# hpgmg/hpgmg

Measured on AMD Instinct MI355X. Metric: DOF/s (fine-grid) for FMG F-cycle, higher is better.
Workload: dtype f64

## Files before the change

### hpgmg_amd/__init__.py

```python
import ctypes
import os

_PKG = os.path.dirname(os.path.abspath(__file__))
REPO_ROOT = os.path.dirname(_PKG)

VECTOR_TEMP, VECTOR_U, VECTOR_F, VECTOR_E, VECTOR_R, VECTOR_DINV = 0, 1, 2, 3, 4, 5
VECTOR_BETA_I, VECTOR_BETA_J, VECTOR_BETA_K, VECTOR_ALPHA, VECTOR_L1INV = 6, 7, 8, 9, 10
BC_PERIODIC, BC_DIRICHLET = 0, 1
STENCIL_SHAPE_BOX, STENCIL_SHAPE_STAR, STENCIL_SHAPE_NO_CORNERS = 0, 1, 2
RESTRICT_CELL, RESTRICT_FACE_I, RESTRICT_FACE_J, RESTRICT_FACE_K = 0, 1, 2, 3
OP_7PT, OP_27PT, OP_FV4, OP_FV2 = 0, 1, 2, 3
SMOOTH_CHEBY, SMOOTH_GSRB, SMOOTH_JACOBI = 0, 1, 2
BOTTOM_BICGSTAB, BOTTOM_CG, BOTTOM_CABICGSTAB, BOTTOM_CACG = 0, 1, 2, 3
(INFO_DIM, INFO_BOX_DIM, INFO_GHOSTS, INFO_JSTRIDE, INFO_KSTRIDE, INFO_VOLUME, INFO_NUM_MY_BOXES,
 INFO_NUM_VECTORS, INFO_BOXES_IN_I, INFO_MY_RANK, INFO_NUM_RANKS, INFO_NUM_MY_BLOCKS, INFO_ACTIVE, INFO_COUNT) = range(14)


class Config(ctypes.Structure):
    _fields_ = [("op", ctypes.c_int), ("smoother", ctypes.c_int), ("helmholtz", ctypes.c_int), ("variable_coeff", ctypes.c_int)]


class UserInfo(ctypes.Structure):
    _fields_ = [("norm_of_residual", ctypes.c_double), ("norm_of_f", ctypes.c_double), ("mean_shift", ctypes.c_double),
                ("vcycles", ctypes.c_int), ("converged", ctypes.c_int)]


DENSE_CELL, DENSE_FACE_I, DENSE_FACE_J, DENSE_FACE_K = 0, 1, 2, 3
DENSE_CHECK_FINITE, DENSE_CHECK_POSITIVE, DENSE_CHECK_NONNEGATIVE = 0, 1, 2
DENSE_NOT_FINITE, DENSE_OUT_OF_RANGE = 1, 2
WHERE_HOST, WHERE_PLUGIN = 0, 1
(USER_OK, USER_BAD_ARGUMENT, USER_CONFLICT, USER_MULTI_RANK, USER_NOT_FINITE, USER_OUT_OF_RANGE,
 USER_NOT_READY, USER_UNSUPPORTED) = 0, -1, -2, -3, -4, -5, -6, -7
USER_FMG, USER_MG, USER_PCG, USER_FPCG = 0, 1, 2, 3
FACE_DIRICHLET, FACE_NEUMANN, FACE_ROBIN = 0, 1, 3


class HipLevel(ctypes.Structure):
    _fields_ = [("box_base", ctypes.c_void_p), ("box_low", ctypes.c_void_p), ("num_boxes", ctypes.c_int),
                ("dim", ctypes.c_int), ("ghosts", ctypes.c_int), ("jStride", ctypes.c_int), ("kStride", ctypes.c_int),
                ("volume", ctypes.c_int), ("dim_i", ctypes.c_int), ("dim_j", ctypes.c_int), ("dim_k", ctypes.c_int),
                ("periodic", ctypes.c_int), ("box_nbr", ctypes.c_void_p), ("flags", ctypes.c_int), ("box_stride", ctypes.c_longlong)]


def _declare_driver_api(lib):
    c_int, c_dbl, vp = ctypes.c_int, ctypes.c_double, ctypes.c_void_p
    P = ctypes.POINTER
    sig = {
        "hpgmg_configure": (c_int, [P(Config)]),
        "hpgmg_get_config": (None, [P(Config)]),
        "hpgmg_vectors_reserved": (c_int, []),
        "hpgmg_backend_name": (ctypes.c_char_p, []),
        "hpgmg_set_verbose": (None, [c_int]),
        "hpgmg_set_box_alignment": (None, [c_int, c_int, c_int, c_int]),
        "hpgmg_choose_boxes_in_i": (c_int, [c_int, c_int, c_int]),
        "hpgmg_solver_create": (vp, [c_int, c_int, c_int, c_int, c_int]),
        "hpgmg_solver_create_explicit": (vp, [c_int, c_int, c_int, c_int, c_int]),
        "hpgmg_solver_destroy": (None, [vp]),
        "hpgmg_solver_num_levels": (c_int, [vp]),
        "hpgmg_solver_level": (vp, [vp, c_int]),
        "hpgmg_solver_restrict_rhs": (None, [vp, c_int]),
        "hpgmg_solver_fmg": (c_dbl, [vp, c_int]),
        "hpgmg_solver_bench": (c_dbl, [vp, c_int, c_int, c_int]),
        "hpgmg_solver_richardson": (None, [vp, P(c_dbl)]),
        "hpgmg_level_info": (None, [vp, P(c_int)]),
        "hpgmg_level_h": (c_dbl, [vp]),
        "hpgmg_level_timers": (None, [vp, P(c_dbl)]),
        "hpgmg_set_timer_mode": (None, [c_int]),
        "hpgmg_get_timer_mode": (c_int, []),
        "hpgmg_level_eigenvalue": (c_dbl, [vp]),
        "hpgmg_level_must_subtract_mean": (c_int, [vp]),
        "hpgmg_level_set_eigenvalue": (None, [vp, c_dbl]),
        "hpgmg_level_box_low": (None, [vp, c_int, P(c_int)]),
        "hpgmg_level_list_counts": (c_int, [vp, c_int, c_int, P(c_int)]),
        "hpgmg_level_read_vector": (None, [vp, c_int, c_int, vp]),
        "hpgmg_level_write_vector": (None, [vp, c_int, c_int, vp]),
        "hpgmg_level_create": (vp, [c_int, c_int, c_int, c_int, c_int, c_int, c_int, c_dbl]),
        "hpgmg_level_destroy": (None, [vp]),
        "hpgmg_mg_create": (vp, [vp, c_dbl, c_dbl, c_int]),
        "hpgmg_mg_destroy": (None, [vp]),
        "hpgmg_mg_level": (vp, [vp, c_int]),
        "hpgmg_mg_num_levels": (c_int, [vp]),
        "hpgmg_set_transport": (None, [vp]),
        "hpgmg_set_bottom_solver": (None, [c_int]), "hpgmg_get_bottom_solver": (c_int, []),
        "hpgmg_set_ucycles": (None, [c_int]),
        "hpgmg_set_fmg_vcycles": (None, [c_int]),
        "MGSolve": (None, [vp, c_int, c_int, c_int, c_dbl, c_dbl, c_dbl]),
        "FMGSolve": (None, [vp, c_int, c_int, c_int, c_dbl, c_dbl, c_dbl]),
        "MGPCG": (None, [vp, c_int, c_int, c_int, c_dbl, c_dbl, c_dbl]),
        "hpgmg_solver_mg": (vp, [vp]),
        "stencil_get_radius": (c_int, []), "stencil_get_shape": (c_int, []),
        "apply_op": (None, [vp, c_int, c_int, c_dbl, c_dbl]),
        "residual": (None, [vp, c_int, c_int, c_int, c_dbl, c_dbl]),
        "smooth": (None, [vp, c_int, c_int, c_dbl, c_dbl]),
        "rebuild_operator": (None, [vp, vp, c_dbl, c_dbl]),
        "restriction": (None, [vp, c_int, vp, c_int, c_int]),
        "interpolation_vcycle": (None, [vp, c_int, c_dbl, vp, c_int]),
        "interpolation_fcycle": (None, [vp, c_int, c_dbl, vp, c_int]),
        "exchange_boundary": (None, [vp, c_int, c_int]),
        "apply_BCs": (None, [vp, c_int, c_int]),
        "apply_BCs_p1": (None, [vp, c_int, c_int]),
        "dot": (c_dbl, [vp, c_int, c_int]), "norm": (c_dbl, [vp, c_int]), "mean": (c_dbl, [vp, c_int]),
        "matmul": (None, [vp, P(c_dbl), P(c_int), P(c_int), c_int, c_int, c_int]),
        "error": (c_dbl, [vp, c_int, c_int]),
        "add_vectors": (None, [vp, c_int, c_dbl, c_int, c_dbl, c_int]),
        "scale_vector": (None, [vp, c_int, c_dbl, c_int]),
        "zero_vector": (None, [vp, c_int]),
        "shift_vector": (None, [vp, c_int, c_int, c_dbl]),
        "mul_vectors": (None, [vp, c_int, c_dbl, c_int, c_int]),
        "invert_vector": (None, [vp, c_int, c_dbl, c_int]),
        "init_vector": (None, [vp, c_int, c_dbl]),
        "color_vector": (None, [vp, c_int, c_int, c_int, c_int, c_int]),
        "random_vector": (None, [vp, c_int]),
        "initialize_problem": (None, [vp, c_dbl, c_dbl, c_dbl]),
        "IterativeSolver": (None, [vp, c_int, c_int, c_dbl, c_dbl, c_dbl]),
        "hpgmg_dense_pack": (c_int, [vp, c_int, vp, c_int, c_int, c_int]),
        "hpgmg_dense_unpack": (c_int, [vp, c_int, vp, c_int]),
        "hpgmg_user_create": (c_int, [c_int, c_int, c_int, c_int, c_int, c_dbl, c_dbl, c_dbl, P(vp)]),
        "hpgmg_user_destroy": (None, [vp]),
        "hpgmg_user_set_verbose": (None, [vp, c_int]),
        "hpgmg_user_solver_of": (vp, [vp]),
        "hpgmg_user_set_coefficients": (c_int, [vp, vp, vp, vp, vp, c_int]),
        "hpgmg_user_set_rhs": (c_int, [vp, vp, c_int, P(c_dbl)]),
        "hpgmg_user_solve": (c_int, [vp, c_int, c_dbl, vp, c_int, P(UserInfo)]),
        "hpgmg_user_set_max_iterations": (c_int, [vp, c_int]),
        "hpgmg_user_get_solution": (c_int, [vp, vp, c_int]),
        "hpgmg_user_apply": (c_int, [vp, vp, vp, c_int]),
        "hpgmg_user_set_rhs_dirichlet": (c_int, [vp, vp, vp, c_int, P(c_dbl)]),
        "hpgmg_user_apply_dirichlet": (c_int, [vp, vp, vp, vp, c_int]),
        "hpgmg_dense_pack_lifted": (c_int, [vp, c_int, vp, c_int, vp, c_dbl]),
        "hpgmg_boundary_flux": (c_int, [vp, vp, vp, c_dbl]),
        "hpgmg_boundary_restrict": (None, [vp, vp, vp, vp]),
        "hpgmg_boundary_lift": (None, [vp, c_int, vp, vp, c_dbl]),
        "hpgmg_boundary_interp": (None, [vp, c_int, vp, vp]),
        "hpgmg_user_create_faces": (c_int, [c_int, c_int, P(c_int), c_int, c_int, c_dbl, c_dbl, c_dbl, P(vp)]),
        "hpgmg_dense_pack_walls": (c_int, [vp, c_int, vp, c_int, c_int, c_int, c_int, vp]),
        "hpgmg_dense_pack_lifted_faces": (c_int, [vp, c_int, vp, c_int, vp, c_dbl, c_int, vp]),
        "hpgmg_boundary_flux_faces": (c_int, [vp, vp, vp, c_dbl, c_int, vp]),
        "hpgmg_boundary_interp_faces": (None, [vp, c_int, vp, vp, c_int]),
        "hpgmg_user_set_coefficients_robin": (c_int, [vp, vp, vp, vp, vp, vp, c_int]),
        "hpgmg_boundary_check_kappa": (c_int, [vp, vp, c_int, c_int, P(c_int)]),
        "hpgmg_boundary_store_walls": (None, [vp, vp, vp, c_int]),
        "hpgmg_dense_pack_lifted_robin": (c_int, [vp, c_int, vp, c_int, vp, c_dbl, c_int, vp, vp]),
        "hpgmg_boundary_flux_robin": (c_int, [vp, vp, vp, c_dbl, c_int, vp, vp]),
        "hpgmg_boundary_interp_robin": (None, [vp, c_int, vp, vp, c_int, vp]),
        "hpgmg_user_flux": (c_int, [vp, vp, vp, vp, vp, vp, c_int]),
        "hpgmg_dense_unpack_flux": (c_int, [vp, c_int, vp, c_dbl, c_int, vp, vp, vp, vp, vp, c_int]),
        "hpgmg_pcg_apply_dot": (c_int, [vp, c_int, c_int, c_dbl, c_dbl, P(c_dbl)]),
        "hpgmg_pcg_update": (c_int, [vp, c_int, c_int, c_int, c_int, c_dbl, P(c_dbl)]),
        "hpgmg_pcg_dot": (c_int, [vp, c_int, c_int, P(c_dbl)]),
        "hpgmg_pcg_dot2": (c_int, [vp, c_int, c_int, c_int, P(c_dbl), P(c_dbl)]),
        "hpgmg_vector_alloc": (vp, [ctypes.c_size_t]),
        "hpgmg_vector_free": (None, [vp]),
        "hpgmg_vector_copy": (None, [vp, vp, ctypes.c_size_t]),
        "hpgmg_vector_upload": (None, [vp, vp, ctypes.c_size_t]),
        "hpgmg_vector_download": (None, [vp, vp, ctypes.c_size_t]),
    }
    for name, (res, args) in sig.items():
        fn = getattr(lib, name)
        fn.restype, fn.argtypes = res, args
    return lib


def _declare_kernel_api(lib):
    c_int, c_dbl, vp = ctypes.c_int, ctypes.c_double, ctypes.c_void_p
    P = ctypes.POINTER
    L = P(HipLevel)
    sig = {
        "hpgmg_hip_device_count": (c_int, []), "hpgmg_hip_set_device": (c_int, [c_int]),
        "hpgmg_hip_set_stream": (None, [vp]), "hpgmg_hip_get_stream": (vp, []), "hpgmg_hip_sync": (c_int, []),
        "hpgmg_hip_malloc": (vp, [ctypes.c_size_t]), "hpgmg_hip_free": (None, [vp]),
        "hpgmg_hip_memcpy_h2d": (c_int, [vp, vp, ctypes.c_size_t]), "hpgmg_hip_memcpy_d2h": (c_int, [vp, vp, ctypes.c_size_t]),
        "hpgmg_hip_last_error": (ctypes.c_char_p, []),
        "hpgmg_hip_event_create": (vp, []), "hpgmg_hip_event_destroy": (None, [vp]),
        "hpgmg_hip_event_record": (c_int, [vp]), "hpgmg_hip_event_elapsed_ms": (c_dbl, [vp, vp]),
        "hpgmg_hip_profile_smoother": (None, [c_int]),
        "hpgmg_hip_profile_smoother_min_cells": (None, [ctypes.c_longlong]),
        "hpgmg_hip_profile_smoother_stride": (None, [c_int]),
        "hpgmg_hip_profile_smoother_read": (c_int, [P(c_dbl), P(ctypes.c_longlong), P(ctypes.c_longlong)]),
        "hpgmg_hip_smooth_cheby": (c_int, [L, c_int, c_int, c_int, c_int, c_dbl, c_dbl, c_dbl, c_dbl, c_dbl]),
        "hpgmg_hip_smooth_gsrb": (c_int, [L, c_int, c_int, c_int, c_int, c_dbl, c_dbl, c_dbl, c_int]),
        "hpgmg_hip_smooth_jacobi": (c_int, [L, c_int, c_int, c_int, c_int, c_dbl, c_dbl, c_dbl, c_dbl]),
        "hpgmg_hip_residual": (c_int, [L, c_int, c_int, c_int, c_int, c_dbl, c_dbl, c_dbl]),
        "hpgmg_hip_fill": (c_int, [L, c_int, c_dbl]),
        "hpgmg_hip_axpby": (c_int, [L, c_int, c_dbl, c_int, c_dbl, c_int]),
        "hpgmg_hip_scale": (c_int, [L, c_int, c_dbl, c_int]),
        "hpgmg_hip_norm_max": (c_int, [L, c_int, P(c_dbl)]),
        "hpgmg_hip_dot": (c_int, [L, c_int, c_int, P(c_dbl)]),
        "hpgmg_hip_sum": (c_int, [L, c_int, P(c_dbl)]),
        "hpgmg_hip_gram": (c_int, [L, P(c_int), c_int, P(c_int), c_int, P(c_dbl)]),
        "hpgmg_hip_pcg_dot2": (c_int, [L, c_int, c_int, c_int, P(c_dbl), P(c_dbl)]),
        "hpgmg_hip_pair_launch_counts": (None, [P(ctypes.c_longlong)]),
    }
    for name, (res, args) in sig.items():
        fn = getattr(lib, name)
        fn.restype, fn.argtypes = res, args
    return lib


def lib_paths():
    return os.path.join(_PKG, "libhpgmg_hip.so"), os.path.join(_PKG, "libhpgmg_fv.so")


_cache = {}


def load_kernels():
    if "hip" not in _cache:
        path = lib_paths()[0]
        if not os.path.exists(path):
            raise ImportError(f"{path} is missing: run `make -C hpgmg_amd/csrc` (or __graft_entry__.build()); "
                              "there is no CPU fallback for the operator kernels")
        _cache["hip"] = _declare_kernel_api(ctypes.CDLL(path, mode=ctypes.RTLD_GLOBAL))
    return _cache["hip"]


def load_driver():
    if "fv" not in _cache:
        load_kernels()
        path = lib_paths()[1]
        if not os.path.exists(path):
            raise ImportError(f"{path} is missing: run `make -C hpgmg_amd/csrc` (or __graft_entry__.build())")
        lib = _declare_driver_api(ctypes.CDLL(path))
        if lib.hpgmg_backend_name() != b"hip":
            raise ImportError("libhpgmg_fv.so is not linked against the HIP operator plugin")
        _cache["fv"] = lib
    return _cache["fv"]


def bind_driver_library(path):
    return _declare_driver_api(ctypes.CDLL(path))
```

### hpgmg_amd/csrc/host/plugin_internal.h

```cpp
#ifndef HPGMG_PLUGIN_INTERNAL_H
#define HPGMG_PLUGIN_INTERNAL_H
#include <stdio.h>
#include <stdlib.h>
#include <string.h>
#include <math.h>
#include <time.h>
#include <stdint.h>
#include "hpgmg_level.h"
#include "hpgmg_operators.h"
#include "hpgmg_mg.h"
#include "hpgmg_hip.h"

int hpgmg_smooth_sweeps(void);
int hpgmg_gsrb_out_of_place(void);

#define HP_INTERNAL __attribute__((visibility("hidden")))

enum { TIMERS_HOST = 0, TIMERS_DEVICE = 1, TIMERS_SYNC = 2 };
#define TICK(L, FIELD, WHAT) const hpgmg_tick tick_ = hpgmg_tick_begin((L), &(L)->timers.FIELD, WHAT)
#define TOCK() hpgmg_tick_end(tick_)
HP_INTERNAL void hp_lazy_flush(void);
#define HIP_OK(call) do { hp_lazy_flush(); int e_ = (call); if (e_) { fprintf(stderr, "hpgmg: %s failed (%d): %s\n", #call, e_, hpgmg_hip_last_error()); abort(); } } while (0)

#define MAX_LISTS 32
typedef struct {
  hpgmg_hip_level dev;
  double **d_box_base;  int *d_box_low;  int *d_box_nbr;  int all_faces_local;
  double  *seen_v0;     int seen_nv, seen_boxes;
  struct { const blockCopy_type *host; int n; blockCopy_type *dev; } lists[MAX_LISTS];
  int num_lists;
  hpgmg_hip_bc_entry *d_bc[STENCIL_MAX_SHAPES]; int n_bc[STENCIL_MAX_SHAPES];
  int *d_fv4_special; int n_fv4_special;
  hpgmg_hip_bc_entry *d_bc_k; int n_bc_k, bc_k_local;
  int bc_sources_local[STENCIL_MAX_SHAPES];
  int *krylov_pinned;
  double *dense_stage; size_t dense_stage_len;
  double *pair_scratch; double **d_pair_base;
  float *coef32; float **d_coef32_base; int coef32_valid;
  int lexicographic;
  int *d_restrict_map;
  struct pair_halo *halo;
  int halo_state;
  struct halo_images *img;
  int img_state;
  int img_active;
} backend_t;

enum { HALO_FIRST = 0, HALO_NEXT = 1, HALO_COEF = 2, HALO_PLANS = 3 };
typedef struct {
  int n_send, n_recv;
  hpgmg_hip_halo_entry *d_send, *d_recv;
  int n_sp, n_rp;
  int *sp_rank, *rp_rank, *sp_size, *rp_size;
  double **sp_ptr, **rp_ptr;
} halo_plan;
typedef struct pair_halo {
  int brick[3], rem[6];
  halo_plan plan[HALO_PLANS];
  double *sendbuf, *recvbuf, *deep, *deep_beta;
  int coef_valid;
} pair_halo;

enum { IMG_PLAN_COEF = 6, IMG_PLANS = 7 };
typedef struct {
  int n_send, n_recv;
  hpgmg_hip_halo_entry *d_send, *d_recv;
  int n_sp, n_rp;
  int *sp_rank, *rp_rank, *sp_size, *rp_size;
  long long *sp_off, *rp_off;
  int built;
} image_plan;
typedef struct halo_images {
  int n_real, n_img, n_all;
  int *gid;
  int *h_nbr;
  int lo[3], n[3];
  int *brick_lo, *brick_n;
  int depth_max;
  double *storage, *scratch;
  double **d_box_base, **d_pair_base; int *d_box_low, *d_box_nbr;
  hpgmg_hip_level dev, dev_all;
  image_plan plan[IMG_PLANS];
  double *sendbuf, *recvbuf; size_t send_cap, recv_cap;
  double **ptr_tmp; int ptr_cap;
  hpgmg_hip_bc_entry *d_bc; int n_bc, n_bc_own;
  hpgmg_hip_bc_entry *d_bc_k; int n_bc_k;
  int *d_special; int n_special;
  int coef_valid, shape;
  double *seen_v0; int seen_nv;
} halo_images;

typedef enum { SW_GHOST_FREE = 0, SW_ONE_LAUNCH_GHOSTS, SW_OVERLAP, SW_PAIR_REMOTE, SW_IMAGES, SW_FUSED_SWEEPS, SW_PAIR_MIN_CELLS, SW_FUSED_RESIDUAL, SW_FUSED_TAIL,
               SW_FUSED_FTAIL, SW_FUSED_BOTTOM, SW_SMALL_FUSED, SW_SMALL_VTAIL, SW_SMALL_27PT_GSRB, SW_SMALL_OPS, SW_LAZY, SW_LAZY_REPORT, SW_TEMP_SCRATCH,
               SW_FV4_NO_EXACT_RB, SW_GRAPH, SW_SMOOTHER_PRECISION, SW_DEFER_NORM, SW_BRICK_VISITS, SW_BRICK_SIZE, SW_BRICK_MIN_DIM, SW_BRICK_FSTEP, SW_BRICK_CHAIN, SW_BRICK_WIDE, SW_BRICK_WIDE_MAX_DIM, SW_BRICK_WIDE_TAIL_DIM, SW_FTAIL_MAX_DIM, SW_COUNT } hp_switch_id;
HP_INTERNAL long long hp_switch(hp_switch_id id);
HP_INTERNAL void hp_switch_set(hp_switch_id id, long long value);

HP_INTERNAL backend_t *hp_backend_of(level_type *L);
HP_INTERNAL const blockCopy_type *hp_mirror(level_type *owner, const blockCopy_type *host, int n);
HP_INTERNAL int  hp_variant(void);
HP_INTERNAL int  hp_ghost_free_mode(void);
HP_INTERNAL int  hp_box_rank_at(const level_type *L, int bi, int bj, int bk);
HP_INTERNAL void hp_ensure_pair_scratch(level_type *L, backend_t *B);
HP_INTERNAL int  hp_bc_entry_from_block(const level_type *L, int box, const int bpos[3], const int lo[3], const int len[3], int subtype,
                                        int (*find)(void *, int), void *ctx, hpgmg_hip_bc_entry *o);
HP_INTERNAL int  hp_images_ready(level_type *L, backend_t *B);
HP_INTERNAL void hp_images_refresh(level_type *L, backend_t *B, int scr, int id, int depth, int rhs_id, int bc_order);
HP_INTERNAL int  hp_images_refresh_begin(level_type *L, backend_t *B, int scr, int id, int depth, int rhs_id, int bc_order);
HP_INTERNAL void hp_images_refresh_end(void);
HP_INTERNAL int  hp_overlap_enabled(void);
HP_INTERNAL void hp_overlap_counted(void);
HP_INTERNAL void hp_images_bcs(level_type *L, backend_t *B, int scr, int id, int bc_order, int part);
HP_INTERNAL const int *hp_images_fv4_special(level_type *L, backend_t *B, int *n_out);
HP_INTERNAL const hpgmg_hip_bc_entry *hp_images_bc_k(level_type *L, backend_t *B, int *n_out);
HP_INTERNAL void hp_images_release(backend_t *B);
HP_INTERNAL void hp_images_invalidate_coefficients(backend_t *B);
extern HP_INTERNAL long long hp_images_exchanges;
static inline const hpgmg_hip_level *hp_stencil_dev(backend_t *B) { return (B->img && B->img_active) ? &B->img->dev : &B->dev; }


extern HP_INTERNAL void *hp_comm_stream, *hp_ev_packed, *hp_ev_landed;
extern HP_INTERNAL long long hp_overlap_count;
HP_INTERNAL double hp_now(void);
HP_INTERNAL void hp_transport_phase(const communicator_type *recv_side, const communicator_type *send_side, int tag);
HP_INTERNAL int hp_exchange_and_bcs_one_launch(level_type *L, int id, int shape, int order, int with_copies);
HP_INTERNAL int hp_ghosts_for_stencil(level_type *L, int id, int out_id);
HP_INTERNAL int hp_overlap_begin(level_type *L, int id);
HP_INTERNAL void hp_overlap_end(void);
HP_INTERNAL void hp_no_kernel(const char *what);
HP_INTERNAL const hpgmg_hip_bc_entry *hp_bc_entries(level_type *L, int shape, int *n_out);
HP_INTERNAL const hpgmg_hip_bc_entry *hp_bc_entries_k(level_type *L, int *n_out, int *all_local_out);
HP_INTERNAL int hp_vcycle_legs_fused(level_type **levels, int n, int e_id, int R_id, double a, double b, int leg);
HP_INTERNAL void hp_coef32_invalidate(level_type *L);
HP_INTERNAL int hp_interp_smooth_fused(level_type *Lf, int e_id, int R_id, level_type *Lc, double a, double b, int exact_state);
HP_INTERNAL void hp_do_smooth(level_type *L, int x_id, int rhs_id, double a, double b, int temp_dead);
HP_INTERNAL void hp_do_residual(level_type *L, int res_id, int x_id, int rhs_id, double a, double b);
HP_INTERNAL void hp_do_apply_op(level_type *L, int Ax_id, int x_id, double a, double b);
HP_INTERNAL int hp_pair_halo_ready(level_type *L, backend_t *B);
HP_INTERNAL int hp_pair_halo_begin(level_type *L, backend_t *B, int first, int x0_scr, int x0_id, int xm1_scr, int xm1_id, int rhs_id);
HP_INTERNAL void hp_do_restriction(level_type *Lc, int id_c, level_type *Lf, int id_f, int type);
HP_INTERNAL int hp_residual_restrict_zero_fused(level_type *Lc, int id_c, level_type *Lf, int res_id, int x_id, int rhs_id, double a, double b, int zero_id);
HP_INTERNAL int hp_norm_scale_restrict_fused(level_type *L, int F_id, int R_id, level_type *Lc, double *norm_out);
HP_INTERNAL void hp_do_interpolation_vcycle(level_type *Lf, int id_f, double prescale, level_type *Lc, int id_c);
HP_INTERNAL void hp_do_zero_vector(level_type *L, int id);
HP_INTERNAL void hp_do_add_vectors(level_type *L, int c, double sa, int a, double sb, int b);
HP_INTERNAL void hp_do_mul_vectors(level_type *L, int c, double s, int a, int b);
HP_INTERNAL void hp_do_scale_vector(level_type *L, int c, double s, int a);
HP_INTERNAL double hp_allreduce_scalar(level_type *L, double v, int op);
HP_INTERNAL void hp_allreduce_values(level_type *L, double *v, int n, int op);
HP_INTERNAL double hp_do_dot(level_type *L, int a, int b);
HP_INTERNAL double hp_do_norm(level_type *L, int a);
HP_INTERNAL void hp_small_ops_forget(void);
HP_INTERNAL const int *hp_restrict_map_of(level_type *Lf, backend_t *Bf);

#define BLAS1(call) do { TICK(L, blas1, "BLAS1"); HIP_OK(call); TOCK(); } while (0)
#define STENCIL_WITH_GHOSTS(L, id, out_id, TIMER, CALL) do {                                                     \
    hp_backend_of(L)->img_active = 0;                                                                    \
    if (hp_overlap_begin(L, id)) {                                                                          \
      TICK(L, TIMER, #TIMER " (overlapped with the halo exchange)");                                     \
      hpgmg_hip_set_defer_mode(1); HIP_OK(CALL);                                                         \
      hp_overlap_end();                                                                                     \
      hpgmg_hip_set_defer_mode(2); HIP_OK(CALL); hpgmg_hip_set_defer_mode(0);                            \
      TOCK();                                                                                            \
    } else {                                                                                             \
      const int two_parts_ = hp_ghosts_for_stencil(L, id, out_id);    \
      TICK(L, TIMER, #TIMER);                                                                            \
      if (two_parts_) {                                                                                  \
        hpgmg_hip_set_tile_part(1); HIP_OK(CALL);                                                        \
        hp_images_refresh_end();                                                                         \
        hpgmg_hip_set_tile_part(2); HIP_OK(CALL); hpgmg_hip_set_tile_part(0);                            \
      } else HIP_OK(CALL);                                                                               \
      TOCK();                                                                                            \
    } } while (0)
#define PAIR_REMOTE_LAUNCH(OVERLAPPED, DISCARD_X1, CALL) do {                                                   \
    pair_halo *H_ = B->halo;                                                                                   \
    if (OVERLAPPED) {                                                                                          \
      hpgmg_hip_pair_set_halo(H_->brick, H_->rem, H_->deep, H_->deep_beta); hpgmg_hip_set_tile_part(1);        \
      if (DISCARD_X1) hpgmg_hip_pair_discard_x1();                                                             \
      HIP_OK(CALL);                                                                                            \
      hp_overlap_end();                                                                                           \
      hpgmg_hip_pair_set_halo(H_->brick, H_->rem, H_->deep, H_->deep_beta); hpgmg_hip_set_tile_part(2);        \
      if (DISCARD_X1) hpgmg_hip_pair_discard_x1();                                                             \
      HIP_OK(CALL);                                                                                            \
      hpgmg_hip_set_tile_part(0);                                                                              \
    } else {                                                                                                   \
      hpgmg_hip_pair_set_halo(H_->brick, H_->rem, H_->deep, H_->deep_beta);                                    \
      if (DISCARD_X1) hpgmg_hip_pair_discard_x1();                                                             \
      HIP_OK(CALL);                                                                                            \
    } } while (0)

#endif
```

### hpgmg_amd/csrc/host/plugin_smooth.c

```c
#include "plugin_internal.h"

static void cheby_coefficients(const level_type *L, int degree, double *c1, double *c2) {
  double beta = 1.000 * L->dominant_eigenvalue_of_DinvA, alpha = 0.125000 * beta;
  double theta = 0.5 * (beta + alpha), delta = 0.5 * (beta - alpha), sigma = theta / delta, rho_n = 1 / sigma;
  int s;
  c1[0] = 0.0; c2[0] = 1 / theta;
  for (s = 1; s < degree; s++) { double rho_nm1 = rho_n; rho_n = 1.0 / (2.0 * sigma - rho_nm1); c1[s] = rho_n * rho_nm1; c2[s] = rho_n * 2.0 / delta; }
}

void hpgmg_level_sync_counters(level_type *L) {
  hpgmg_hip_timer_flush();
  hpgmg_level_ext *X = hpgmg_level_ext_get(L);
  backend_t *B = (backend_t *)X->backend;
  if (!B || !B->krylov_pinned) return;
  HIP_OK(hpgmg_hip_sync());
  L->Krylov_iterations += *B->krylov_pinned;
  *B->krylov_pinned = 0;
}

int hpgmg_vcycle_legs_fused(level_type **levels, int n, int e_id, int R_id, double a, double b, int leg) { hp_lazy_flush(); return hp_vcycle_legs_fused(levels, n, e_id, R_id, a, b, leg); }
static int bottom_solve_fused_impl(level_type *L, int e_id, int R_id, double a, double b, double want, int ask_only);
static level_type *tail_books_on = NULL;
static int tail_follows_bricks = 0;
static long long small_vtails = 0;
long long hpgmg_small_vtails(void) { return small_vtails; }
void hpgmg_set_small_vtail(int on) { hp_switch_set(SW_SMALL_VTAIL, (on == 2) ? 2 : (on ? 1 : 0)); }
static int small_vtail_fused(level_type **levels, int n, int e_id, int R_id, double a, double b, int legs, int ask_only) {
  hpgmg_config cfg;
  hpgmg_hip_small_tail_args T;
  int l;
  const int small_vtail_on = (int)hp_switch(SW_SMALL_VTAIL);
  if (!small_vtail_on) return 0;
  hpgmg_get_config(&cfg);
  if (small_vtail_on == 2 && cfg.op == HPGMG_OP_27PT && cfg.smoother == HPGMG_SMOOTH_GSRB && !tail_follows_bricks) return 0;
  const int sweeps = hpgmg_smooth_sweeps();
  if (n < 2 || n > HPGMG_HIP_SMALL_TAIL_MAX_LEVELS || sweeps < 1 || sweeps > 8 || (sweeps & 1) || hp_switch(SW_GRAPH)) return 0;
  if (cfg.smoother != HPGMG_SMOOTH_CHEBY && cfg.smoother != HPGMG_SMOOTH_GSRB && cfg.smoother != HPGMG_SMOOTH_JACOBI) return 0;
  memset(&T, 0, sizeof T);
  T.n = n; T.legs = legs; T.mode = (cfg.smoother == HPGMG_SMOOTH_CHEBY) ? 0 : (cfg.smoother == HPGMG_SMOOTH_GSRB ? 1 : 2);
  T.sweeps = sweeps; T.out_of_place = (T.mode == 1) ? hpgmg_gsrb_out_of_place() : 0;
  T.e_id = e_id; T.R_id = R_id; T.krylov_base = hpgmg_vectors_reserved(); T.a = a; T.b = b; T.want = MG_DEFAULT_BOTTOM_NORM;
  const int shape = stencil_get_shape();
  for (l = 0; l < n; l++) {
    level_type *L = levels[l];
    if (!L->active || L->num_my_boxes != 1 || L->boxes_in.i * L->boxes_in.j * L->boxes_in.k != 1) return 0;
    if (L->boundary_condition.type != BC_DIRICHLET || L->dim.i != L->dim.j || L->dim.i != L->dim.k) return 0;
    if (l > 0 && 2 * L->dim.i != levels[l - 1]->dim.i) return 0;
    {
      communicator_type *C = &L->exchange_ghosts[shape], *CB = &L->exchange_ghosts[STENCIL_SHAPE_BOX];
      if (C->num_sends + C->num_recvs > 0 || C->num_blocks[0] || C->num_blocks[1] || C->num_blocks[2]) return 0;
      if (CB->num_sends + CB->num_recvs > 0 || CB->num_blocks[0] || CB->num_blocks[1] || CB->num_blocks[2]) return 0;
    }
    backend_t *B = hp_backend_of(L);
    hpgmg_hip_small_tail_level *v = &T.lv[l];
    v->L = B->dev;
    v->h2inv = 1.0 / (L->h * L->h);
    v->n_bc = L->boundary_condition.num_blocks[shape];
    v->bc_list = v->n_bc ? hp_mirror(L, L->boundary_condition.blocks[shape], v->n_bc) : NULL;
    if (cfg.op == HPGMG_OP_27PT) v->bc_kind = (L->box_dim < 2) ? 1 : 2;
    else if (cfg.op == HPGMG_OP_FV2 || L->box_dim < 4) { v->bc_kind = (L->box_dim < 2) ? 1 : 3; v->zero_first = (v->bc_kind == 3 && L->box_ghosts > 1); }
    else { v->bc_kind = 4; v->zero_first = (L->box_ghosts > 2); }
    v->n_ibc = L->boundary_condition.num_blocks[STENCIL_SHAPE_BOX];
    v->ibc_list = v->n_ibc ? hp_mirror(L, L->boundary_condition.blocks[STENCIL_SHAPE_BOX], v->n_ibc) : NULL;
    if (cfg.op == HPGMG_OP_27PT) v->ibc_kind = (L->box_dim < 2) ? 1 : 2;
    else { v->ibc_kind = (L->box_dim < 2) ? 1 : 3; v->ibc_zero_first = (v->ibc_kind == 3 && L->box_ghosts > 1); }
    if (v->n_bc > 32 || v->n_ibc > 32) return 0;
    if (l + 1 < n) {
      if (T.mode == 0) { if (L->dominant_eigenvalue_of_DinvA <= 0.0) return 0; cheby_coefficients(L, sweeps, v->c1, v->c2); }
      if (T.mode == 2) { int q; for (q = 0; q < sweeps; q++) v->c2[q] = 2.0 / 3.0; }
    } else if (legs & 2) {
      if (L->must_subtract_mean != 0) return 0;
      if ((long long)L->dim.i * L->dim.j * L->dim.k > hpgmg_hip_bottom_bicgstab_max_cells()) return 0;
      if (L->numVectors < hpgmg_vectors_reserved() + IterativeSolver_NumVectors()) return 0;
      if (!B->krylov_pinned) { B->krylov_pinned = (int *)hpgmg_hip_host_malloc(64); if (B->krylov_pinned) *B->krylov_pinned = 0; }
      if (!B->krylov_pinned) return 0;
      T.krylov_iterations = B->krylov_pinned;
    }
  }
  if (hpgmg_hip_small_vtail_lds_doubles(&T) > hpgmg_hip_small_vtail_lds_limit()) return 0;
  if (ask_only) return 1;
  TICK(tail_books_on ? tail_books_on : levels[0], smooth, "fused V-cycle tail (levels of one box)");
  HIP_OK(hpgmg_hip_small_vtail(&T, hp_variant()));
  TOCK();
  small_vtails++;
  return 1;
}
void hpgmg_set_fused_tail(int on) { hp_switch_set(SW_FUSED_TAIL, on ? 1 : 0); }
void hpgmg_set_fused_bottom(int on) { hp_switch_set(SW_FUSED_BOTTOM, on ? 1 : 0); }
void hpgmg_set_brick_visits(int on) { hp_switch_set(SW_BRICK_VISITS, on ? 1 : 0); if (on == 8 || on == 16) hp_switch_set(SW_BRICK_SIZE, on); }
long long hpgmg_brick_visits(void) { return hpgmg_hip_brick_visits(); }
void hpgmg_set_brick_wide(int on) { hp_switch_set(SW_BRICK_WIDE, on ? 1 : 0); }
void hpgmg_set_brick_chains(int on) { hp_switch_set(SW_BRICK_CHAIN, on ? 1 : 0); }
static int dense_level_ok(level_type *L) {
  backend_t *B = hp_backend_of(L);
  const int nb = L->dim.i / L->box_dim;
  int bx;
  if (!L->active || L->num_my_boxes < 1 || !B->all_faces_local) return 0;
  if (L->boundary_condition.type != BC_DIRICHLET || L->dim.i != L->dim.j || L->dim.i != L->dim.k) return 0;
  if (L->num_my_boxes != nb * nb * nb) return 0;
  for (bx = 0; bx < L->num_my_boxes; bx++) {
    const box_type *X = &L->my_boxes[bx];
    if (X->low.i != (bx % nb) * L->box_dim || X->low.j != ((bx / nb) % nb) * L->box_dim || X->low.k != (bx / (nb * nb)) * L->box_dim) return 0;
  }
  return 1;
}
static int brick_op_is_wide(const hpgmg_config *cfg) { return cfg->op == HPGMG_OP_27PT || cfg->op == HPGMG_OP_FV4; }
static long long brick_capacity_refusals = 0;
long long hpgmg_brick_capacity_refusals(void) { return brick_capacity_refusals; }
static int brick_prefix(level_type **levels, int n, const hpgmg_config *cfg) {
  const int sweeps = hpgmg_smooth_sweeps();
  int k = 0;
  const int wide = brick_op_is_wide(cfg);
  if (!hp_switch(SW_BRICK_VISITS) || !hp_switch(SW_FUSED_TAIL) || hp_switch(SW_GRAPH)) return 0;
  if (wide ? (!hp_switch(SW_BRICK_WIDE) || (cfg->smoother != HPGMG_SMOOTH_CHEBY && cfg->smoother != HPGMG_SMOOTH_GSRB) || (cfg->smoother == HPGMG_SMOOTH_GSRB && !hpgmg_gsrb_out_of_place()))
           : (!hp_ghost_free_mode() || cfg->op != HPGMG_OP_7PT)) return 0;
  if (sweeps < 1 || sweeps > hpgmg_hip_brick_visit_max_sweeps() || (sweeps & 1)) return 0;
  while (k + 1 < n) {
    level_type *L = levels[k];
    const int fits_tail = wide ? (L->num_my_boxes == 1 && L->boxes_in.i * L->boxes_in.j * L->boxes_in.k == 1 && L->dim.i <= (int)hp_switch(SW_BRICK_WIDE_TAIL_DIM))
                               : ((long long)L->dim.i * L->dim.j * L->dim.k <= hpgmg_hip_tail_max_cells());
    if ((wide || L->dim.i < (int)hp_switch(SW_BRICK_MIN_DIM)) && fits_tail) break;
    if (wide && L->dim.i > (int)hp_switch(SW_BRICK_WIDE_MAX_DIM)) return 0;
    if (!dense_level_ok(L) || !dense_level_ok(levels[k + 1]) || 2 * levels[k + 1]->dim.i != L->dim.i) return 0;
    const int wide_brick = wide ? hpgmg_hip_brick_wide_supported(&hp_backend_of(L)->dev, hp_variant()) : 0;
    if (wide ? !wide_brick
             : !hpgmg_hip_brick_visit_supported(&hp_backend_of(L)->dev, (int)hp_switch(SW_BRICK_SIZE))) { if (fits_tail) break; return 0; }
    {
      const int brick = wide ? wide_brick : (int)hp_switch(SW_BRICK_SIZE), side = L->dim.i / brick;
      const int capacity = wide ? hpgmg_hip_brick_wide_capacity(hp_variant(), cfg->smoother) : hpgmg_hip_brick_chain_capacity(hp_variant(), cfg->smoother, brick);
      if (side * side * side > capacity) { brick_capacity_refusals++; if (fits_tail) break; return 0; }
    }
    if (L->dominant_eigenvalue_of_DinvA <= 0.0 && cfg->smoother == HPGMG_SMOOTH_CHEBY) return 0;
    k++;
  }
  return k;
}
static void brick_chain(level_type *top, level_type **levels, int first, int count, const hpgmg_config *cfg, int e_id, int R_id, double a, double b, int dir, int top_e_zero, int below_zero) {
  const int sweeps = hpgmg_smooth_sweeps(), chain = (int)hp_switch(SW_BRICK_CHAIN), max_n = (chain == 1 || (chain == 2 && dir != 1) || (chain == 3 && dir == 1)) ? hpgmg_hip_brick_chain_max_levels() : 1;
  int done = 0;
  while (done < count) {
    hpgmg_hip_brick_level lv[4];
    int n = count - done, j, s;
    if (n > max_n) n = max_n;
    if (brick_op_is_wide(cfg)) {
      const int v = hp_variant();
      if (dir == 1) { const int b0 = hpgmg_hip_brick_wide_supported(&hp_backend_of(levels[first + count - done - 1])->dev, v);
                      int m = 1; while (m < n && hpgmg_hip_brick_wide_supported(&hp_backend_of(levels[first + count - done - 1 - m])->dev, v) == b0) m++; n = m; }
      else          { const int b0 = hpgmg_hip_brick_wide_supported(&hp_backend_of(levels[first + done])->dev, v);
                      int m = 1; while (m < n && hpgmg_hip_brick_wide_supported(&hp_backend_of(levels[first + done + m])->dev, v) == b0) m++; n = m; }
    }
    const int lo = (dir == 1) ? first + count - done - n : first + done;
    for (j = 0; j < n; j++) {
      level_type *L = levels[lo + j];
      lv[j].L = hp_backend_of(L)->dev; lv[j].h2inv = 1.0 / (L->h * L->h);
      for (s = 0; s < 8; s++) lv[j].c1[s] = lv[j].c2[s] = 0.0;
      if (cfg->smoother == HPGMG_SMOOTH_CHEBY) cheby_coefficients(L, sweeps, lv[j].c1, lv[j].c2);
    }
    const int is_first_launch = (done == 0), is_last_launch = (done + n == count);
    TICK(top, smooth, dir == 1 ? "level visits, up (bricks: interpolation + smooth per level, one launch)" :
                      (dir == 0 ? "level visits, down (bricks: smooth + residual + restriction per level, one launch)" : "interpolation_fcycle + level visit, down (bricks, one launch)"));
    if (brick_op_is_wide(cfg))
      HIP_OK(hpgmg_hip_brick_wide_chain(n, lv, &hp_backend_of(levels[lo + n])->dev, sweeps, hp_variant(), cfg->smoother, e_id, R_id, a, b, dir,
                                        dir == 0 ? (is_first_launch ? top_e_zero : 1) : 0, (dir != 1 && is_last_launch) ? below_zero : 0));
    else
    HIP_OK(hpgmg_hip_brick_chain(n, lv, &hp_backend_of(levels[lo + n])->dev, sweeps, hp_variant(), cfg->smoother, e_id, R_id, a, b, dir, (int)hp_switch(SW_BRICK_SIZE),
                                 dir == 0 ? (is_first_launch ? top_e_zero : 1) : 0, (dir != 1 && is_last_launch) ? below_zero : 0));
    TOCK();
    done += n;
  }
}
int hp_vcycle_legs_fused(level_type **levels, int n, int e_id, int R_id, double a, double b, int leg) {
  hpgmg_config cfg;
  const hpgmg_hip_level *dev[8];
  int l, s, probe = 0;
  double h2inv[8], c1[64], c2[64];
  const int enabled = (int)hp_switch(SW_FUSED_TAIL), bottom_enabled = (int)hp_switch(SW_FUSED_BOTTOM);
  hpgmg_get_config(&cfg);
  if (leg >= HPGMG_LEG_ASK) { probe = 1; leg -= HPGMG_LEG_ASK; }
  if ((leg <= HPGMG_LEG_VCYCLE || leg == HPGMG_LEG_FCYCLE_STEP) && !probe) {
    const int fstep = (leg == HPGMG_LEG_FCYCLE_STEP), vleg = fstep ? HPGMG_LEG_VCYCLE : leg;
    if (fstep && (!hp_switch(SW_BRICK_FSTEP) || brick_op_is_wide(&cfg))) return 0;
    const int k = brick_prefix(levels, n, &cfg);
    const int outer_follows = tail_follows_bricks;
    tail_follows_bricks = outer_follows || (k > 0);
    const int tail_ok = (k > (fstep ? 1 : 0)) && hp_vcycle_legs_fused(levels + k, n - k, e_id, R_id, a, b, HPGMG_LEG_ASK + vleg);
    tail_follows_bricks = outer_follows;
    if (tail_ok) {
      if (vleg != 1) {
        if (fstep) { brick_chain(levels[0], levels, 0, 1, &cfg, e_id, R_id, a, b, 2, 0, 0); brick_chain(levels[0], levels, 1, k - 1, &cfg, e_id, R_id, a, b, 0, 1, 1); }
        else brick_chain(levels[0], levels, 0, k, &cfg, e_id, R_id, a, b, 0, 0, 1);
      }
      tail_books_on = levels[0]; tail_follows_bricks = 1;
      const int taken = hp_vcycle_legs_fused(levels + k, n - k, e_id, R_id, a, b, vleg);
      tail_books_on = NULL; tail_follows_bricks = outer_follows;
      if (!taken) { fprintf(stderr, "hpgmg: the V-cycle tail was refused after being accepted\n"); abort(); }
      if (vleg != 0) brick_chain(levels[0], levels, 0, k, &cfg, e_id, R_id, a, b, 1, 0, 0);
      return 1;
    }
    if (fstep) return 0;
  }
  if (leg == HPGMG_LEG_FCYCLE_STEP) return 0;
  if (leg >= 2 && (e_id >= hpgmg_vectors_reserved() || R_id >= hpgmg_vectors_reserved())) return 0;
  if (leg >= 2 && hpgmg_get_bottom_solver() != HPGMG_BOTTOM_BICGSTAB) return 0;
  const int sweeps = hpgmg_smooth_sweeps();
  const int with_bottom = (leg >= 2);
  if (enabled && cfg.op != HPGMG_OP_7PT && n == 1 && tail_follows_bricks && leg <= 2) {
    if (leg != 2) return 1;
    if (!bottom_enabled || hpgmg_get_bottom_solver() != HPGMG_BOTTOM_BICGSTAB || e_id >= hpgmg_vectors_reserved() || R_id >= hpgmg_vectors_reserved()) return 0;
    return bottom_solve_fused_impl(levels[0], e_id, R_id, a, b, MG_DEFAULT_BOTTOM_NORM, probe);
  }
  if (enabled && cfg.op != HPGMG_OP_7PT) {
    if (leg == 2) return bottom_enabled ? small_vtail_fused(levels, n, e_id, R_id, a, b, 7, probe) : 0;
    if (leg == 0 || leg == 1) return small_vtail_fused(levels, n, e_id, R_id, a, b, leg == 0 ? 1 : 4, probe);
    return 0;
  }
  if (!enabled || !hp_ghost_free_mode() || cfg.op != HPGMG_OP_7PT || n > 8 || n > hpgmg_hip_tail_max_levels() || sweeps > 8) return 0;
  if (with_bottom && !bottom_enabled) return 0;
  if (n < (leg == 3 ? 1 : 2)) return 0;
  if (leg >= 4 && (!hp_switch(SW_FUSED_FTAIL) || levels[0]->dim.i > (int)hp_switch(SW_FTAIL_MAX_DIM))) return 0;
  for (l = 0; l < n; l++) {
    level_type *L = levels[l];
    backend_t *B = hp_backend_of(L);
    const long long cells = (long long)L->dim.i * L->dim.j * L->dim.k;
    if (!L->active || L->num_my_boxes < 1 || !B->all_faces_local) return 0;
    if (L->boundary_condition.type != BC_DIRICHLET || L->dim.i != L->dim.j || L->dim.i != L->dim.k || (sweeps & 1)) return 0;
    if (l > 0 && 2 * L->dim.i != levels[l - 1]->dim.i) return 0;
    {
      const int nb = L->dim.i / L->box_dim;
      int bx;
      if (L->num_my_boxes != nb * nb * nb) return 0;
      for (bx = 0; bx < L->num_my_boxes; bx++) {
        const box_type *X = &L->my_boxes[bx];
        if (X->low.i != (bx % nb) * L->box_dim || X->low.j != ((bx / nb) % nb) * L->box_dim || X->low.k != (bx / (nb * nb)) * L->box_dim) return 0;
      }
    }
    if (l + 1 < n) {
      if (cells > hpgmg_hip_tail_max_cells()) return 0;
      if (L->dominant_eigenvalue_of_DinvA <= 0.0 && cfg.smoother == HPGMG_SMOOTH_CHEBY) return 0;
      cheby_coefficients(L, sweeps, c1 + l * sweeps, c2 + l * sweeps);
    } else {
      for (s = 0; s < sweeps; s++) c1[l * sweeps + s] = c2[l * sweeps + s] = 0.0;
      if (with_bottom) {
        if (cells > hpgmg_hip_tail_bottom_max_cells() || L->must_subtract_mean == 1) return 0;
        if (L->numVectors < hpgmg_vectors_reserved() + IterativeSolver_NumVectors()) return 0;
        L->must_subtract_mean = 0;
        if (!B->krylov_pinned) B->krylov_pinned = (int *)hpgmg_hip_host_malloc(64);
        if (!B->krylov_pinned) return 0;
      }
    }
    dev[l] = &B->dev;
    h2inv[l] = 1.0 / (L->h * L->h);
  }
  if (leg == HPGMG_LEG_FCYCLE_TAIL_ASK || probe) return 1;
  TICK(tail_books_on ? tail_books_on : levels[0], smooth, leg == 3 ? "bottom solve (device BiCGStab)" : (leg == 4 ? "fused F-cycle tail" : "fused V-cycle tail"));
  HIP_OK(hpgmg_hip_vcycle_tail(n, dev, h2inv, c1, c2, sweeps, hp_variant(), cfg.smoother, e_id, R_id, a, b, leg,
                               hpgmg_vectors_reserved(), MG_DEFAULT_BOTTOM_NORM, with_bottom ? hp_backend_of(levels[n - 1])->krylov_pinned : NULL));
  TOCK();
  return 1;
}

static int boxes_lexicographic(level_type *L) {
  backend_t *B = hp_backend_of(L);
  if (B->lexicographic < 0) {
    int bx, ok = (L->num_my_boxes == L->boxes_in.i * L->boxes_in.j * L->boxes_in.k);
    for (bx = 0; ok && bx < L->num_my_boxes; bx++) {
      const box_type *X = &L->my_boxes[bx];
      if (X->low.i != (bx % L->boxes_in.i) * L->box_dim || X->low.j != ((bx / L->boxes_in.i) % L->boxes_in.j) * L->box_dim ||
          X->low.k != (bx / (L->boxes_in.i * L->boxes_in.j)) * L->box_dim) ok = 0;
    }
    B->lexicographic = ok;
  }
  return B->lexicographic;
}

void hpgmg_set_smoother_precision(int bits) { hp_switch_set(SW_SMOOTHER_PRECISION, (bits == 32) ? 32 : 64); }
int hpgmg_get_smoother_precision(void) {
  return hp_switch(SW_SMOOTHER_PRECISION) == 32 ? 32 : 64;
}
static const float *const *coef32_of(level_type *L) {
  backend_t *B = hp_backend_of(L);
  if (hpgmg_get_smoother_precision() != 32) return NULL;
  if (!B->coef32) {
    int bx;
    float **base = (float **)calloc((size_t)L->num_my_boxes, sizeof(float *));
    B->coef32 = (float *)hpgmg_hip_malloc(((size_t)L->num_my_boxes * 5 * (size_t)L->box_volume + 4) * sizeof(float));
    B->d_coef32_base = (float **)hpgmg_hip_malloc((size_t)L->num_my_boxes * sizeof(float *));
    if (!B->coef32 || !B->d_coef32_base) { fprintf(stderr, "hpgmg: no memory for the fp32 coefficient copies\n"); abort(); }
    const size_t pad = ((uintptr_t)L->my_boxes[0].vectors[0] % 16) / sizeof(double);
    for (bx = 0; bx < L->num_my_boxes; bx++) base[bx] = B->coef32 + pad + (size_t)bx * 5 * (size_t)L->box_volume;
    HIP_OK(hpgmg_hip_memcpy_h2d(B->d_coef32_base, base, (size_t)L->num_my_boxes * sizeof(float *)));
    free(base);
    B->coef32_valid = 0;
  }
  if (!B->coef32_valid) { HIP_OK(hpgmg_hip_coef32_refresh(&B->dev, (float *const *)B->d_coef32_base, L->numVectors)); B->coef32_valid = 1; }
  return (const float *const *)B->d_coef32_base;
}
void hp_coef32_invalidate(level_type *L) { backend_t *B = hp_backend_of(L); B->coef32_valid = 0; if (B->halo) B->halo->coef_valid = 0; hp_images_invalidate_coefficients(B); hpgmg_hip_pair_packed_invalidate(&B->dev); }

static long long pair_remote_smooths = 0, fp32_pair_smooths = 0;
long long hpgmg_pair_remote_smooths(void) { return pair_remote_smooths; }
long long hpgmg_fp32_pair_smooths(void) { hp_lazy_flush(); return fp32_pair_smooths; }

void hp_ensure_pair_scratch(level_type *L, backend_t *B) {
  if (!B->pair_scratch) {
    int bx;
    double **base = (double **)calloc((size_t)L->num_my_boxes, sizeof(double *));
    B->pair_scratch = (double *)hpgmg_hip_malloc(((size_t)L->num_my_boxes * 2 * (size_t)L->box_volume + 2) * sizeof(double));
    B->d_pair_base = (double **)hpgmg_hip_malloc((size_t)L->num_my_boxes * sizeof(double *));
    if (!B->pair_scratch || !B->d_pair_base) { fprintf(stderr, "hpgmg: no memory for the sweep-pair scratch vectors\n"); abort(); }
    const size_t pad = ((uintptr_t)L->my_boxes[0].vectors[0] % 16) / sizeof(double);
    for (bx = 0; bx < L->num_my_boxes; bx++) base[bx] = B->pair_scratch + pad + (size_t)bx * 2 * (size_t)L->box_volume;
    HIP_OK(hpgmg_hip_memcpy_h2d(B->d_pair_base, base, (size_t)L->num_my_boxes * sizeof(double *)));
    free(base);
  }
}
void hpgmg_set_fused_sweeps(int on) { hp_switch_set(SW_FUSED_SWEEPS, on ? 1 : 0); }
void hpgmg_set_pair_min_cells(long long cells) { hp_switch_set(SW_PAIR_MIN_CELLS, cells > 0 ? cells : 2000000); }
static int pair_kernel_ready(level_type *L, int x_id, int rhs_id, int sweeps) {
  hpgmg_config cfg;
  hpgmg_get_config(&cfg);
  backend_t *B = hp_backend_of(L);
  if (!hp_switch(SW_FUSED_SWEEPS) || sweeps != 4 || cfg.op != HPGMG_OP_7PT || !hp_ghost_free_mode() || stencil_get_shape() != STENCIL_SHAPE_STAR) return 0;
  if (L->boundary_condition.type != BC_DIRICHLET || x_id == VECTOR_TEMP || rhs_id == VECTOR_TEMP) return 0;
  if (B->all_faces_local) { if (!hpgmg_hip_smooth_cheby_pair_supported(&B->dev, hp_variant()) || !boxes_lexicographic(L)) return 0; }
  else if (!hp_pair_halo_ready(L, B)) return 0;
  {
    if ((long long)L->dim.i * L->dim.j * L->dim.k < hp_switch(SW_PAIR_MIN_CELLS)) return 0;
  }
  hp_ensure_pair_scratch(L, B);
  hpgmg_hip_set_ghost_free(1);
  return 1;
}


static long long interp_folded_remote = 0;
long long hpgmg_interp_folded_remote(void) { return interp_folded_remote; }
static int first_pair_folded(const hpgmg_hip_level *fold_Lc, backend_t *B, int v, int x_id, int rhs_id, double a, double b, double h2inv, const double *c1, const double *c2) {
  hpgmg_hip_pair_fold_interpolation(fold_Lc, x_id, 1.0);
  return hpgmg_hip_smooth_cheby_pair(&B->dev, v, (double *const *)B->d_pair_base, NULL, 0, x_id, 0, VECTOR_TEMP, 1, 0, 1, 1, rhs_id, a, b, h2inv, c1[0], c2[0], c1[1], c2[1]);
}
static int smooth_cheby_pairs_fold(level_type *L, int x_id, int rhs_id, double a, double b, const double *c1, const double *c2, int sweeps, int temp_dead, const hpgmg_hip_level *fold_Lc) {
  if (!pair_kernel_ready(L, x_id, rhs_id, sweeps)) return 0;
  backend_t *B = hp_backend_of(L);
  const double h2inv = 1.0 / (L->h * L->h);
  const int v = hp_variant();
  const int remote = !B->all_faces_local;
  const float *const *c32 = remote ? NULL : coef32_of(L);
  int over = 0;
  if (c32) fp32_pair_smooths++;
  if (remote) {
    pair_remote_smooths++;
    if (fold_Lc) { hpgmg_hip_pair_halo_fold_interpolation(fold_Lc, x_id, 1.0); interp_folded_remote++; }
    over = hp_pair_halo_begin(L, B, 1, 0, x_id, 0, VECTOR_TEMP, rhs_id);
  }
  { TICK(L, smooth, "smooth (Chebyshev sweeps 1+2)");
    if (remote && fold_Lc) PAIR_REMOTE_LAUNCH(over, 0, first_pair_folded(fold_Lc, B, v, x_id, rhs_id, a, b, h2inv, c1, c2));
    else if (remote) PAIR_REMOTE_LAUNCH(over, 0, hpgmg_hip_smooth_cheby_pair(&B->dev, v, (double *const *)B->d_pair_base, c32, 0, x_id, 0, VECTOR_TEMP, 1, 0, 1, 1, rhs_id, a, b, h2inv, c1[0], c2[0], c1[1], c2[1]));
    else HIP_OK(hpgmg_hip_smooth_cheby_pair(&B->dev, v, (double *const *)B->d_pair_base, c32, 0, x_id, 0, VECTOR_TEMP, 1, 0, 1, 1, rhs_id, a, b, h2inv, c1[0], c2[0], c1[1], c2[1]));
    TOCK(); }
  if (remote) over = hp_pair_halo_begin(L, B, 0, 1, 1, 1, 0, rhs_id);
  { TICK(L, smooth, "smooth (Chebyshev sweeps 3+4)");
    if (remote) PAIR_REMOTE_LAUNCH(over, temp_dead, hpgmg_hip_smooth_cheby_pair(&B->dev, v, (double *const *)B->d_pair_base, c32, 1, 1, 1, 0, 0, VECTOR_TEMP, 0, x_id, rhs_id, a, b, h2inv, c1[2], c2[2], c1[3], c2[3]));
    else {
      if (temp_dead) hpgmg_hip_pair_discard_x1();
      HIP_OK(hpgmg_hip_smooth_cheby_pair(&B->dev, v, (double *const *)B->d_pair_base, c32, 1, 1, 1, 0, 0, VECTOR_TEMP, 0, x_id, rhs_id, a, b, h2inv, c1[2], c2[2], c1[3], c2[3]));
    }
    TOCK(); }
  return 1;
}
static int smooth_cheby_pairs(level_type *L, int x_id, int rhs_id, double a, double b, const double *c1, const double *c2, int sweeps, int temp_dead) {
  return smooth_cheby_pairs_fold(L, x_id, rhs_id, a, b, c1, c2, sweeps, temp_dead, NULL);
}
static int smooth_gsrb_pairs(level_type *L, int x_id, int rhs_id, double a, double b, int sweeps) {
  if (hpgmg_gsrb_out_of_place() || !pair_kernel_ready(L, x_id, rhs_id, sweeps)) return 0;
  backend_t *B = hp_backend_of(L);
  const double h2inv = 1.0 / (L->h * L->h);
  const int v = hp_variant();
  const int remote = !B->all_faces_local;
  int over = 0;
  if (remote) { pair_remote_smooths++; over = hp_pair_halo_begin(L, B, 1, 0, x_id, 0, x_id, rhs_id); }
  { TICK(L, smooth, "smooth (GSRB half sweeps 1+2)");
    if (remote) PAIR_REMOTE_LAUNCH(over, 0, hpgmg_hip_smooth_gsrb_pair(&B->dev, v, (double *const *)B->d_pair_base, NULL, 0, x_id, 0, 1, 1, rhs_id, a, b, h2inv, 0));
    else HIP_OK(hpgmg_hip_smooth_gsrb_pair(&B->dev, v, (double *const *)B->d_pair_base, NULL, 0, x_id, 0, 1, 1, rhs_id, a, b, h2inv, 0));
    TOCK(); }
  if (remote) over = hp_pair_halo_begin(L, B, 0, 1, 1, 1, 1, rhs_id);
  { TICK(L, smooth, "smooth (GSRB half sweeps 3+4)");
    if (remote) PAIR_REMOTE_LAUNCH(over, 0, hpgmg_hip_smooth_gsrb_pair(&B->dev, v, (double *const *)B->d_pair_base, NULL, 1, 1, 0, 0, x_id, rhs_id, a, b, h2inv, 2));
    else HIP_OK(hpgmg_hip_smooth_gsrb_pair(&B->dev, v, (double *const *)B->d_pair_base, NULL, 1, 1, 0, 0, x_id, rhs_id, a, b, h2inv, 2));
    TOCK(); }
  return 1;
}

int hpgmg_interp_smooth_fused(level_type *Lf, int e_id, int R_id, level_type *Lc, double a, double b) { hp_lazy_flush(); return hp_interp_smooth_fused(Lf, e_id, R_id, Lc, a, b, 0); }
static long long interp_folded_single = 0;
long long hpgmg_interp_folded_single(void) { return interp_folded_single; }
static int interp_smooth_fused_single(level_type *Lf, int e_id, int R_id, level_type *Lc, double a, double b) {
  hpgmg_config cfg;
  hpgmg_get_config(&cfg);
  const int sweeps = hpgmg_smooth_sweeps(), v = hp_variant();
  communicator_type *S = &Lc->interpolation, *Rv = &Lf->interpolation;
  if (!hp_switch(SW_FUSED_RESIDUAL) || cfg.op != HPGMG_OP_7PT || cfg.smoother != HPGMG_SMOOTH_CHEBY || !Lf->active || !Lc->active || sweeps < 2) return 0;
  if (Lf->num_my_boxes < 1 || Lc->num_my_boxes < 1 || !hp_ghost_free_mode() || Lf->boundary_condition.type != BC_DIRICHLET) return 0;
  if (S->num_sends || Rv->num_recvs || S->num_blocks[0] || Rv->num_blocks[2]) return 0;
  if (e_id == VECTOR_TEMP || R_id == VECTOR_TEMP || Lf->dominant_eigenvalue_of_DinvA <= 0.0) return 0;
  backend_t *B = hp_backend_of(Lf), *Bc = hp_backend_of(Lc);
  if (!B->all_faces_local || stencil_get_shape() != STENCIL_SHAPE_STAR) return 0;
  hpgmg_hip_set_ghost_free(1);
  if (!hpgmg_hip_smooth_cheby_fold_supported(&B->dev, v)) return 0;
  const int *map = hp_restrict_map_of(Lf, B);
  if (!map) return 0;
  double c1[16], c2[16];
  const double h2inv = 1.0 / (Lf->h * Lf->h);
  int s;
  cheby_coefficients(Lf, sweeps, c1, c2);
  B->img_active = 0;
  for (s = 0; s < sweeps; s++) {
    const int src = (s & 1) ? VECTOR_TEMP : e_id, dst = (s & 1) ? e_id : VECTOR_TEMP;
    TICK(Lf, smooth, s < 2 ? "smooth (Chebyshev sweep, interpolation folded in)" : "smooth");
    if (s < 2) hpgmg_hip_stencil_fold_interpolation(&Bc->dev, e_id, map, s + 1);
    HIP_OK(hpgmg_hip_smooth_cheby(&B->dev, v, src, dst, R_id, a, b, h2inv, c1[s], c2[s]));
    TOCK();
  }
  interp_folded_single++;
  return 1;
}
int hp_interp_smooth_fused(level_type *Lf, int e_id, int R_id, level_type *Lc, double a, double b, int exact_state) {
  hpgmg_config cfg;
  hpgmg_get_config(&cfg);
  const int sweeps = hpgmg_smooth_sweeps();
  communicator_type *S = &Lc->interpolation, *Rv = &Lf->interpolation;
  if (cfg.op != HPGMG_OP_7PT || !Lf->active || !Lc->active) return 0;
  if (cfg.smoother != HPGMG_SMOOTH_CHEBY && !(cfg.smoother == HPGMG_SMOOTH_GSRB && !hpgmg_gsrb_out_of_place())) return 0;
  if (S->num_sends || Rv->num_recvs || S->num_blocks[0] || Rv->num_blocks[2]) return 0;
  const int remote = !hp_backend_of(Lf)->all_faces_local;
  int parents_in_place = (Lc->num_my_boxes == Lf->num_my_boxes), bx;
  for (bx = 0; parents_in_place && bx < Lf->num_my_boxes; bx++)
    parents_in_place = (2 * Lc->my_boxes[bx].low.i == Lf->my_boxes[bx].low.i && 2 * Lc->my_boxes[bx].low.j == Lf->my_boxes[bx].low.j && 2 * Lc->my_boxes[bx].low.k == Lf->my_boxes[bx].low.k);
  if ((remote && Lf->box_dim % 128 != 0) || Lc->box_dim * 2 != Lf->box_dim || !parents_in_place ||       (!remote && !boxes_lexicographic(Lc)) ||
      (remote && (cfg.smoother != HPGMG_SMOOTH_CHEBY || !hp_switch(SW_PAIR_REMOTE))) ||
      !pair_kernel_ready(Lf, e_id, R_id, sweeps))
    return interp_smooth_fused_single(Lf, e_id, R_id, Lc, a, b);
  if (cfg.smoother == HPGMG_SMOOTH_CHEBY && Lf->dominant_eigenvalue_of_DinvA <= 0.0) return 0;
  if (!remote) hpgmg_hip_pair_fold_interpolation(&hp_backend_of(Lc)->dev, e_id, 1.0);
  if (cfg.smoother == HPGMG_SMOOTH_CHEBY) {
    double c1[16], c2[16];
    cheby_coefficients(Lf, sweeps, c1, c2);
    const int done = smooth_cheby_pairs_fold(Lf, e_id, R_id, a, b, c1, c2, sweeps, !exact_state && hp_switch(SW_TEMP_SCRATCH), remote ? &hp_backend_of(Lc)->dev : NULL);
    if (!done) { fprintf(stderr, "hpgmg: fused interpolation+smooth refused after being accepted\n"); abort(); }
  } else if (!smooth_gsrb_pairs(Lf, e_id, R_id, a, b, sweeps)) { fprintf(stderr, "hpgmg: fused interpolation+smooth refused after being accepted\n"); abort(); }
  return 1;
}

void hpgmg_set_small_fused(int mode) { hp_switch_set(SW_SMALL_FUSED, (mode == 1 || mode == 2) ? 2 : 0); }
static int small_level_try(level_type *L, int mode, int x_id, int rhs_id, int res_id, double a, double b) {
  hpgmg_config cfg;
  const int small_fused = hp_switch(SW_SMALL_FUSED) ? 2 : 0;
  hpgmg_get_config(&cfg);
  const int small_27 = (int)hp_switch(SW_SMALL_27PT_GSRB);
  const int worth = (mode <= 2) && (small_27 || !(cfg.op == HPGMG_OP_27PT && cfg.smoother == HPGMG_SMOOTH_GSRB));
  const int enabled = (small_fused == 2 && worth && L->num_my_boxes == 1 && (size_t)9 * (size_t)L->box_volume * sizeof(double) <= (size_t)150 * 1024);
  if (!enabled || cfg.op == HPGMG_OP_7PT || L->num_my_boxes < 1) return 0;
  if ((long long)L->dim.i * L->dim.j * L->dim.k > hpgmg_hip_small_level_max_cells()) return 0;
  if (L->num_my_boxes != L->boxes_in.i * L->boxes_in.j * L->boxes_in.k) return 0;
  const int shape = stencil_get_shape();
  communicator_type *C = &L->exchange_ghosts[shape];
  if (C->num_sends + C->num_recvs > 0 || C->num_blocks[0] || C->num_blocks[2]) return 0;
  int bc_kind = 0, zero_first = 0, n_bc = 0;
  if (L->boundary_condition.type != BC_PERIODIC) {
    n_bc = L->boundary_condition.num_blocks[shape];
    if (cfg.op == HPGMG_OP_27PT) bc_kind = (L->box_dim < 2) ? 1 : 2;
    else if (cfg.op == HPGMG_OP_FV2 || L->box_dim < 4) { bc_kind = (L->box_dim < 2) ? 1 : 3; zero_first = (bc_kind == 3 && L->box_ghosts > 1); }
    else { bc_kind = 4; zero_first = (L->box_ghosts > 2); }
  }
  const int sweeps = (mode <= 2) ? hpgmg_smooth_sweeps() : 1;
  double c1[16], c2[16];
  int q;
  for (q = 0; q < 16; q++) c1[q] = c2[q] = 0.0;
  if (mode == 0) cheby_coefficients(L, sweeps, c1, c2);
  if (mode == 2) for (q = 0; q < sweeps; q++) c2[q] = 2.0 / 3.0;
  if (sweeps > 8) return 0;
  backend_t *B = hp_backend_of(L);
  const double t_h2inv = 1.0 / (L->h * L->h);
  hpgmg_tick tk = hpgmg_tick_begin(L, mode <= 2 ? &L->timers.smooth : (mode == 3 ? &L->timers.residual : &L->timers.apply_op), "small level, one launch");
  HIP_OK(hpgmg_hip_small_level_op(&B->dev, hp_variant(), mode, sweeps, x_id, rhs_id, res_id, mode == 1 ? hpgmg_gsrb_out_of_place() : 0, a, b, t_h2inv, c1, c2,
                                  hp_mirror(L, C->blocks[1], C->num_blocks[1]), C->num_blocks[1],
                                  n_bc ? hp_mirror(L, L->boundary_condition.blocks[shape], n_bc) : NULL, n_bc, bc_kind, zero_first));
  hpgmg_tick_end(tk);
  return 1;
}

static int bottom_solve_fused_impl(level_type *L, int e_id, int R_id, double a, double b, double want, int ask_only);
int hpgmg_bottom_solve_fused(level_type *L, int e_id, int R_id, double a, double b, double want) { return bottom_solve_fused_impl(L, e_id, R_id, a, b, want, 0); }
static int bottom_solve_fused_impl(level_type *L, int e_id, int R_id, double a, double b, double want, int ask_only) {
  hpgmg_config cfg;
  const int on = (int)hp_switch(SW_FUSED_BOTTOM);
  hpgmg_get_config(&cfg);
  if (!on || cfg.op == HPGMG_OP_7PT || !L->active || L->num_my_boxes != 1 || L->boxes_in.i * L->boxes_in.j * L->boxes_in.k != 1) return 0;
  if (e_id >= hpgmg_vectors_reserved() || R_id >= hpgmg_vectors_reserved()) return 0;
  if (L->boundary_condition.type == BC_PERIODIC || L->must_subtract_mean == 1) return 0;
  if ((long long)L->dim.i * L->dim.j * L->dim.k > hpgmg_hip_bottom_bicgstab_max_cells()) return 0;
  const int shape = stencil_get_shape();
  communicator_type *C = &L->exchange_ghosts[shape];
  if (C->num_sends + C->num_recvs > 0 || C->num_blocks[0] || C->num_blocks[1] || C->num_blocks[2]) return 0;
  int bc_kind, zero_first = 0;
  const int n_bc = L->boundary_condition.num_blocks[shape];
  if (cfg.op == HPGMG_OP_27PT) bc_kind = (L->box_dim < 2) ? 1 : 2;
  else if (cfg.op == HPGMG_OP_FV2 || L->box_dim < 4) { bc_kind = (L->box_dim < 2) ? 1 : 3; zero_first = (bc_kind == 3 && L->box_ghosts > 1); }
  else { bc_kind = 4; zero_first = (L->box_ghosts > 2); }
  if (L->numVectors < hpgmg_vectors_reserved() + IterativeSolver_NumVectors()) return 0;
  if (ask_only) return 1;
  hp_lazy_flush();
  backend_t *B = hp_backend_of(L);
  if (!B->krylov_pinned) { B->krylov_pinned = (int *)hpgmg_hip_host_malloc(64); if (B->krylov_pinned) *B->krylov_pinned = 0; }
  if (!B->krylov_pinned) return 0;
  HIP_OK(hpgmg_hip_bottom_bicgstab(&B->dev, hp_variant(), e_id, R_id, hpgmg_vectors_reserved(), a, b, 1.0 / (L->h * L->h), want,
                                   n_bc ? hp_mirror(L, L->boundary_condition.blocks[shape], n_bc) : NULL, n_bc, bc_kind, zero_first, B->krylov_pinned));
  return 1;
}

int hpgmg_smooth_in_cycle(level_type *L, int x_id, int rhs_id, double a, double b) {
  hp_lazy_flush();
  hp_do_smooth(L, x_id, rhs_id, a, b, (int)hp_switch(SW_TEMP_SCRATCH));
  return 1;
}
static long long fv4_rb_smooths = 0, rb27_smooth_passes = 0;
long long hpgmg_rb27_passes(void) { return rb27_smooth_passes; }
long long hpgmg_fv4_rb_smooths(void) { return fv4_rb_smooths; }
static void fv4_rb_bcs(level_type *L, backend_t *B, int scratch, int id) {
  const int shape = stencil_get_shape();
  if (L->boundary_condition.type == BC_PERIODIC) return;
  if (!scratch) { if (!hp_exchange_and_bcs_one_launch(L, id, shape, 4, 0)) apply_BCs(L, id, shape); return; }
  int n = 0;
  const hpgmg_hip_bc_entry *e = hp_bc_entries(L, shape, &n);
  hpgmg_hip_level Ls = B->dev;
  Ls.box_base = (double *const *)B->d_pair_base;
  TICK(L, boundary_conditions, "apply_BCs_v4 (private vector)");
  HIP_OK(hpgmg_hip_exchange_and_bc(&Ls, id, NULL, 0, e, n, 4));
  TOCK();
}
static const int *fv4_special_cells(level_type *L, backend_t *B, int *n_out) {
  if (B->n_fv4_special < 0) {
    int cap = 1024, n = 0, b, ax, side, u, v;
    int *h = (int *)malloc((size_t)cap * 4 * sizeof(int));
    const int dim = L->box_dim, N[3] = { L->dim.i, L->dim.j, L->dim.k }, nb[3] = { L->boxes_in.i, L->boxes_in.j, L->boxes_in.k };
    if (L->boundary_condition.type != BC_PERIODIC)
    for (b = 0; b < L->num_my_boxes; b++) {
      const int low[3] = { L->my_boxes[b].low.i, L->my_boxes[b].low.j, L->my_boxes[b].low.k };
      for (ax = 0; ax < 3; ax++) for (side = 0; side < 2; side++) {
        const int bpos = low[ax] / dim + (side ? 1 : -1);
        if (bpos < 0 || bpos >= nb[ax]) continue;
        const int a1 = (ax + 1) % 3, a2 = (ax + 2) % 3;
        for (v = 0; v < dim; v++) for (u = 0; u < dim; u++) {
          const int g1 = low[a1] + u, g2 = low[a2] + v;
          if (!(g1 == 0 || g1 == N[a1] - 1 || g2 == 0 || g2 == N[a2] - 1)) continue;
          int c[3];
          c[ax] = side ? dim - 1 : 0; c[a1] = u; c[a2] = v;
          if (n == cap) { cap *= 2; h = (int *)realloc(h, (size_t)cap * 4 * sizeof(int)); }
          h[4 * n] = b; h[4 * n + 1] = c[0]; h[4 * n + 2] = c[1]; h[4 * n + 3] = c[2]; n++;
        }
      }
    }
    B->d_fv4_special = (int *)hpgmg_hip_malloc((size_t)(n > 0 ? n : 1) * 4 * sizeof(int));
    if (!B->d_fv4_special) { fprintf(stderr, "hpgmg: device allocation failed: %s\n", hpgmg_hip_last_error()); abort(); }
    if (n > 0) HIP_OK(hpgmg_hip_memcpy_h2d(B->d_fv4_special, h, (size_t)n * 4 * sizeof(int)));
    free(h);
    B->n_fv4_special = n;
  }
  *n_out = B->n_fv4_special;
  return B->d_fv4_special;
}
static int smooth_fv4_rb(level_type *L, int x_id, int rhs_id, double a, double b, int sweeps, int temp_dead) {
  hpgmg_config cfg;
  hpgmg_get_config(&cfg);
  backend_t *B = hp_backend_of(L);
  const int passes = sweeps / 2, v = hp_variant();
  if (cfg.op != HPGMG_OP_FV4 || !hpgmg_gsrb_out_of_place() || !temp_dead || !hp_ghost_free_mode() || (sweeps & 1) || passes < 1) return 0;
  if (L->num_my_boxes < 1 || x_id == VECTOR_TEMP || rhs_id == VECTOR_TEMP || L->box_dim < 8) return 0;
  const int images = !B->all_faces_local;
  if (images && !hp_images_ready(L, B)) return 0;
  const hpgmg_hip_level *dev = images ? &B->img->dev : &B->dev;
  if (!hpgmg_hip_smooth_gsrb_fv4_rb_supported(dev, v)) return 0;
  int n_k = 0, k_local = 1, n_all = 0, p;
  const hpgmg_hip_bc_entry *e_k = NULL;
  if (images) e_k = hp_images_bc_k(L, B, &n_k);
  else if (L->boundary_condition.type != BC_PERIODIC) {
    e_k = hp_bc_entries_k(L, &n_k, &k_local);
    (void)hp_bc_entries(L, stencil_get_shape(), &n_all);
    if (!k_local || !B->bc_sources_local[stencil_get_shape()]) return 0;
  }
  hp_ensure_pair_scratch(L, B);
  double *const *pair_base = images ? (double *const *)B->img->d_pair_base : (double *const *)B->d_pair_base;
  hpgmg_hip_set_tile_ghost_free(1);
  const double h2inv = 1.0 / (L->h * L->h);
  int n_sp = 0;
  const int *sp_cells = images ? hp_images_fv4_special(L, B, &n_sp) : fv4_special_cells(L, B, &n_sp);
  int src_s = 0, src_id = x_id;
  for (p = 0; p < passes; p++) {
    int dst_s = 0, dst_id;
    const int left = passes - p;
    if (left == 1) dst_id = (passes == 1) ? VECTOR_TEMP : x_id;
    else if (left == 2 && !(src_s == 0 && src_id == x_id)) { dst_s = 1; dst_id = 0; }
    else dst_id = (src_s == 0 && src_id == VECTOR_TEMP) ? x_id : VECTOR_TEMP;
    if (left == 2 && src_s == 0 && src_id == x_id) dst_id = VECTOR_TEMP;
    int overlapped = 0;
    if (images) overlapped = hp_images_refresh_begin(L, B, src_s, src_id, 3, p == 0 ? rhs_id : -1, 4);
    else fv4_rb_bcs(L, B, src_s, src_id);
    TICK(L, smooth, "smooth (fv4 GSRB, red + black half sweeps in one pass)");
    if (overlapped) {
      hpgmg_hip_set_tile_part(1);
      HIP_OK(hpgmg_hip_smooth_gsrb_fv4_rb(dev, v, pair_base, src_s, src_id, dst_s, dst_id, 1, rhs_id, a, b, h2inv, 2 * p));
      hp_images_refresh_end();
      hpgmg_hip_set_tile_part(2);
    }
    HIP_OK(hpgmg_hip_fv4_rb_prepass(images ? &B->img->dev_all : dev, v, pair_base, src_s, src_id, 1, rhs_id, a, b, h2inv, 2 * p, e_k, n_k, sp_cells, n_sp));
    HIP_OK(hpgmg_hip_smooth_gsrb_fv4_rb(dev, v, pair_base, src_s, src_id, dst_s, dst_id, 1, rhs_id, a, b, h2inv, 2 * p));
    if (overlapped) hpgmg_hip_set_tile_part(0);
    TOCK();
    src_s = dst_s; src_id = dst_id;
  }
  if (passes == 1) hp_do_scale_vector(L, x_id, 1.0, VECTOR_TEMP);
  fv4_rb_smooths++;
  return 1;
}
void hp_do_smooth(level_type *L, int x_id, int rhs_id, double a, double b, int temp_dead) {
  hpgmg_config cfg;
  hpgmg_get_config(&cfg);
  const int sweeps = hpgmg_smooth_sweeps(), v = hp_variant();
  const double h2inv = 1.0 / (L->h * L->h);
  backend_t *B = hp_backend_of(L);
  int s;
  if (cfg.op != HPGMG_OP_7PT && small_level_try(L, cfg.smoother == HPGMG_SMOOTH_CHEBY ? 0 : (cfg.smoother == HPGMG_SMOOTH_GSRB ? 1 : 2), x_id, rhs_id, x_id, a, b)) return;
  if (cfg.smoother == HPGMG_SMOOTH_CHEBY) {
    double c1[16], c2[16];
    if (L->dominant_eigenvalue_of_DinvA <= 0.0 && L->my_rank == 0) fprintf(stderr, "dominant_eigenvalue_of_DinvA <= 0.0 !\n");
    cheby_coefficients(L, sweeps, c1, c2);
    if (smooth_cheby_pairs(L, x_id, rhs_id, a, b, c1, c2, sweeps, temp_dead)) return;
    for (s = 0; s < sweeps; s++) {
      const int src = (s & 1) ? VECTOR_TEMP : x_id, dst = (s & 1) ? x_id : VECTOR_TEMP;
      STENCIL_WITH_GHOSTS(L, src, dst, smooth, hpgmg_hip_smooth_cheby(hp_stencil_dev(B), v, src, dst, rhs_id, a, b, h2inv, c1[s], c2[s]));
    }
  } else if (cfg.smoother == HPGMG_SMOOTH_GSRB) {
    const int oop = hpgmg_gsrb_out_of_place();
    if (smooth_gsrb_pairs(L, x_id, rhs_id, a, b, sweeps)) return;
    if (cfg.op == HPGMG_OP_27PT && oop && temp_dead && hp_ghost_free_mode() && sweeps % 4 == 0 && L->num_my_boxes > 0 &&
        (B->all_faces_local || hp_images_ready(L, B)) && x_id != VECTOR_TEMP && rhs_id != VECTOR_TEMP) {
      const int images = !B->all_faces_local;
      const hpgmg_hip_level *dev = images ? &B->img->dev : &B->dev;
      const int tiled = hpgmg_hip_smooth_gsrb27_rb_supported(dev);
      const int boxed = !tiled && hpgmg_hip_smooth_gsrb27_rb_box_supported(dev);
      if (tiled || boxed) {
        for (s = 0; s < sweeps; s += 2) {
          const int src = (s & 2) ? VECTOR_TEMP : x_id, dst = (s & 2) ? x_id : VECTOR_TEMP;
          int overlapped = 0;
          if (images && tiled) overlapped = hp_images_refresh_begin(L, B, 0, src, 2, s == 0 ? rhs_id : -1, 12);
          else if (images) hp_images_refresh(L, B, 0, src, 2, s == 0 ? rhs_id : -1, 12);
          else if (tiled && !hp_exchange_and_bcs_one_launch(L, src, stencil_get_shape(), 12, 0)) apply_BCs(L, src, stencil_get_shape());
          TICK(L, smooth, "smooth (27-point GSRB, red + black half sweeps in one pass)");
          if (overlapped) {
            hpgmg_hip_set_tile_part(1); HIP_OK(hpgmg_hip_smooth_gsrb27_rb(dev, src, dst, rhs_id, a, b, h2inv, s));
            hp_images_refresh_end();
            hpgmg_hip_set_tile_part(2); HIP_OK(hpgmg_hip_smooth_gsrb27_rb(dev, src, dst, rhs_id, a, b, h2inv, s));
            hpgmg_hip_set_tile_part(0);
          } else
          if (tiled) HIP_OK(hpgmg_hip_smooth_gsrb27_rb(dev, src, dst, rhs_id, a, b, h2inv, s));
          else       HIP_OK(hpgmg_hip_smooth_gsrb27_rb_box(dev, src, dst, rhs_id, a, b, h2inv, s));
          TOCK();
          rb27_smooth_passes++;
        }
        return;
      }
    }
    if (smooth_fv4_rb(L, x_id, rhs_id, a, b, sweeps, temp_dead)) return;
    int first_half_sweep = 0;
    if (cfg.op == HPGMG_OP_FV4 && oop && !temp_dead && sweeps >= 6 && !(sweeps & 1) && (((sweeps - 2) / 2) & 1) == 0 && !hp_switch(SW_FV4_NO_EXACT_RB)) {
      if (smooth_fv4_rb(L, x_id, rhs_id, a, b, sweeps - 2, 1)) first_half_sweep = sweeps - 2;
    }
    for (s = first_half_sweep; s < sweeps; s++) {
      const int src = (oop && (s & 1)) ? VECTOR_TEMP : x_id, dst = oop ? ((s & 1) ? x_id : VECTOR_TEMP) : x_id;
      STENCIL_WITH_GHOSTS(L, src, dst, smooth, hpgmg_hip_smooth_gsrb(hp_stencil_dev(B), v, src, dst, rhs_id, a, b, h2inv, s));
    }
  } else {
    for (s = 0; s < sweeps; s++) {
      const int src = (s & 1) ? VECTOR_TEMP : x_id, dst = (s & 1) ? x_id : VECTOR_TEMP;
      STENCIL_WITH_GHOSTS(L, src, dst, smooth, hpgmg_hip_smooth_jacobi(hp_stencil_dev(B), v, src, dst, rhs_id, a, b, h2inv, 2.0 / 3.0));
    }
  }
}

void hp_do_residual(level_type *L, int res_id, int x_id, int rhs_id, double a, double b) {
  if (small_level_try(L, 3, x_id, rhs_id, res_id, a, b)) return;
  STENCIL_WITH_GHOSTS(L, x_id, res_id, residual, hpgmg_hip_residual(hp_stencil_dev(hp_backend_of(L)), hp_variant(), res_id, x_id, rhs_id, a, b, 1.0 / (L->h * L->h)));
}
void hp_do_apply_op(level_type *L, int Ax_id, int x_id, double a, double b) {
  if (small_level_try(L, 4, x_id, -1, Ax_id, a, b)) return;
  STENCIL_WITH_GHOSTS(L, x_id, Ax_id, apply_op, hpgmg_hip_residual(hp_stencil_dev(hp_backend_of(L)), hp_variant(), Ax_id, x_id, -1, a, b, 1.0 / (L->h * L->h)));
}
```

### hpgmg_amd/csrc/host/plugin_switches.c

```c
#include "plugin_internal.h"

enum { K_ON = 0, K_OFF = 1, K_INT = 2, K_TRI = 3 };
static struct { const char *env; int kind; long long dflt; const char *what; long long value; int known; } table[SW_COUNT] = {
  [SW_GHOST_FREE]        = { "HPGMG_GHOST_FREE", K_ON, 1, "stencil launches read neighbouring boxes and the Dirichlet rule themselves; 0: the reference's exchange + boundary + stencil launches" },
  [SW_ONE_LAUNCH_GHOSTS] = { "HPGMG_ONE_LAUNCH_GHOSTS", K_ON, 1, "27-pt / fv2 / fv4: box-to-box ghost copies and boundary conditions as one launch" },
  [SW_OVERLAP]           = { "HPGMG_OVERLAP", K_ON, 1, "N > 1: halo exchanges on a second stream under the part of the stencil launch that does not need them" },
  [SW_PAIR_REMOTE]       = { "HPGMG_PAIR_REMOTE", K_ON, 1, "N > 1, 7-pt: sweep pairs across rank boundaries (two-deep halo, one exchange per pair); 0: one exchange per sweep" },
  [SW_IMAGES]            = { "HPGMG_IMAGES", K_ON, 1, "N > 1, 27-pt / fv4: images of the neighbouring ranks' boxes (one-pass red + black kernels keep running); 0: exchange_boundary per half sweep" },
  [SW_FUSED_SWEEPS]      = { "HPGMG_FUSED_SWEEPS", K_ON, 1, "7-pt: two smoother sweeps per pass on bandwidth-bound levels" },
  [SW_PAIR_MIN_CELLS]    = { "HPGMG_PAIR_MIN_CELLS", K_INT, 2000000, "7-pt: smallest level (cells) that takes the sweep-pair kernel (2 M: the 128^3 level too, since the kernel picks its launch shape per launch -- 16 workgroup rows of 10 waves x 16 chunks = 256 workgroups there: config 2 2.70 vs 2.74 ms; with 16 waves it lost, 3.02 vs 2.92: profiles/r06k_ab_pair_min.txt, r06n_ab_pair_min.txt)" },
  [SW_FUSED_RESIDUAL]    = { "HPGMG_FUSED_RESIDUAL", K_ON, 1, "residual + restriction (+ zero_vector), residual + norm, norm + copy + restriction as one pass each" },
  [SW_FUSED_TAIL]        = { "HPGMG_FUSED_TAIL", K_ON, 1, "7-pt: the V-cycle below the brick levels (<= 8^3; <= 16^3 without them) as one single-workgroup launch" },
  [SW_FUSED_FTAIL]       = { "HPGMG_FUSED_FTAIL", K_ON, 1, "7-pt: the F-cycle's own work below 32^3 as one launch" },
  [SW_FUSED_BOTTOM]      = { "HPGMG_FUSED_BOTTOM", K_ON, 1, "BiCGStab bottom solve on the device; 0: driven from the host (host/solvers.c) through the operators" },
  [SW_SMALL_FUSED]       = { "HPGMG_SMALL_FUSED", K_TRI, 2, "27-pt / fv2 / fv4: smooth() of a one-box level as one launch on an LDS image (2, default); 0 off" },
  [SW_SMALL_VTAIL]       = { "HPGMG_SMALL_VTAIL", K_TRI, 2, "27-pt / fv2 / fv4: the V-cycle below a one-box level as one launch: 2 on except for 27-pt GSRB (default), 1 on, 0 off" },
  [SW_SMALL_27PT_GSRB]   = { "HPGMG_TUNE_SMALL_27PT_GSRB", K_OFF, 0, "27-pt GSRB: the one-launch small-level smooth() instead of the one-workgroup-per-box red + black kernel" },
  [SW_SMALL_OPS]         = { "HPGMG_SMALL_OPS", K_ON, 1, "BLAS-1 / operator calls of a host-driven Krylov solver on a small one-box level go out with the scalar that follows them" },
  [SW_LAZY]              = { "HPGMG_LAZY", K_ON, 1, "void operators are postponed while they follow MGVCycle's call order and issued fused (the reference's own driver, INTEGRATION.md Route B)" },
  [SW_LAZY_REPORT]       = { "HPGMG_LAZY_REPORT", K_OFF, 0, "print what the operator queue did when the process ends" },
  [SW_TEMP_SCRATCH]      = { "HPGMG_TEMP_SCRATCH", K_ON, 1, "inside a cycle VECTOR_TEMP is scratch after smooth(): in-cycle smoother forms; 0: the exact state of smooth() everywhere" },
  [SW_FV4_NO_EXACT_RB]   = { "HPGMG_TUNE_FV4_NO_EXACT_RB", K_OFF, 0, "fv4: the exported smooth() as six half sweeps (no red + black passes)" },
  [SW_GRAPH]             = { "HPGMG_GRAPH", K_OFF, 0, "capture / replay the launch-bound segments as hipGraphs (measured slower with a full stream)" },
  [SW_DEFER_NORM]        = { "HPGMG_DEFER_NORM", K_ON, 1, "FMGSolve: norm(F) of the opening pass is collected at the end, where it is used, instead of waited for at the start" },
  [SW_BRICK_VISITS]     = { "HPGMG_BRICK_VISITS", K_ON, 1, "7-pt: the 64^3 / 32^3 / 16^3 levels of a V-cycle leg as one launch of 8^3 bricks that trade faces, residuals and corrections inside the launch; 0 when other processes run such launches on the same GPU" },
  [SW_BRICK_SIZE]       = { "HPGMG_TUNE_BRICK", K_INT, 8, "side of those bricks: 8 (512 lanes, one cell each) or 16 (1024 lanes, four cells each)" },
  [SW_BRICK_MIN_DIM]    = { "HPGMG_TUNE_BRICK_MIN", K_INT, 16, "smallest level (cells per side) visited as bricks; the levels below it are the single-workgroup tail's" },
  [SW_BRICK_FSTEP]      = { "HPGMG_TUNE_BRICK_FSTEP", K_ON, 1, "FMGSolve: interpolation_fcycle onto a brick level rides in the first launch of the V-cycle that follows it" },
  [SW_BRICK_CHAIN]      = { "HPGMG_TUNE_BRICK_CHAIN", K_INT, 1, "consecutive brick levels of a V-cycle leg in ONE launch (what passes between the levels passes inside it); 0: one launch per level visit" },
  [SW_BRICK_WIDE]       = { "HPGMG_BRICK_WIDE", K_ON, 1, "27-pt / fv4: the same for the operators with wide stencils (kernels/brick_wide.hip: halo of the stencil's radius, apply_BCs_p2 / _v4 on the LDS image)" },
  [SW_BRICK_WIDE_MAX_DIM] = { "HPGMG_TUNE_BRICK_WIDE_MAX", K_INT, 64, "largest level (cells per side) the 27-pt / fv4 plugins visit as bricks (measured: fv4 `7 64` 29.71 / 29.91 / 30.15 ms with 64 / 32 / 16, 27-pt 12.27 / 12.51 / 12.52)" },
  [SW_BRICK_WIDE_TAIL_DIM] = { "HPGMG_TUNE_BRICK_WIDE_TAIL", K_INT, 1, "27-pt / fv4: the largest one-box level left to the single-workgroup tail (1: the 8^3, 4^3 (and 27-pt: 2^3) levels are visited as ONE brick each and only the bottom solve is left; 2 / 4 / 8: the tail starts there)" },
  [SW_FTAIL_MAX_DIM]    = { "HPGMG_TUNE_FTAIL_MAX", K_INT, 8, "7-pt: the largest level (cells per side) the single-launch F-cycle tail starts from (8: the 16^3 step of the climb is a brick launch each way, eight CUs instead of one: config 1 0.320 vs 0.328 ms with 16, config 2 the same within noise; profiles/r06i_ab_ftail.txt)" },
  [SW_SMOOTHER_PRECISION]= { "HPGMG_SMOOTHER_PRECISION", K_INT, 64, "32: fp32 coefficient streams in the Chebyshev sweep pairs (BASELINE config 5: within 2e-4 of the fp64 norms, and bit-exact against the CPU oracle's fp32 mode, which rounds the same coefficients); 64: bit-exact" },
};

long long hp_switch(hp_switch_id id) {
  if (!table[id].known) {
    const char *e = getenv(table[id].env);
    long long v = table[id].dflt;
    switch (table[id].kind) {
      case K_ON:  v = !(e && e[0] == '0'); break;
      case K_OFF: v = (e && e[0] == '1'); break;
      case K_INT: if (e && *e) v = atoll(e); break;
      default:    v = (e && e[0] == '0') ? 0 : ((e && e[0] == '1') ? 1 : table[id].dflt); break;
    }
    table[id].value = v; table[id].known = 1;
  }
  return table[id].value;
}
void hp_switch_set(hp_switch_id id, long long value) { table[id].value = value; table[id].known = 1; }

void hpgmg_print_switches(void) {
  int q;
  for (q = 0; q < SW_COUNT; q++) fprintf(stderr, "  %-28s = %-8lld (default %lld)  %s\n", table[q].env, hp_switch((hp_switch_id)q), table[q].dflt, table[q].what);
}
__attribute__((constructor)) static void switches_report(void) { const char *e = getenv("HPGMG_SWITCHES"); if (e && e[0] == '1') hpgmg_print_switches(); }
```

### hpgmg_amd/csrc/kernels/cheby_pair.hpp

```cpp
#pragma once
#include "common.hpp"
#include "stencil_math.hpp"

namespace hpgmg {

struct VecRef { int scratch, id; };
struct PairArgs {
  VecRef x0, xm1, out1, out2;
  int rhs_id;
  double a, b, h2inv, c1a, c2a, c1b, c2b;
  int sweep_a;
  int keep_x1;
  hpgmg_hip_level Lc; int coarse_id; double prescale;
  double *const *scr_base;
  const float *const *c32_base;
  int nbi, nbj;
  int Di, Dj, Dk;
  int rem[6];
  const double *deep;
  const double *deep_beta;
  int tiles_i, slabs_j, chunks_k, KC, per_xcd, total_blocks;
  int edge_blocks, edge_per_xcd;
  double *edge_coef;
  const int *order;
};

__device__ __forceinline__ double *pair_vec(const hpgmg_hip_level &L, const PairArgs &A, VecRef r, int box) {
  double *base = r.scratch ? A.scr_base[box] : L.box_base[box];
  return base + (size_t)r.id * (size_t)L.volume + (size_t)L.ghosts * (size_t)(1 + L.jStride + L.kStride);
}
struct LaneShift { long long lvl, scr, c32; };
__device__ __forceinline__ long long shift_of(const LaneShift &s, VecRef r) { return r.scratch ? s.scr : s.lvl; }

struct alignas(16) p2 { double x, y; };
typedef double __attribute__((ext_vector_type(2))) d2v;
typedef const d2v __attribute__((address_space(1))) *gd2cptr;
typedef d2v __attribute__((address_space(1))) *gd2ptr;
__device__ __forceinline__ p2 pld(const double *p) { const d2v v = *(gd2cptr)as_global(p); return p2{v.x, v.y}; }
__device__ __forceinline__ void pst(double *p, p2 v) { d2v w; w.x = v.x; w.y = v.y; *(gd2ptr)as_global(p) = w; }
__device__ __forceinline__ double gld1(const double *p) { return *as_global(p); }
__device__ __forceinline__ p2 pneg(p2 v) { return p2{-v.x, -v.y}; }
__device__ __forceinline__ int uni(int v) { return __builtin_amdgcn_readfirstlane(v); }

enum { C32_DINV = 0, C32_ALPHA, C32_BETA_I, C32_BETA_J, C32_BETA_K, C32_COUNT };
template <bool C32> struct CoefStream {
  const double *p64; const float *p32;
  __device__ __forceinline__ CoefStream(const hpgmg_hip_level &L, const PairArgs &A, int box, int vec_id, int slot, const LaneShift &sh = LaneShift{0, 0, 0}) {
    const size_t first = (size_t)L.ghosts * (size_t)(1 + L.jStride + L.kStride);
    if (C32) { p32 = A.c32_base[box] + (size_t)slot * (size_t)L.volume + first + sh.c32; p64 = nullptr; }
    else     { p64 = L.box_base[box] + (size_t)vec_id * (size_t)L.volume + first + sh.lvl; p32 = nullptr; }
  }
  __device__ __forceinline__ p2 pair(int off) const {
    if (C32) { typedef float __attribute__((ext_vector_type(2))) f2v; const f2v f = *(const f2v __attribute__((address_space(1))) *)(p32 + off); return p2{(double)f.x, (double)f.y}; }
    return pld(p64 + off);
  }
  __device__ __forceinline__ double one(int off) const { return C32 ? (double)*(const float __attribute__((address_space(1))) *)(p32 + off) : gld1(p64 + off); }
};

template <int V> struct PlaneCoef { p2 rhs, dinv, al, bi, bjlo, bjhi, bk0, bk1; double bir; };

enum { PAIR_CHEBY = 0, PAIR_GSRB = 1 };
template <int V, int SM>
__device__ __forceinline__ p2 pair_update(p2 c, double left, double right, p2 jm, p2 jp, p2 km, p2 kp, p2 old,
                                          const PlaneCoef<V> &q, double a, double b, double h2inv, double c1, double c2, bool first_is_swept) {
  const double Ax0 = apply_op_7pt<V>(c.x, left, c.y, jm.x, jp.x, km.x, kp.x, q.bi.x, q.bi.y, q.bjlo.x, q.bjhi.x, q.bk0.x, q.bk1.x, q.al.x, a, b, h2inv);
  const double Ax1 = apply_op_7pt<V>(c.y, c.x, right, jm.y, jp.y, km.y, kp.y, q.bi.y, q.bir, q.bjlo.y, q.bjhi.y, q.bk0.y, q.bk1.y, q.al.y, a, b, h2inv);
  p2 o;
  if (SM == PAIR_CHEBY) {
    o.x = c.x + c1 * (c.x - old.x) + c2 * q.dinv.x * (q.rhs.x - Ax0);
    o.y = c.y + c1 * (c.y - old.y) + c2 * q.dinv.y * (q.rhs.y - Ax1);
  } else {
    const double nx = c.x + q.dinv.x * (q.rhs.x - Ax0), ny = c.y + q.dinv.y * (q.rhs.y - Ax1);
    o.x = first_is_swept ? nx : c.x;
    o.y = first_is_swept ? c.y : ny;
  }
  return o;
}

constexpr int kPairMaxBoxes = 1024;
template <int V, int NW, bool C32, int SM, bool NARROW, bool INTERP, bool REMOTE = false>
__global__ __launch_bounds__(64 * NW) void cheby_pair_kernel(const hpgmg_hip_level L_in, const PairArgs A_in) {
  static_assert(!(REMOTE && C32) && !(REMOTE && NARROW && INTERP), "the multi-rank variant is built for fp64 coefficients; with narrow boxes the interpolation is not folded in");
  constexpr bool kVC = (V != HPGMG_HIP_7PT_CC);
  constexpr bool kHelm = (V == HPGMG_HIP_7PT_VC_HELMHOLTZ);
  constexpr int NR = NW - 2;
  extern __shared__ p2 pair_lds[];
  p2 (*slabX0)[NW][64] = reinterpret_cast<p2 (*)[NW][64]>(pair_lds);
  p2 (*slabX1)[NW][64] = reinterpret_cast<p2 (*)[NW][64]>(pair_lds + 2 * NW * 64);
  p2 (*slabBJ)[NW][64] = reinterpret_cast<p2 (*)[NW][64]>(pair_lds + 4 * NW * 64);
  __shared__ double *sTabLvl[kPairMaxBoxes];
  __shared__ double *sTabScr[kPairMaxBoxes];
  __shared__ const float *sTabC32[C32 ? kPairMaxBoxes : 1];
  __shared__ double *sTabCrs[INTERP ? kPairMaxBoxes : 1];
  hpgmg_hip_level L = L_in;
  PairArgs A = A_in;
  {
    const int nt = 64 * NW, tid0 = (int)threadIdx.y * 64 + (int)threadIdx.x;
    for (int bx = tid0; bx < L_in.num_boxes; bx += nt) {
      sTabLvl[bx] = L_in.box_base[bx];
      sTabScr[bx] = A_in.scr_base ? A_in.scr_base[bx] : nullptr;
      if (C32) sTabC32[bx] = A_in.c32_base[bx];
      if (INTERP) sTabCrs[bx] = A_in.Lc.box_base[bx];
    }
    L.box_base = sTabLvl; A.scr_base = sTabScr;
    if (C32) A.c32_base = sTabC32;
    if (INTERP) A.Lc.box_base = sTabCrs;
    __syncthreads();
  }

  int logical = xcd_logical_block((int)blockIdx.x, A.per_xcd);
  if (REMOTE && A.order) logical = A.order[logical];
  if (logical >= A.total_blocks) return;
  int t = logical;
  const int ti = t % A.tiles_i; t /= A.tiles_i;
  const int sj = t % A.slabs_j; t /= A.slabs_j;
  const int ck = t;

  const int lane = (int)threadIdx.x, w = uni((int)threadIdx.y);
  const int bd = L.dim, jS = L.jStride, kS = L.kStride;
  const int gi0 = ti * 128, R = sj * NR, K0 = ck * A.KC;
  const int NRs = (R + NR <= A.Dj) ? NR : A.Dj - R;
  const int KCs = (K0 + A.KC <= A.Dk) ? A.KC : A.Dk - K0;
  const int gj = R - 1 + w;
  const int jlo = (REMOTE && A.rem[2]) ? -1 : 0, jhi = (REMOTE && A.rem[3]) ? A.Dj + 1 : A.Dj;
  const int klo = (REMOTE && A.rem[4]) ? -1 : 0, khi = (REMOTE && A.rem[5]) ? A.Dk + 1 : A.Dk;
  auto x0row = [&](int r) { return r >= ((REMOTE && A.rem[2]) ? -2 : 0) && r < ((REMOTE && A.rem[3]) ? A.Dj + 2 : A.Dj); };
  auto x0plane = [&](int g) { return g >= ((REMOTE && A.rem[4]) ? -2 : 0) && g < ((REMOTE && A.rem[5]) ? A.Dk + 2 : A.Dk); };
  const bool row_x1 = (gj >= jlo && gj < jhi && w <= NRs + 1);
  const bool row_out = (w >= 1 && w <= NRs);
  const int lanes_per_box = NARROW ? bd / 2 : 64, hop = NARROW ? lane / lanes_per_box : 0;
  const int bi_ = gi0 / bd, li = NARROW ? 2 * (lane - hop * lanes_per_box) : gi0 - bi_ * bd + 2 * lane;
  LaneShift sh = {0, 0, 0};
  if (NARROW) { sh.lvl = (long long)hop * L.box_stride; sh.scr = (long long)hop * 2 * L.volume; sh.c32 = (long long)hop * C32_COUNT * L.volume; }
  const int gjc = row_x1 ? gj : 0;
  const int nbj_ = A.Dj / bd, nbk_ = A.Dk / bd;
  auto jbox = [&](int r) { return !REMOTE ? r / bd : (r < 0 ? 0 : (r >= A.Dj ? nbj_ - 1 : r / bd)); };
  auto kbox = [&](int g) { return !REMOTE ? g / bd : (g < 0 ? 0 : (g >= A.Dk ? nbk_ - 1 : g / bd)); };
  const int bj_ = jbox(gjc), lj = gjc - bj_ * bd;
  const bool ghost_row = REMOTE && (gjc < 0 || gjc >= A.Dj);
  const int row_off = li + lj * jS;
  const bool left_dom = (gi0 == 0), right_dom = (gi0 + 128 == A.Di);
  const int biL = left_dom ? bi_ : (gi0 - 1) / bd, liL = left_dom ? (REMOTE ? -1 : 0) : (gi0 - 1) - biL * bd;
  const int biR = right_dom ? (gi0 + 127) / bd : (gi0 + 128) / bd, liR = right_dom ? (REMOTE ? bd : 0) : (gi0 + 128) - biR * bd;
  const bool left_ghost = REMOTE && left_dom && A.rem[0], right_ghost = REMOTE && right_dom && A.rem[1];
  const bool far_lo = row_x1 && (w == 0) && x0row(gj - 1);
  const bool far_hi = row_x1 && (w == NRs + 1) && x0row(gj + 1);
  const int gjf = far_lo ? gj - 1 : (far_hi ? gj + 1 : gjc);
  const bool far_deep = REMOTE && (gjf < -1 || gjf > A.Dj);
  const int bjf = jbox(gjf), ljf = gjf - bjf * bd;

  auto box_of = [&](int bi, int bj, int gk) { return uni(bi + A.nbi * (bj + A.nbj * kbox(gk))); };
  auto plane_off = [&](int gk) { return !REMOTE ? (gk % bd) * kS : (gk - kbox(gk) * bd) * kS; };
  auto x0_pair = [&](int box, int l_i, int l_j, int gk) -> p2 {
    p2 v = pld(pair_vec(L, A, A.x0, box) + shift_of(sh, A.x0) + l_i + l_j * jS + plane_off(gk));
    if (INTERP && (!REMOTE || (l_j >= 0 && l_j < bd && gk >= 0 && gk < A.Dk))) {
      const int lk = REMOTE ? gk - kbox(gk) * bd : gk % bd;
      const double c = gld1(vec_origin(A.Lc, NARROW ? box + hop : box, A.coarse_id) + ((l_i >> 1) + (l_j >> 1) * A.Lc.jStride + (lk >> 1) * A.Lc.kStride));
      v.x = A.prescale * v.x + c; v.y = A.prescale * v.y + c;
    }
    return v;
  };
  auto x0_one = [&](int box, int l_i, int l_j, int gk) -> double {
    double v = gld1(pair_vec(L, A, A.x0, box) + (l_i + l_j * jS + plane_off(gk)));
    if (INTERP && (!REMOTE || (l_i >= 0 && l_i < bd && l_j >= 0 && l_j < bd && gk >= 0 && gk < A.Dk))) {
      const int lk = REMOTE ? gk - kbox(gk) * bd : gk % bd;
      v = A.prescale * v + gld1(vec_origin(A.Lc, box, A.coarse_id) + ((l_i >> 1) + (l_j >> 1) * A.Lc.jStride + (lk >> 1) * A.Lc.kStride));
    }
    return v;
  };
  auto x0_row = [&](int bj, int l_j, int gk) -> p2 {
    if (REMOTE && (gk < -1 || gk > A.Dk)) {
      if (l_j < 0 || l_j >= bd) return p2{0, 0};
      const int box = box_of(bi_, bj, gk) + hop;
      return pld(A.deep + (((size_t)box * 6 + (gk < 0 ? 4 : 5)) * bd + l_j) * bd + li);
    }
    return x0_pair(box_of(bi_, bj, gk), li, l_j, gk);
  };
  auto far_row = [&](int gk) -> p2 {
    if (REMOTE && far_deep) {
      if (gk < 0 || gk >= A.Dk) return p2{0, 0};
      const int box = box_of(bi_, bjf, gk) + hop;
      return pld(A.deep + (((size_t)box * 6 + (gjf < 0 ? 2 : 3)) * bd + (gk - kbox(gk) * bd)) * bd + li);
    }
    return REMOTE ? x0_row(bjf, ljf, gk) : x0_pair(box_of(bi_, bjf, gk), li, ljf, gk);
  };

  const int P0 = K0 - 1, P1 = K0 + KCs;
  auto in_dom = [&](int gk) { return gk >= klo && gk < khi; };

  p2 x0m = {0, 0}, x0c = {0, 0}, x0p = {0, 0};
  p2 x1m2 = {0, 0}, x1m1 = {0, 0}, x1c = {0, 0};
  p2 far_c = {0, 0}, far_n = {0, 0};
  p2 bj_c = {0, 0}, bj_n = {0, 0};
  PlaneCoef<V> qc = {}, qp = {};

  const int pstart = in_dom(P0) ? P0 : P0 + 1;
  if (row_x1) {
    const int box = box_of(bi_, bj_, pstart), off = row_off + plane_off(pstart);
    x0c = REMOTE ? x0_row(bj_, lj, pstart) : x0_pair(box, li, lj, pstart);
    if (kVC) bj_c = CoefStream<C32>(L, A, box, VECTOR_BETA_J, C32_BETA_J, sh).pair(off);
    if (x0plane(pstart - 1)) x0m = REMOTE ? x0_row(bj_, lj, pstart - 1) : x0_pair(box_of(bi_, bj_, pstart - 1), li, lj, pstart - 1);
    if (far_lo || far_hi) far_c = far_row(pstart);
    slabX0[pstart & 1][w][lane] = x0c;
    slabBJ[pstart & 1][w][lane] = bj_c;
  }
  __syncthreads();

#ifdef HPGMG_EXP_TIMELINE
  unsigned long long *tl = (unsigned long long *)A.deep;
  const bool probe = !REMOTE && tl && logical == 0 && w == 1 && lane == 0;
  int tl_n = 0;
#define TL_MARK() do { if (probe && tl_n < 4000) tl[tl_n++] = __builtin_amdgcn_s_memrealtime(); } while (0)
#else
#define TL_MARK() do { } while (0)
#endif
  for (int p = pstart; p <= P1 && p < khi; p++) {
    const int box = box_of(bi_, bj_, p), off = row_off + plane_off(p);
    TL_MARK();
    const bool have_next = in_dom(p + 1) && (p + 1 <= P1);
    const bool above_in = x0plane(p + 1);
    const bool ghost_plane = REMOTE && (p < 0 || p >= A.Dk);
    if (row_x1) {
      if (above_in) {
        const int bn = box_of(bi_, bj_, p + 1), offn = row_off + plane_off(p + 1);
        x0p = REMOTE ? x0_row(bj_, lj, p + 1) : x0_pair(bn, li, lj, p + 1);
        if (have_next) {
          if (kVC) bj_n = CoefStream<C32>(L, A, bn, VECTOR_BETA_J, C32_BETA_J, sh).pair(offn);
          if (far_lo || far_hi) far_n = far_row(p + 1);
        }
      }
      qc.rhs = pld(vec_origin(L, box, A.rhs_id) + sh.lvl + off);
      qc.dinv = CoefStream<C32>(L, A, box, VECTOR_DINV, C32_DINV, sh).pair(off);
      if (kHelm) qc.al = CoefStream<C32>(L, A, box, VECTOR_ALPHA, C32_ALPHA, sh).pair(off);
      if (kVC) {
        const CoefStream<C32> bis(L, A, box, VECTOR_BETA_I, C32_BETA_I, sh), bks(L, A, box, VECTOR_BETA_K, C32_BETA_K, sh);
        qc.bi = bis.pair(off);
        qc.bir = __shfl_down(qc.bi.x, 1, 64);
        if (lane == 63) qc.bir = bis.one(off + 2);
        if (p == pstart || (p % bd) == 0) qc.bk0 = bks.pair(off); else qc.bk0 = qp.bk1;
        if (REMOTE && p >= A.Dk) qc.bk1 = ghost_row ? p2{0, 0} : pld(A.deep_beta + (((size_t)(box + hop) * 3 + 2) * bd + lj) * bd + li);
        else qc.bk1 = bks.pair(off + kS);
        qc.bjlo = bj_c;
        if (REMOTE && gj >= A.Dj) qc.bjhi = ghost_plane ? p2{0, 0} : pld(A.deep_beta + (((size_t)(box + hop) * 3 + 1) * bd + (p - kbox(p) * bd)) * bd + li);
        else if (w == NRs + 1 || gj + 1 >= jhi || ((lj + 1) == bd)) qc.bjhi = CoefStream<C32>(L, A, box, VECTOR_BETA_J, C32_BETA_J, sh).pair(off + jS);
        else qc.bjhi = slabBJ[p & 1][w + 1][lane];
      }
      p2 xm1 = x0c;
      if (SM == PAIR_CHEBY && A.c1a != 0.0) xm1 = pld(pair_vec(L, A, A.xm1, box) + shift_of(sh, A.xm1) + off);
#ifdef HPGMG_EXP_TIMELINE
      if (probe) { asm volatile("s_waitcnt vmcnt(0)" ::: "memory"); }
      TL_MARK();
#endif

      p2 jm, jp;
      if (!x0row(gj - 1)) jm = pneg(x0c); else if (w == 0) jm = far_c; else jm = slabX0[p & 1][w - 1][lane];
      if (!x0row(gj + 1)) jp = pneg(x0c); else if (w == NRs + 1) jp = far_c; else jp = slabX0[p & 1][w + 1][lane];
      const p2 km = x0plane(p - 1) ? x0m : pneg(x0c);
      const p2 kp = above_in ? x0p : pneg(x0c);
      double left = __shfl_up(x0c.y, 1, 64), right = __shfl_down(x0c.x, 1, 64);
      if (lane == 0)  left  = (left_dom && !left_ghost)   ? -x0c.x : x0_one(box_of(biL, bj_, p), liL, lj, p);
      if (lane == 63) right = (right_dom && !right_ghost) ? -x0c.y : x0_one(box_of(biR, bj_, p), liR, lj, p);
      if (!(ghost_row && ghost_plane))
        x1c = pair_update<V, SM>(x0c, left, right, jm, jp, km, kp, xm1, qc, A.a, A.b, A.h2inv, A.c1a, A.c2a, ((gj ^ p ^ A.sweep_a) & 1) == 0);
    }
#ifdef HPGMG_EXP_TIMELINE
    if (probe) { asm volatile("" :: "v"(x1c.x)); }
    TL_MARK();
#endif

    const int q = p - 1;
    if (row_out && q >= K0) {
      const int boxq = box_of(bi_, bj_, q), offq = row_off + plane_off(q);
      p2 jm, jp;
      if (gj - 1 < jlo) jm = pneg(x1m1); else jm = slabX1[q & 1][w - 1][lane];
      if (gj + 1 >= jhi) jp = pneg(x1m1); else jp = slabX1[q & 1][w + 1][lane];
      const p2 km = in_dom(q - 1) ? x1m2 : pneg(x1m1);
      const p2 kp = x1c;
      double left = __shfl_up(x1m1.y, 1, 64), right = __shfl_down(x1m1.x, 1, 64);
      if (lane == 0)  left  = (left_dom && !left_ghost)   ? -x1m1.x : gld1(pair_vec(L, A, A.out1, box_of(biL, bj_, q)) + (liL + lj * jS + plane_off(q)));
      if (lane == 63) right = (right_dom && !right_ghost) ? -x1m1.y : gld1(pair_vec(L, A, A.out1, box_of(biR, bj_, q)) + (liR + lj * jS + plane_off(q)));
      const p2 x2 = pair_update<V, SM>(x1m1, left, right, jm, jp, km, kp, x0m, qp, A.a, A.b, A.h2inv, A.c1b, A.c2b, ((gj ^ q ^ (A.sweep_a + 1)) & 1) == 0);
      pst(pair_vec(L, A, A.out2, boxq) + shift_of(sh, A.out2) + offq, x2);
    }
    if (SM == PAIR_CHEBY && A.keep_x1 && row_out && p >= K0 && p < K0 + KCs) pst(pair_vec(L, A, A.out1, box) + shift_of(sh, A.out1) + off, x1c);

    TL_MARK();
    if (row_x1) {
      slabX1[p & 1][w][lane] = x1c;
      if (have_next) { slabX0[(p + 1) & 1][w][lane] = x0p; slabBJ[(p + 1) & 1][w][lane] = bj_n; }
    }
    __syncthreads();
    TL_MARK();
    x0m = x0c; x0c = x0p; x1m2 = x1m1; x1m1 = x1c; far_c = far_n; bj_c = bj_n; qp = qc;
  }
#ifdef HPGMG_EXP_TIMELINE
  if (probe) tl[4095] = (unsigned long long)tl_n;
#endif
#undef TL_MARK

  if (P1 >= khi && row_out) {
    const int q = A.Dk - 1;
    if (q >= K0) {
      const int boxq = box_of(bi_, bj_, q), offq = row_off + plane_off(q);
      p2 jm, jp;
      if (gj - 1 < jlo) jm = pneg(x1m1); else jm = slabX1[q & 1][w - 1][lane];
      if (gj + 1 >= jhi) jp = pneg(x1m1); else jp = slabX1[q & 1][w + 1][lane];
      const p2 km = in_dom(q - 1) ? x1m2 : pneg(x1m1);
      const p2 kp = pneg(x1m1);
      double left = __shfl_up(x1m1.y, 1, 64), right = __shfl_down(x1m1.x, 1, 64);
      if (lane == 0)  left  = (left_dom && !left_ghost)   ? -x1m1.x : gld1(pair_vec(L, A, A.out1, box_of(biL, bj_, q)) + (liL + lj * jS + plane_off(q)));
      if (lane == 63) right = (right_dom && !right_ghost) ? -x1m1.y : gld1(pair_vec(L, A, A.out1, box_of(biR, bj_, q)) + (liR + lj * jS + plane_off(q)));
      const p2 x2 = pair_update<V, SM>(x1m1, left, right, jm, jp, km, kp, x0m, qp, A.a, A.b, A.h2inv, A.c1b, A.c2b, ((gj ^ q ^ (A.sweep_a + 1)) & 1) == 0);
      pst(pair_vec(L, A, A.out2, boxq) + shift_of(sh, A.out2) + offq, x2);
    }
  }
}

template <int V, bool C32, int SM, bool INTERP, bool REMOTE = false, bool PACK = false>
__global__ __launch_bounds__(256) void cheby_pair_edge_kernel(const hpgmg_hip_level L, const PairArgs A) {
  constexpr bool kVC = (V != HPGMG_HIP_7PT_CC);
  constexpr bool kHelm = (V == HPGMG_HIP_7PT_VC_HELMHOLTZ);
  const int logical = xcd_logical_block((int)blockIdx.x, A.edge_per_xcd);
  if (logical >= A.edge_blocks) return;
  const int jblocks = (A.Dj + 63) / 64;
  const int gj = (logical % jblocks) * 64 + (int)threadIdx.x, gk = (logical / jblocks) % A.Dk, col = logical / (jblocks * A.Dk);
  if (gj >= A.Dj) return;
  const int ncol_in = 2 * (A.tiles_i - 1);
  int gi;
  if (col < ncol_in) gi = 128 * (col / 2 + 1) - 1 + (col & 1);
  else if (REMOTE) { const int which = (col - ncol_in == 0 && A.rem[0]) ? 0 : 1; gi = which ? A.Di : -1; }
  else return;
  const int bd = L.dim, jS = L.jStride, kS = L.kStride;
  const int nbi_ = A.Di / bd, nbj_ = A.Dj / bd, nbk_ = A.Dk / bd;
  auto clampbox = [&](int c, int D, int nb) { return !REMOTE ? c / bd : (c < 0 ? 0 : (c >= D ? nb - 1 : c / bd)); };
  auto cell = [&](int ci, int cj, int ck, int &box) -> int {
    const int bi = clampbox(ci, A.Di, nbi_), bj = clampbox(cj, A.Dj, nbj_), bk = clampbox(ck, A.Dk, nbk_);
    box = bi + A.nbi * (bj + A.nbj * bk);
    return (ci - bi * bd) + (cj - bj * bd) * jS + (ck - bk * bd) * kS;
  };
  auto x0_at = [&](int ci, int cj, int ck, double centre) -> double {
    if (!REMOTE) { if (ci < 0 || cj < 0 || ck < 0 || ci >= A.Di || cj >= A.Dj || ck >= A.Dk) return -centre; }
    else {
      if ((ci < 0 && !A.rem[0]) || (ci >= A.Di && !A.rem[1]) || (cj < 0 && !A.rem[2]) || (cj >= A.Dj && !A.rem[3]) || (ck < 0 && !A.rem[4]) || (ck >= A.Dk && !A.rem[5])) return -centre;
      if (ci < -1 || ci > A.Di) {
        const int bj = cj / bd, bk = ck / bd, box = ((ci < 0) ? 0 : nbi_ - 1) + A.nbi * (bj + A.nbj * bk);
        return A.deep[(((size_t)box * 6 + (ci < 0 ? 0 : 1)) * bd + (ck - bk * bd)) * bd + (cj - bj * bd)];
      }
    }
    int box; const int idx = cell(ci, cj, ck, box);
    double v = gld1(pair_vec(L, A, A.x0, box) + idx);
    if (INTERP && (!REMOTE || (ci >= 0 && ci < A.Di && cj >= 0 && cj < A.Dj && ck >= 0 && ck < A.Dk)))
      v = A.prescale * v + gld1(vec_origin(A.Lc, box, A.coarse_id) + (((ci % bd) >> 1) + ((cj % bd) >> 1) * A.Lc.jStride + ((ck % bd) >> 1) * A.Lc.kStride));
    return v;
  };
  int box; const int idx = cell(gi, gj, gk, box);
  double bi0 = 0, bi1 = 0, bj0 = 0, bj1 = 0, bk0 = 0, bk1 = 0, al = 0, dinv = 0;
  const bool packed = !PACK && !REMOTE && !C32 && kVC && A.edge_coef != nullptr;
  double *const pk = (!REMOTE && !C32 && kVC && A.edge_coef) ? A.edge_coef + ((size_t)(col * A.Dk + gk) * A.Dj + gj) * 8 : nullptr;
  if (packed) {
    const d2v v0 = *(gd2cptr)as_global(pk), v1 = *(gd2cptr)as_global(pk + 2), v2 = *(gd2cptr)as_global(pk + 4), v3 = *(gd2cptr)as_global(pk + 6);
    bi0 = v0.x; bi1 = v0.y; bj0 = v1.x; bj1 = v1.y; bk0 = v2.x; bk1 = v2.y; al = v3.x; dinv = v3.y;
  }
  const double xc = PACK ? 0.0 : x0_at(gi, gj, gk, 0.0);
  if (kVC && !packed) {
    const CoefStream<C32> bi(L, A, box, VECTOR_BETA_I, C32_BETA_I), bj(L, A, box, VECTOR_BETA_J, C32_BETA_J), bk(L, A, box, VECTOR_BETA_K, C32_BETA_K);
    bi0 = bi.one(idx); bj0 = bj.one(idx); bj1 = bj.one(idx + jS); bk0 = bk.one(idx); bk1 = bk.one(idx + kS);
    if (REMOTE && gi >= A.Di) bi1 = A.deep_beta[(((size_t)box * 3 + 0) * bd + (gk % bd)) * bd + (gj % bd)];
    else bi1 = bi.one(idx + 1);
  }
  if (kHelm && !packed) al = CoefStream<C32>(L, A, box, VECTOR_ALPHA, C32_ALPHA).one(idx);
  if (!packed) dinv = CoefStream<C32>(L, A, box, VECTOR_DINV, C32_DINV).one(idx);
  if (PACK) {
    if (pk) { pk[0] = bi0; pk[1] = bi1; pk[2] = bj0; pk[3] = bj1; pk[4] = bk0; pk[5] = bk1; pk[6] = al; pk[7] = dinv; }
    return;
  }
  const double Ax = apply_op_7pt<V>(xc, x0_at(gi - 1, gj, gk, xc), x0_at(gi + 1, gj, gk, xc), x0_at(gi, gj - 1, gk, xc), x0_at(gi, gj + 1, gk, xc),
                                    x0_at(gi, gj, gk - 1, xc), x0_at(gi, gj, gk + 1, xc), bi0, bi1, bj0, bj1, bk0, bk1, al, A.a, A.b, A.h2inv);
  const double rhs = vec_origin(L, box, A.rhs_id)[idx];
  if (SM == PAIR_CHEBY) {
    const double xnm1 = (A.c1a != 0.0) ? pair_vec(L, A, A.xm1, box)[idx] : xc;
    pair_vec(L, A, A.out1, box)[idx] = xc + A.c1a * (xc - xnm1) + A.c2a * dinv * (rhs - Ax);
  } else {
    pair_vec(L, A, A.out1, box)[idx] = (((gi ^ gj ^ gk ^ A.sweep_a) & 1) == 0) ? xc + dinv * (rhs - Ax) : xc;
  }
}

__global__ __launch_bounds__(256) void coef32_convert_kernel(const hpgmg_hip_level L, float *const *c32_base, int num_vectors) {
  const int box = blockIdx.y;
  const int ids[C32_COUNT] = { VECTOR_DINV, VECTOR_ALPHA, VECTOR_BETA_I, VECTOR_BETA_J, VECTOR_BETA_K };
  const long long n = (long long)C32_COUNT * L.volume;
  for (long long t = (long long)blockIdx.x * blockDim.x + threadIdx.x; t < n; t += (long long)gridDim.x * blockDim.x) {
    const int slot = (int)(t / L.volume), idx = (int)(t - (long long)slot * L.volume);
    if (ids[slot] < num_vectors)
      c32_base[box][(size_t)slot * (size_t)L.volume + idx] = (float)L.box_base[box][(size_t)ids[slot] * (size_t)L.volume + idx];
  }
}

}
```

### hpgmg_amd/csrc/kernels/pair.hip

```cpp
#include "stencil_direct.hpp"
#include "cheby_pair.hpp"

namespace hpgmg {
struct HaloRefs { VecRef x0, xm1; int rhs_id; double *const *scr_base; int fold; hpgmg_hip_level Lc; int coarse_id; double prescale; };
__device__ __forceinline__ double *halo_vec(const hpgmg_hip_level &L, const HaloRefs &R, int vec, int box) {
  const size_t first = (size_t)L.ghosts * (size_t)(1 + L.jStride + L.kStride);
  if (vec >= 16) return L.box_base[box] + (size_t)(vec - 16) * (size_t)L.volume + first;
  if (vec == 2) return L.box_base[box] + (size_t)R.rhs_id * (size_t)L.volume + first;
  const VecRef r = (vec == 0) ? R.x0 : R.xm1;
  return (r.scratch ? R.scr_base[box] : L.box_base[box]) + (size_t)r.id * (size_t)L.volume + first;
}
template <bool kUnpack>
__global__ __launch_bounds__(256) void pair_halo_kernel(const hpgmg_hip_level L, const HaloRefs R, const hpgmg_hip_halo_entry *__restrict__ list,
                                                        double *buf, double *deep, double *deep_beta) {
  const hpgmg_hip_halo_entry e = list[blockIdx.x];
  const int n = e.ni * e.nj * e.nk, jS = L.jStride, kS = L.kStride;
  double *v = halo_vec(L, R, e.vec, e.box) + e.i + e.j * jS + e.k * kS;
  double *b = buf + e.off;
  double *plane = nullptr;
  if (kUnpack && e.deep >= 8) plane = deep_beta + ((size_t)e.box * 3 + (e.deep - 8)) * (size_t)L.dim * L.dim;
  else if (kUnpack && e.deep >= 0) plane = deep + ((size_t)e.box * 6 + e.deep) * (size_t)L.dim * L.dim;
  for (int t = blockIdx.y * 256 + threadIdx.x; t < n; t += gridDim.y * 256) {
    const int ti = t % e.ni, tj = (t / e.ni) % e.nj, tk = t / (e.ni * e.nj);
    if (!kUnpack) {
      double val = v[ti + tj * jS + tk * kS];
      if (R.fold && e.vec == 0) {
        const int ci = e.i + ti, cj = e.j + tj, ck = e.k + tk;
        val = R.prescale * val + vec_origin(R.Lc, e.box, R.coarse_id)[(ci >> 1) + (cj >> 1) * R.Lc.jStride + (ck >> 1) * R.Lc.kStride];
      }
      b[t] = val;
    }
    else if (plane) plane[t] = b[t];
    else v[ti + tj * jS + tk * kS] = b[t];
  }
}
#ifdef HPGMG_EXP_TIMELINE
double *g_exp_timeline = nullptr;
#endif
}
using namespace hpgmg;

extern "C" {
int hpgmg_hip_graph_flush(void);

static int pair_supported_dims(const hpgmg_hip_level *L, int variant, int Di, int Dj, int Dk) {
  if (variant != HPGMG_HIP_7PT_VC_HELMHOLTZ && variant != HPGMG_HIP_7PT_VC_POISSON && variant != HPGMG_HIP_7PT_CC) return 0;
  if (L->num_boxes <= 0 || L->num_boxes > kPairMaxBoxes || L->periodic || !(L->flags & 1) || L->ghosts < 1 || Di % 128 != 0) return 0;
  if (L->dim % 128 != 0 && !(128 % L->dim == 0 && L->dim >= 16 && (L->box_stride > 0 || L->num_boxes == 1))) return 0;
  if (L->jStride % 2 || L->kStride % 2 || L->volume % 2) return 0;
  if (Di % L->dim || Dj % L->dim || Dk % L->dim) return 0;
  if ((long long)(Di / L->dim) * (Dj / L->dim) * (Dk / L->dim) != L->num_boxes) return 0;
  return 1;
}
int hpgmg_hip_smooth_cheby_pair_supported(const hpgmg_hip_level *L, int variant) { return pair_supported_dims(L, variant, L->dim_i, L->dim_j, L->dim_k); }
int hpgmg_hip_smooth_cheby_pair_supported_brick(const hpgmg_hip_level *L, int variant, int nbi, int nbj, int nbk) {
  return pair_supported_dims(L, variant, nbi * L->dim, nbj * L->dim, nbk * L->dim);
}
int hpgmg_hip_coef32_refresh(const hpgmg_hip_level *L, float *const *c32_base, int num_vectors) {
  HPGMG_SKIP_IF_REPLAY();
  if (L->num_boxes <= 0) return 0;
  hipLaunchKernelGGL(coef32_convert_kernel, dim3(512, L->num_boxes), dim3(256), 0, g_stream, *L, c32_base, num_vectors);
  HPGMG_LAUNCH_CHECK("coef32_convert_kernel");
  return 0;
}
static bool g_pair_halo_set = false;
static int g_pair_rem[6], g_pair_brick[3];
static const double *g_pair_deep = nullptr, *g_pair_deep_beta = nullptr;
static long long g_pair_launches = 0, g_pair_remote_launches = 0;
static int g_pair_discard_x1 = 0;
static const hpgmg_hip_level *g_pair_interp_level = nullptr;
static int g_pair_interp_id = 0;
static double g_pair_interp_prescale = 1.0;
struct EdgePack { const void *key; int variant, Di, Dj, Dk; double *buf; bool valid; };
static std::vector<EdgePack> g_edge_packs;
extern "C" void hpgmg_hip_pair_packed_invalidate(const hpgmg_hip_level *L) { for (EdgePack &e : g_edge_packs) if (!L || e.key == (const void *)L->box_base) e.valid = false; }
extern "C" void hpgmg_hip_pair_packed_forget(const hpgmg_hip_level *L) {
  for (size_t q = 0; q < g_edge_packs.size();) {
    if (!L || g_edge_packs[q].key == (const void *)L->box_base) { (void)hipStreamSynchronize(g_stream); (void)hipFree(g_edge_packs[q].buf); g_edge_packs.erase(g_edge_packs.begin() + (long)q); }
    else q++;
  }
}
static EdgePack *edge_pack_slot(const hpgmg_hip_level *L, int variant, const PairArgs &A) {
  static const int on = env_int("HPGMG_TUNE_PAIR_PACKED", 1);
  if (!on || A.tiles_i < 2 || variant == HPGMG_HIP_7PT_CC) return nullptr;
  for (EdgePack &e : g_edge_packs) if (e.key == (const void *)L->box_base && e.variant == variant && e.Di == A.Di && e.Dj == A.Dj && e.Dk == A.Dk) return &e;
  EdgePack e = { (const void *)L->box_base, variant, A.Di, A.Dj, A.Dk, nullptr, false };
  const size_t n = (size_t)2 * (A.tiles_i - 1) * A.Dk * A.Dj * 8;
  if (hipMalloc((void **)&e.buf, n * sizeof(double)) != hipSuccess) return nullptr;
  g_edge_packs.push_back(e);
  return &g_edge_packs.back();
}
struct PairOrder { int ti, sj, ck, rem[6], part; int *d_order; int grid, per_xcd, count; };
static std::vector<PairOrder> g_pair_orders;
static const PairOrder *pair_part_order(const PairArgs &A, int part) {
  for (const PairOrder &o : g_pair_orders)
    if (o.ti == A.tiles_i && o.sj == A.slabs_j && o.ck == A.chunks_k && o.part == part && memcmp(o.rem, A.rem, sizeof o.rem) == 0) return &o;
  PairOrder o = {}; o.ti = A.tiles_i; o.sj = A.slabs_j; o.ck = A.chunks_k; o.part = part; memcpy(o.rem, A.rem, sizeof o.rem);
  std::vector<int> sel;
  for (int l = 0; l < A.total_blocks; l++) {
    int t = l;
    const int ti = t % A.tiles_i; t /= A.tiles_i;
    const int sj = t % A.slabs_j; t /= A.slabs_j;
    const int ck = t;
    const bool later = (ti == 0 && A.rem[0]) || (ti == A.tiles_i - 1 && A.rem[1]) || (sj == 0 && A.rem[2]) || (sj == A.slabs_j - 1 && A.rem[3]) || (ck == 0 && A.rem[4]) || (ck == A.chunks_k - 1 && A.rem[5]);
    if (later == (part == 2)) sel.push_back(l);
  }
  o.count = (int)sel.size();
  if (o.count > 0) {
    o.per_xcd = (o.count + kXcds - 1) / kXcds; o.grid = o.per_xcd * kXcds;
    sel.resize((size_t)o.grid, A.total_blocks);
    if (hipMalloc((void **)&o.d_order, sel.size() * sizeof(int)) != hipSuccess) return nullptr;
    if (hipMemcpy(o.d_order, sel.data(), sel.size() * sizeof(int), hipMemcpyHostToDevice) != hipSuccess) { (void)hipFree(o.d_order); return nullptr; }
  }
  g_pair_orders.push_back(o);
  return &g_pair_orders.back();
}
static int smooth_pair(const hpgmg_hip_level *L, int variant, int gsrb, int sweep_a, double *const *scr_base, const float *const *c32_base,
                       int x0_scr, int x0_id, int xm1_scr, int xm1_id, int out1_scr, int out1_id, int out2_scr, int out2_id,
                       int rhs_id, double a, double b, double h2inv, double c1a, double c2a, double c1b, double c2b) {
  const bool remote = g_pair_halo_set;
  const int discard_x1 = g_pair_discard_x1;
  const hpgmg_hip_level *const interp_level = g_pair_interp_level;
  g_pair_halo_set = false; g_pair_discard_x1 = 0; g_pair_interp_level = nullptr;
  HPGMG_SKIP_IF_REPLAY();
  const int Di = remote ? g_pair_brick[0] * L->dim : L->dim_i, Dj = remote ? g_pair_brick[1] * L->dim : L->dim_j, Dk = remote ? g_pair_brick[2] * L->dim : L->dim_k;
  if (!pair_supported_dims(L, variant, Di, Dj, Dk)) return record_error(hipErrorInvalidValue, "smooth_cheby_pair: level not supported");
  if (remote && c32_base) return record_error(hipErrorInvalidValue, "smooth_cheby_pair: remote faces need fp64 coefficients");
  static const int tune_kc = env_int("HPGMG_TUNE_PAIR_KC", 0);
  static const int tune_nw = env_int("HPGMG_TUNE_PAIR_NW", 0);
  int nw = 16, kc = tune_kc;
  {
    const int slots = 256, cand[3] = {10, 12, 16}, step_cost[3] = {46, 51, 75};
    long long best_cost = -1;
    for (int ci = 0; ci < 3; ci++) {
      const int w = cand[ci];
      if (tune_nw > 0 && w != tune_nw) continue;
      if (tune_nw <= 0 && c32_base && w == 10) continue;
      const int per_plane = (Di / 128) * ((Dj + (w - 2) - 1) / (w - 2));
      auto steps = [&](int c) { const long long wgs = (long long)per_plane * ((Dk + c - 1) / c); return ((wgs + slots - 1) / slots) * (c + 2); };
      int k = tune_kc;
      if (k <= 0) {
        long long best = -1;
        for (int c = 8; c <= 64 && c <= Dk; c++) { const long long cost = steps(c); if (best < 0 || cost < best) { best = cost; k = c; } }
        for (int c = k + 1; c <= 64 && c <= Dk; c++) if (steps(c) * 100 <= best * 103) k = c;
      }
      const long long cost = steps(k) * step_cost[ci];
      if (best_cost < 0 || cost < best_cost) { best_cost = cost; nw = w; kc = k; }
    }
  }
  PairArgs A = {};
  A.x0 = VecRef{x0_scr, x0_id}; A.xm1 = VecRef{xm1_scr, xm1_id}; A.out1 = VecRef{out1_scr, out1_id}; A.out2 = VecRef{out2_scr, out2_id};
  A.rhs_id = rhs_id; A.a = a; A.b = b; A.h2inv = h2inv; A.c1a = c1a; A.c2a = c2a; A.c1b = c1b; A.c2b = c2b;
  A.scr_base = scr_base; A.c32_base = c32_base; A.sweep_a = sweep_a;
  A.keep_x1 = discard_x1 ? 0 : 1;
  const bool interp = (interp_level != nullptr);
  if (interp) {
    const hpgmg_hip_level *C = interp_level;
    if ((remote && L->dim % 128 != 0) || C->num_boxes != L->num_boxes || C->num_boxes > kPairMaxBoxes || 2 * C->dim != L->dim) return record_error(hipErrorInvalidValue, "smooth pair with interpolation: level pair not supported");
    A.Lc = *C; A.coarse_id = g_pair_interp_id; A.prescale = g_pair_interp_prescale;
  }
  A.nbi = Di / L->dim; A.nbj = Dj / L->dim;
  A.Di = Di; A.Dj = Dj; A.Dk = Dk;
  if (remote) { for (int d = 0; d < 6; d++) A.rem[d] = g_pair_rem[d]; A.deep = g_pair_deep; A.deep_beta = g_pair_deep_beta; }
#ifdef HPGMG_EXP_TIMELINE
  else A.deep = g_exp_timeline;
#endif
  A.tiles_i = A.Di / 128; A.slabs_j = (A.Dj + (nw - 2) - 1) / (nw - 2); A.KC = kc; A.chunks_k = (A.Dk + kc - 1) / kc;
  A.total_blocks = A.tiles_i * A.slabs_j * A.chunks_k;
  int grid = grid_for(A.total_blocks, &A.per_xcd);
  long long cells = (long long)A.Di * A.Dj * A.Dk;
  const long long whole_cells = cells;
  const int part = remote ? g_tile_part : 0;
  if (part) {
    const PairOrder *o = pair_part_order(A, part);
    if (!o) return record_error(hipErrorOutOfMemory, "smooth pair: dispatch list of a partial launch");
    if (o->count == 0) return 0;
    A.order = o->d_order; grid = o->grid; A.per_xcd = o->per_xcd;
    cells = cells * o->count / A.total_blocks;
  }
  const size_t lds = (size_t)nw * 6 * 64 * sizeof(p2);
  if (!remote && !c32_base) {
    EdgePack *pk = edge_pack_slot(L, variant, A);
    if (pk) {
      A.edge_coef = pk->buf;
      if (!pk->valid) {
        A.edge_blocks = ((A.Dj + 63) / 64) * A.Dk * 2 * (A.tiles_i - 1);
        const dim3 pgrid(grid_for(A.edge_blocks, &A.edge_per_xcd));
        if (variant == HPGMG_HIP_7PT_VC_HELMHOLTZ) hipLaunchKernelGGL((cheby_pair_edge_kernel<HPGMG_HIP_7PT_VC_HELMHOLTZ, false, PAIR_CHEBY, false, false, true>), pgrid, dim3(64), 0, g_stream, *L, A);
        else hipLaunchKernelGGL((cheby_pair_edge_kernel<HPGMG_HIP_7PT_VC_POISSON, false, PAIR_CHEBY, false, false, true>), pgrid, dim3(64), 0, g_stream, *L, A);
        HPGMG_LAUNCH_CHECK("cheby_pair_edge_kernel (packing)");
        pk->valid = true;
      }
    }
  }
  const int prof = profile_begin(whole_cells);
#define PAIR_NW_SWITCH(...) switch (nw) { case 10: { constexpr int NWC = 10; __VA_ARGS__ } break; case 12: { constexpr int NWC = 12; __VA_ARGS__ } break; default: { constexpr int NWC = 16; __VA_ARGS__ } break; }
#define PAIR_LAUNCH2(VAR, C32, SM, NARROW, INTERP) PAIR_NW_SWITCH( \
      static bool once = false; if (!once) { HPGMG_CHECK(hipFuncSetAttribute((const void *)cheby_pair_kernel<VAR, NWC, C32, SM, NARROW, INTERP>, hipFuncAttributeMaxDynamicSharedMemorySize, (int)((size_t)NWC * 6 * 64 * sizeof(p2)))); once = true; } \
      hipLaunchKernelGGL((cheby_pair_kernel<VAR, NWC, C32, SM, NARROW, INTERP>), dim3(grid), dim3(64, NWC), lds, g_stream, *L, A); )
#define PAIR_LAUNCH_REMOTE_IP(VAR, SM, NRW, IP) { \
      const int ecols = 2 * (A.tiles_i - 1) + (A.rem[0] ? 1 : 0) + (A.rem[1] ? 1 : 0); \
      A.edge_blocks = ((A.Dj + 63) / 64) * A.Dk * ecols; const int egrid_r = grid_for(A.edge_blocks, &A.edge_per_xcd); \
      if (ecols > 0) hipLaunchKernelGGL((cheby_pair_edge_kernel<VAR, false, SM, IP, true>), dim3(egrid_r), dim3(64), 0, g_stream, *L, A); \
      PAIR_NW_SWITCH( \
      static bool once = false; if (!once) { HPGMG_CHECK(hipFuncSetAttribute((const void *)cheby_pair_kernel<VAR, NWC, false, SM, NRW, IP, true>, hipFuncAttributeMaxDynamicSharedMemorySize, (int)((size_t)NWC * 6 * 64 * sizeof(p2)))); once = true; } \
      hipLaunchKernelGGL((cheby_pair_kernel<VAR, NWC, false, SM, NRW, IP, true>), dim3(grid), dim3(64, NWC), lds, g_stream, *L, A); ) }
#define PAIR_LAUNCH_REMOTE(VAR, SM) { if (L->dim % 128 != 0) PAIR_LAUNCH_REMOTE_IP(VAR, SM, true, false) else if (interp) PAIR_LAUNCH_REMOTE_IP(VAR, SM, false, true) else PAIR_LAUNCH_REMOTE_IP(VAR, SM, false, false) }
#define PAIR_LAUNCH(VAR, C32, SM) { \
      A.edge_blocks = ((A.Dj + 63) / 64) * A.Dk * 2 * (A.tiles_i - 1); const dim3 egrid(A.edge_blocks > 0 ? grid_for(A.edge_blocks, &A.edge_per_xcd) : 1); \
      if (remote) PAIR_LAUNCH_REMOTE(VAR, SM) \
      else if (interp) { \
        if (A.tiles_i > 1) hipLaunchKernelGGL((cheby_pair_edge_kernel<VAR, C32, SM, true>), egrid, dim3(64), 0, g_stream, *L, A); \
        if (L->dim % 128 == 0) PAIR_LAUNCH2(VAR, C32, SM, false, true) else PAIR_LAUNCH2(VAR, C32, SM, true, true) \
      } else { \
        if (A.tiles_i > 1) hipLaunchKernelGGL((cheby_pair_edge_kernel<VAR, C32, SM, false>), egrid, dim3(64), 0, g_stream, *L, A); \
        if (L->dim % 128 == 0) PAIR_LAUNCH2(VAR, C32, SM, false, false) else PAIR_LAUNCH2(VAR, C32, SM, true, false) \
      } }
#define PAIR_CASE(VAR) case VAR: \
    if (gsrb) { if (c32_base) PAIR_LAUNCH(VAR, true, PAIR_GSRB) else PAIR_LAUNCH(VAR, false, PAIR_GSRB) } \
    else      { if (c32_base) PAIR_LAUNCH(VAR, true, PAIR_CHEBY) else PAIR_LAUNCH(VAR, false, PAIR_CHEBY) } break;
  switch (variant) {
    PAIR_CASE(HPGMG_HIP_7PT_VC_HELMHOLTZ)
    PAIR_CASE(HPGMG_HIP_7PT_VC_POISSON)
    PAIR_CASE(HPGMG_HIP_7PT_CC)
    default: return record_error(hipErrorInvalidValue, "smooth_cheby_pair: variant");
  }
#undef PAIR_CASE
#undef PAIR_LAUNCH
#undef PAIR_LAUNCH2
#undef PAIR_NW_SWITCH
#undef PAIR_LAUNCH_REMOTE
#undef PAIR_LAUNCH_REMOTE_IP
  if (part != 1) { g_pair_launches++; if (remote) g_pair_remote_launches++; }
  profile_end(prof, 2 * cells, part == 1);
  HPGMG_LAUNCH_CHECK("cheby_pair_kernel");
  return 0;
}
int hpgmg_hip_smooth_cheby_pair(const hpgmg_hip_level *L, int variant, double *const *scr_base, const float *const *c32_base,
                                int x0_scr, int x0_id, int xm1_scr, int xm1_id, int out1_scr, int out1_id, int out2_scr, int out2_id,
                                int rhs_id, double a, double b, double h2inv, double c1a, double c2a, double c1b, double c2b) {
  return smooth_pair(L, variant, 0, 0, scr_base, c32_base, x0_scr, x0_id, xm1_scr, xm1_id, out1_scr, out1_id, out2_scr, out2_id, rhs_id, a, b, h2inv, c1a, c2a, c1b, c2b);
}
void hpgmg_hip_pair_fold_interpolation(const hpgmg_hip_level *Lc, int coarse_id, double prescale) {
  g_pair_interp_level = Lc; g_pair_interp_id = coarse_id; g_pair_interp_prescale = prescale;
}
void hpgmg_hip_pair_set_halo(const int brick_boxes[3], const int remote_face[6], const double *deep, const double *deep_beta) {
  for (int d = 0; d < 3; d++) g_pair_brick[d] = brick_boxes[d];
  for (int d = 0; d < 6; d++) g_pair_rem[d] = remote_face[d];
  g_pair_deep = deep; g_pair_deep_beta = deep_beta; g_pair_halo_set = true;
}
void hpgmg_hip_pair_discard_x1(void) { g_pair_discard_x1 = 1; }
#ifdef HPGMG_EXP_TIMELINE
void hpgmg_hip_exp_timeline(void *buf) { g_exp_timeline = (double *)buf; }
#endif
void hpgmg_hip_pair_launch_counts(long long out[2]) { out[0] = g_pair_launches; out[1] = g_pair_remote_launches; }

static const hpgmg_hip_level *g_halo_fold_level = nullptr;
static int g_halo_fold_id = 0;
static double g_halo_fold_prescale = 1.0;
static int pair_halo_move(bool unpack, const hpgmg_hip_level *L, double *const *scr_base, int x0_scr, int x0_id, int xm1_scr, int xm1_id, int rhs_id,
                          const hpgmg_hip_halo_entry *entries, int n, double *buf, double *deep, double *deep_beta) {
  const hpgmg_hip_level *fold = unpack ? nullptr : g_halo_fold_level;
  if (!unpack) g_halo_fold_level = nullptr;
  HPGMG_SKIP_IF_REPLAY();
  if (n <= 0) return 0;
  HaloRefs R = {}; R.x0 = VecRef{x0_scr, x0_id}; R.xm1 = VecRef{xm1_scr, xm1_id}; R.rhs_id = rhs_id; R.scr_base = scr_base;
  if (fold) { R.fold = 1; R.Lc = *fold; R.coarse_id = g_halo_fold_id; R.prescale = g_halo_fold_prescale; }
  const int slabs = (L->dim * L->dim + 4095) / 4096;
  if (unpack) hipLaunchKernelGGL((pair_halo_kernel<true>), dim3(n, slabs), dim3(256), 0, g_stream, *L, R, entries, buf, deep, deep_beta);
  else        hipLaunchKernelGGL((pair_halo_kernel<false>), dim3(n, slabs), dim3(256), 0, g_stream, *L, R, entries, buf, deep, deep_beta);
  HPGMG_LAUNCH_CHECK("pair_halo_kernel");
  return 0;
}
void hpgmg_hip_pair_halo_fold_interpolation(const hpgmg_hip_level *Lc, int coarse_id, double prescale) { g_halo_fold_level = Lc; g_halo_fold_id = coarse_id; g_halo_fold_prescale = prescale; }
int hpgmg_hip_pair_halo_pack(const hpgmg_hip_level *L, double *const *scr_base, int x0_scr, int x0_id, int xm1_scr, int xm1_id, int rhs_id,
                             const hpgmg_hip_halo_entry *entries, int n, double *sendbuf) {
  return pair_halo_move(false, L, scr_base, x0_scr, x0_id, xm1_scr, xm1_id, rhs_id, entries, n, sendbuf, nullptr, nullptr);
}
int hpgmg_hip_pair_halo_unpack(const hpgmg_hip_level *L, double *const *scr_base, int x0_scr, int x0_id, int xm1_scr, int xm1_id, int rhs_id,
                               const hpgmg_hip_halo_entry *entries, int n, double *recvbuf, double *deep, double *deep_beta) {
  return pair_halo_move(true, L, scr_base, x0_scr, x0_id, xm1_scr, xm1_id, rhs_id, entries, n, recvbuf, deep, deep_beta);
}

int hpgmg_hip_smooth_gsrb_pair(const hpgmg_hip_level *L, int variant, double *const *scr_base, const float *const *c32_base,
                               int x0_scr, int x0_id, int edge_scr_id, int out2_scr, int out2_id, int rhs_id,
                               double a, double b, double h2inv, int sweep) {
  return smooth_pair(L, variant, 1, sweep, scr_base, c32_base, x0_scr, x0_id, x0_scr, x0_id, 1, edge_scr_id, out2_scr, out2_id, rhs_id, a, b, h2inv, 0.0, 0.0, 0.0, 0.0);
}

}
```

### include/hpgmg_hip.h

```cpp
#ifndef HPGMG_HIP_H
#define HPGMG_HIP_H

#include <stddef.h>
#include "hpgmg_level.h"

#ifdef __cplusplus
extern "C" {
#endif

typedef struct {
  double *const *box_base;
  const int *box_low;
  int num_boxes;
  int dim, ghosts, jStride, kStride, volume;
  int dim_i, dim_j, dim_k;
  int periodic;
  const int *box_nbr;
  int flags;
  long long box_stride;
} hpgmg_hip_level;

enum { HPGMG_HIP_7PT_VC_HELMHOLTZ = 0, HPGMG_HIP_7PT_VC_POISSON = 1, HPGMG_HIP_7PT_CC = 2,
       HPGMG_HIP_27PT_CC = 3, HPGMG_HIP_FV4_VC_HELMHOLTZ = 4, HPGMG_HIP_FV4_VC_POISSON = 5 };

int    hpgmg_hip_device_count(void);
int    hpgmg_hip_set_device(int dev);
void   hpgmg_hip_set_stream(void *hip_stream);
void  *hpgmg_hip_get_stream(void);
int    hpgmg_hip_sync(void);
void  *hpgmg_hip_malloc(size_t bytes);
void   hpgmg_hip_free(void *p);
void  *hpgmg_hip_host_malloc(size_t bytes);
void   hpgmg_hip_host_free(void *p);
int    hpgmg_hip_memcpy_h2d(void *dst, const void *src, size_t bytes);
int    hpgmg_hip_memcpy_d2h(void *dst, const void *src, size_t bytes);
int    hpgmg_hip_memcpy_d2d(void *dst, const void *src, size_t bytes);
int    hpgmg_hip_memset0(void *dst, size_t bytes);
const char *hpgmg_hip_last_error(void);
void  *hpgmg_hip_event_create(void);
void   hpgmg_hip_event_destroy(void *ev);
int    hpgmg_hip_event_record(void *ev);
void  *hpgmg_hip_stream_create(void);
void   hpgmg_hip_stream_destroy(void *stream);
int    hpgmg_hip_stream_wait_event(void *ev);
double hpgmg_hip_event_elapsed_ms(void *start, void *stop);
int    hpgmg_hip_timer_begin(double *acc_seconds);
void   hpgmg_hip_timer_end(int slot);
int    hpgmg_hip_timer_flush(void);
void   hpgmg_hip_timer_forget(const void *lo, const void *hi);
int    hpgmg_hip_range_enabled(void);
void   hpgmg_hip_range_push(const char *name);
void   hpgmg_hip_range_pop(void);
void   hpgmg_hip_profile_smoother(int enable);
void   hpgmg_hip_profile_smoother_min_cells(long long min_cells);
void hpgmg_hip_profile_smoother_stride(int stride);
int    hpgmg_hip_profile_smoother_read(double *total_ms, long long *launches, long long *cells);

void hpgmg_hip_set_ghost_free(int on);
int  hpgmg_hip_get_ghost_free(void);

int  hpgmg_hip_smooth_cheby_fold_supported(const hpgmg_hip_level *L, int variant);
void hpgmg_hip_stencil_fold_interpolation(const hpgmg_hip_level *Lc, int coarse_id, const int *map, int which);
int hpgmg_hip_smooth_cheby(const hpgmg_hip_level *L, int variant, int xn_id, int xnp1_id, int rhs_id,
                           double a, double b, double h2inv, double c1, double c2);
int hpgmg_hip_smooth_gsrb(const hpgmg_hip_level *L, int variant, int xn_id, int xnp1_id, int rhs_id,
                          double a, double b, double h2inv, int sweep);
int hpgmg_hip_smooth_jacobi(const hpgmg_hip_level *L, int variant, int xn_id, int xnp1_id, int rhs_id,
                            double a, double b, double h2inv, double weight);
int hpgmg_hip_residual(const hpgmg_hip_level *L, int variant, int res_id, int x_id, int rhs_id,
                       double a, double b, double h2inv);
int hpgmg_hip_residual_fused_supported(const hpgmg_hip_level *L, int variant);
int  hpgmg_hip_residual_restrict_supported(const hpgmg_hip_level *L, int variant);
int hpgmg_hip_residual_restrict(const hpgmg_hip_level *L, int variant, int x_id, int rhs_id, double a, double b, double h2inv,
                                const hpgmg_hip_level *Lc, int coarse_id, const int *map, int zero_id);
int hpgmg_hip_residual_restrict_store(const hpgmg_hip_level *L, int variant, int res_id, int x_id, int rhs_id, double a, double b, double h2inv,
                                      const hpgmg_hip_level *Lc, int coarse_id, const int *map, int zero_id);
int hpgmg_hip_residual_norm(const hpgmg_hip_level *L, int variant, int res_id, int x_id, int rhs_id, double a, double b, double h2inv, double *norm_out);
int hpgmg_hip_small_level_max_cells(void);
int hpgmg_hip_small_level_op(const hpgmg_hip_level *L, int variant, int mode, int sweeps, int x_id, int rhs_id, int res_id, int out_of_place,
                             double a, double b, double h2inv, const double *c1, const double *c2,
                             const blockCopy_type *copy_list, int n_copy, const blockCopy_type *bc_list, int n_bc, int bc_kind, int zero_first);
int hpgmg_hip_bottom_bicgstab_max_cells(void);
int hpgmg_hip_bottom_bicgstab(const hpgmg_hip_level *L, int variant, int x_id, int rhs_id, int krylov_base, double a, double b, double h2inv, double want,
                              const blockCopy_type *bc_list, int n_bc, int bc_kind, int zero_first, int *krylov_iterations);
int hpgmg_hip_small_ops_max(void);
int hpgmg_hip_small_ops(const hpgmg_hip_level *L, int variant, int n, const int *kinds, const int *c, const int *a, const int *b, const double *sa, const double *sb,
                        const blockCopy_type *bc_list, int n_bc, int bc_kind, int zero_first, double op_a, double op_b, double h2inv, double *value_out, double *value2_out);
long long hpgmg_hip_small_ops_launch_count(void);
#define HPGMG_HIP_SMALL_TAIL_MAX_LEVELS 4
typedef struct {
  hpgmg_hip_level L;
  const blockCopy_type *bc_list, *ibc_list;
  int n_bc, bc_kind, zero_first, n_ibc, ibc_kind, ibc_zero_first;
  double h2inv, c1[8], c2[8];
} hpgmg_hip_small_tail_level;
typedef struct {
  int n, mode, sweeps, out_of_place, e_id, R_id, krylov_base, legs;
  double a, b, want;
  int *krylov_iterations;
  hpgmg_hip_small_tail_level lv[HPGMG_HIP_SMALL_TAIL_MAX_LEVELS];
} hpgmg_hip_small_tail_args;
long long hpgmg_hip_small_vtail_lds_doubles(const hpgmg_hip_small_tail_args *args);
long long hpgmg_hip_small_vtail_lds_limit(void);
int hpgmg_hip_small_vtail(const hpgmg_hip_small_tail_args *args, int variant);
long long hpgmg_hip_small_vtail_launch_count(void);
void hpgmg_hip_set_defer_mode(int mode);
void hpgmg_hip_set_tile_part(int part);
void hpgmg_hip_set_tile_ghost_free(int on);
void hpgmg_hip_set_27pt_tile32(int on);
int  hpgmg_hip_smooth_gsrb27_rb_supported(const hpgmg_hip_level *L);
int  hpgmg_hip_smooth_gsrb27_rb(const hpgmg_hip_level *L, int x_id, int out_id, int rhs_id, double a, double b, double h2inv, int sweep);
int  hpgmg_hip_smooth_gsrb27_rb_box_supported(const hpgmg_hip_level *L);
void hpgmg_hip_set_27pt_rb_box_maxdim(int dim);
int  hpgmg_hip_smooth_gsrb27_rb_box(const hpgmg_hip_level *L, int x_id, int out_id, int rhs_id, double a, double b, double h2inv, int sweep);
long long hpgmg_hip_rb27_launch_count(void);
int  hpgmg_hip_tile_kernel_applies(const hpgmg_hip_level *L, int variant, int out_of_place);

int hpgmg_hip_smooth_cheby_pair_supported(const hpgmg_hip_level *L, int variant);
int hpgmg_hip_smooth_cheby_pair(const hpgmg_hip_level *L, int variant, double *const *scr_base, const float *const *c32_base,
                                int x0_scr, int x0_id, int xm1_scr, int xm1_id, int out1_scr, int out1_id, int out2_scr, int out2_id,
                                int rhs_id, double a, double b, double h2inv, double c1a, double c2a, double c1b, double c2b);
int  hpgmg_hip_smooth_cheby_pair_supported_brick(const hpgmg_hip_level *L, int variant, int nbi, int nbj, int nbk);
void hpgmg_hip_pair_set_halo(const int brick_boxes[3], const int remote_face[6], const double *deep, const double *deep_beta);
void hpgmg_hip_pair_discard_x1(void);
void hpgmg_hip_pair_packed_invalidate(const hpgmg_hip_level *L);
void hpgmg_hip_pair_packed_forget(const hpgmg_hip_level *L);
void hpgmg_hip_pair_launch_counts(long long out[2]);
typedef struct { int box, vec, i, j, k, ni, nj, nk, deep, pad_; long long off; } hpgmg_hip_halo_entry;
void hpgmg_hip_pair_halo_fold_interpolation(const hpgmg_hip_level *Lc, int coarse_id, double prescale);
int  hpgmg_hip_pair_halo_pack(const hpgmg_hip_level *L, double *const *scr_base, int x0_scr, int x0_id, int xm1_scr, int xm1_id, int rhs_id,
                              const hpgmg_hip_halo_entry *entries, int n, double *sendbuf);
int  hpgmg_hip_pair_halo_unpack(const hpgmg_hip_level *L, double *const *scr_base, int x0_scr, int x0_id, int xm1_scr, int xm1_id, int rhs_id,
                                const hpgmg_hip_halo_entry *entries, int n, double *recvbuf, double *deep, double *deep_beta);
int hpgmg_hip_smooth_gsrb_pair(const hpgmg_hip_level *L, int variant, double *const *scr_base, const float *const *c32_base,
                               int x0_scr, int x0_id, int edge_scr_id, int out2_scr, int out2_id, int rhs_id,
                               double a, double b, double h2inv, int sweep);
void hpgmg_hip_pair_fold_interpolation(const hpgmg_hip_level *Lc, int coarse_id, double prescale);
int hpgmg_hip_coef32_refresh(const hpgmg_hip_level *L, float *const *c32_base, int num_vectors );

int hpgmg_hip_copy_blocks(const hpgmg_hip_level *L, int id, const blockCopy_type *blocks, int num_blocks);
int hpgmg_hip_increment_blocks(const hpgmg_hip_level *L, int id, double prescale, const blockCopy_type *blocks, int num_blocks);
int hpgmg_hip_apply_bc_p1(const hpgmg_hip_level *L, int id, const blockCopy_type *blocks, int num_blocks);
int hpgmg_hip_apply_bc_p2(const hpgmg_hip_level *L, int id, const blockCopy_type *blocks, int num_blocks);
int hpgmg_hip_apply_bc_v2(const hpgmg_hip_level *L, int id, const blockCopy_type *blocks, int num_blocks);
int hpgmg_hip_apply_bc_v4(const hpgmg_hip_level *L, int id, const blockCopy_type *blocks, int num_blocks);
int hpgmg_hip_extrapolate_betas(const hpgmg_hip_level *L, const blockCopy_type *blocks, int num_blocks);
typedef struct { int box, nn, base, len0, len1, fs0, fs1, step[3], src_box, src_base;
                 int zbase, zi, zj, zk;
} hpgmg_hip_bc_entry;
int hpgmg_hip_apply_bc_fv(const hpgmg_hip_level *L, int id, const hpgmg_hip_bc_entry *entries, int num_entries, int order);
int hpgmg_hip_exchange_and_bc(const hpgmg_hip_level *L, int id, const blockCopy_type *copies, int num_copies,
                              const hpgmg_hip_bc_entry *entries, int num_entries, int order);

int  hpgmg_hip_smooth_gsrb_fv4_rb_supported(const hpgmg_hip_level *L, int variant);
int  hpgmg_hip_fv4_rb_prepass(const hpgmg_hip_level *L, int variant, double *const *scr_base, int x_scratch, int x_id, int tg_id, int rhs_id,
                              double a, double b, double h2inv, int sweep, const hpgmg_hip_bc_entry *entries_k, int n_k,
                              const int *special_cells , int n_special);
int  hpgmg_hip_smooth_gsrb_fv4_rb(const hpgmg_hip_level *L, int variant, double *const *scr_base, int x_scratch, int x_id, int out_scratch, int out_id,
                                  int tg_id, int rhs_id, double a, double b, double h2inv, int sweep);
long long hpgmg_hip_rb_fv4_launch_count(void);
int hpgmg_hip_restrict_blocks(const hpgmg_hip_level *Lc, int id_c, const hpgmg_hip_level *Lf, int id_f,
                              const blockCopy_type *blocks, int num_blocks, int type);
int hpgmg_hip_restrict_cell_and_zero(const hpgmg_hip_level *Lc, int id_c, const hpgmg_hip_level *Lf, int id_f,
                                     const blockCopy_type *blocks, int num_blocks, int zero_id);
int hpgmg_hip_interpolate_blocks(const hpgmg_hip_level *Lf, int id_f, double prescale, const hpgmg_hip_level *Lc, int id_c,
                                 const blockCopy_type *blocks, int num_blocks, int order);

int hpgmg_hip_fill(const hpgmg_hip_level *L, int id, double interior_value);
int hpgmg_hip_axpby(const hpgmg_hip_level *L, int id_c, double sa, int id_a, double sb, int id_b);
int hpgmg_hip_mul(const hpgmg_hip_level *L, int id_c, double s, int id_a, int id_b);
int hpgmg_hip_invert(const hpgmg_hip_level *L, int id_c, double s, int id_a);
int hpgmg_hip_scale(const hpgmg_hip_level *L, int id_c, double s, int id_a);
int hpgmg_hip_shift(const hpgmg_hip_level *L, int id_c, int id_a, double shift);
int hpgmg_hip_color(const hpgmg_hip_level *L, int id, int colors, int ic, int jc, int kc);
int hpgmg_hip_random(const hpgmg_hip_level *L, int id);
int hpgmg_hip_norm_max(const hpgmg_hip_level *L, int id, double *out);
int hpgmg_hip_dot(const hpgmg_hip_level *L, int id_a, int id_b, double *out);
int hpgmg_hip_norm_copy_restrict(const hpgmg_hip_level *L, int f_id, int r_id, const hpgmg_hip_level *Lc, int rc_id, const int *map, double *norm_out);
int  hpgmg_hip_norm_copy_restrict_deferred(const hpgmg_hip_level *L, int f_id, int r_id, const hpgmg_hip_level *Lc, int rc_id, const int *restrict_map);
int  hpgmg_hip_deferred_fetch(double *out);
int hpgmg_hip_sum(const hpgmg_hip_level *L, int id, double *out);
int hpgmg_hip_gram(const hpgmg_hip_level *L, const int *id_A, int rows, const int *id_B, int cols, double *C_host);
int hpgmg_hip_pcg_supported(const hpgmg_hip_level *L, int variant);
int hpgmg_hip_pcg_apply_dot(const hpgmg_hip_level *L, int variant, int Ap_id, int p_id, double a, double b, double h2inv, double *dot);
int hpgmg_hip_pcg_update(const hpgmg_hip_level *L, int x_id, int r_id, int p_id, int Ap_id, double alpha, double *rmax);
int hpgmg_hip_pcg_dot(const hpgmg_hip_level *L, int a_id, int b_id, double *dot);
int hpgmg_hip_pcg_dot2(const hpgmg_hip_level *L, int a_id, int c_id, int b_id, double *ab, double *cb);

int hpgmg_hip_dense_pack(const hpgmg_hip_level *L, int id, const double *src, int ni, int nj, int nk, int check, int *status);
int hpgmg_hip_dense_unpack(const hpgmg_hip_level *L, int id, double *dst);
int hpgmg_hip_dense_pack_lifted(const hpgmg_hip_level *L, int id, const double *src, const double *g, double w, int *status);
int hpgmg_hip_boundary_flux(const hpgmg_hip_level *L, double *phi, const double *g, double w, int *status);
int hpgmg_hip_boundary_restrict(double *g_c, const double *g_f, int n_c);
int hpgmg_hip_boundary_lift(const hpgmg_hip_level *L, int id, const double *phi, const double *phi_fine, double sign);
int hpgmg_hip_boundary_interp(const hpgmg_hip_level *L, int id, const double *g_c, int n_c);
int hpgmg_hip_dense_pack_walls(const hpgmg_hip_level *L, int id, const double *src, int axis, int check, int mask, double *wall, int *status);
int hpgmg_hip_dense_pack_lifted_faces(const hpgmg_hip_level *L, int id, const double *src, const double *g, double w, int mask, const double *wall,
                                      double wn, int *status);
int hpgmg_hip_boundary_flux_faces(const hpgmg_hip_level *L, double *phi, const double *g, double w, int mask, const double *wall, double wn, int *status);
int hpgmg_hip_boundary_interp_faces(const hpgmg_hip_level *L, int id, const hpgmg_hip_level *Lc, int boxes_per_side, const double *g_c, double h_c, int mask);
int hpgmg_hip_boundary_check_kappa(const double *kappa, int n, int robin_mask, int *status);
int hpgmg_hip_boundary_store_walls(const hpgmg_hip_level *L, const double *wall, const double *kappa, double h, int mask);
int hpgmg_hip_dense_pack_lifted_robin(const hpgmg_hip_level *L, int id, const double *src, const double *g, double w, int mask, const double *wall,
                                      double wn, const double *kappa, double h, int *status);
int hpgmg_hip_boundary_flux_robin(const hpgmg_hip_level *L, double *phi, const double *g, double w, int mask, const double *wall, double wn,
                                  const double *kappa, double h, int *status);
int hpgmg_hip_boundary_interp_robin(const hpgmg_hip_level *L, int id, const hpgmg_hip_level *Lc, int boxes_per_side, const double *g_c, double h_c, int mask,
                                    const double *kappa_c);
int hpgmg_hip_dense_unpack_flux(const hpgmg_hip_level *L, int id, const double *g, double b, double wq, double h, int mask, const double *wall,
                                const double *kappa, double *flux_i, double *flux_j, double *flux_k, int *status);

int hpgmg_hip_blackbox_accumulate(const hpgmg_hip_level *L, int variant, int x_id, int Aii_id, int sumAbs_id, double a, double b, double h2inv);
int hpgmg_hip_blackbox_finalize(const hpgmg_hip_level *L, int Aii_id, int sumAbs_id, double a, double b, double h2inv, double *lambda_max_out);

int hpgmg_hip_rebuild_7pt(const hpgmg_hip_level *L, int variable_coeff, int alpha_id, int l1inv_id,
                          double a, double b, double h2inv, double *lambda_max_out);

int hpgmg_hip_tail_max_levels(void);
int hpgmg_hip_tail_max_cells(void);
int hpgmg_hip_tail_bottom_max_cells(void);
int hpgmg_hip_vcycle_tail(int n, const hpgmg_hip_level *const *levels, const double *h2inv,
                          const double *c1, const double *c2, int sweeps,
                          int variant, int smoother, int e_id, int R_id, double a, double b, int leg,
                          int krylov_base, double bottom_norm, int *krylov_iterations);

typedef struct { hpgmg_hip_level L; double h2inv, c1[8], c2[8]; } hpgmg_hip_brick_level;
int hpgmg_hip_brick_visit_supported(const hpgmg_hip_level *L, int brick);
int hpgmg_hip_brick_visit_max_sweeps(void);
int hpgmg_hip_brick_chain_max_levels(void);
int hpgmg_hip_brick_chain(int n, const hpgmg_hip_brick_level *levels, const hpgmg_hip_level *below, int sweeps, int variant, int smoother,
                          int e_id, int R_id, double a, double b, int dir, int brick, int top_e_zero, int below_zero);
int hpgmg_hip_brick_wide_supported(const hpgmg_hip_level *L, int variant);
int hpgmg_hip_brick_wide_capacity(int variant, int smoother);
int hpgmg_hip_brick_wide_chain(int n, const hpgmg_hip_brick_level *levels, const hpgmg_hip_level *below, int sweeps, int variant, int smoother,
                               int e_id, int R_id, double a, double b, int dir, int top_e_zero, int below_zero);
long long hpgmg_hip_brick_visits(void);
int hpgmg_hip_brick_visit_error(void);
int hpgmg_hip_brick_visit_error_clear(void);
int hpgmg_hip_brick_chain_capacity(int variant, int smoother, int brick);

void hpgmg_hip_graph_enable(int on);
int  hpgmg_hip_graph_enabled(void);
int  hpgmg_hip_graph_begin(long long key);
int  hpgmg_hip_graph_end(void);
int  hpgmg_hip_graph_is_open(void);
int  hpgmg_hip_graph_flush(void);
void hpgmg_hip_graph_reset(void);
void hpgmg_hip_graph_stats(long long out[3]);

int  hpgmg_hip_rccl_unique_id(char *out128);
int  hpgmg_hip_rccl_init(const char *id128, int rank, int size);
void hpgmg_hip_rccl_finalize(void);
void hpgmg_hip_rccl_sendrecv(void *ctx, int nrecv, double *const *rbuf, const int *rsize, const int *rrank,
                             int nsend, double *const *sbuf, const int *ssize, const int *srank, int tag);
void hpgmg_hip_rccl_allreduce(void *ctx, double *vals, int n, int op, const int *ranks, int nranks);
void hpgmg_hip_rccl_prepare_subset(void *ctx, const int *ranks, int nranks);
long long hpgmg_hip_rccl_subset_collectives(void);
long long hpgmg_hip_rccl_subset_alltoalls(void);
int  hpgmg_hip_rccl_allreduce_max_world(double *vals, int n);
int  hpgmg_hip_rccl_allreduce_ordered_world(double *vals, int n, int op);
long long hpgmg_hip_rccl_allgather_count(void);

int  hpgmg_hip_ipc_init(const char *name, int rank, int size);
void hpgmg_hip_ipc_finalize(void);
void hpgmg_hip_ipc_sendrecv(void *ctx, int nrecv, double *const *rbuf, const int *rsize, const int *rrank,
                            int nsend, double *const *sbuf, const int *ssize, const int *srank, int tag);
void hpgmg_hip_ipc_allreduce(void *ctx, double *vals, int n, int op, const int *ranks, int nranks);
long long hpgmg_hip_ipc_message_count(void);

#ifdef __cplusplus
}
#endif
#endif
```

Baseline: 6.366 billion.

## Form tile-edge x1 values inline in the 7-pt sweep-pair kernel, dropping the prepass

Adds an EDGE_INLINE variant of the Chebyshev/GSRB sweep-pair kernel, used by default for the 10- and 12-wave shapes. In it the halo waves load the neighbouring column's inputs into LDS and compute the first-sweep x1 values on the cells just outside each interior 128-cell tile edge. Previously a separate edge-kernel launch ran ahead of every pair, so this removes a launch and its global write/read round-trip. In exchange the halo waves do extra loads and wave barriers and the kernel uses more shared memory, which could lengthen the critical path or lower occupancy. An env switch restores the prepass.

```diff
diff --git a/hpgmg_amd/__init__.py b/hpgmg_amd/__init__.py
--- a/hpgmg_amd/__init__.py
+++ b/hpgmg_amd/__init__.py
@@ -190,6 +190,8 @@
         "hpgmg_hip_gram": (c_int, [L, P(c_int), c_int, P(c_int), c_int, P(c_dbl)]),
         "hpgmg_hip_pcg_dot2": (c_int, [L, c_int, c_int, c_int, P(c_dbl), P(c_dbl)]),
         "hpgmg_hip_pair_launch_counts": (None, [P(ctypes.c_longlong)]),
+        "hpgmg_hip_pair_prepass_launches": (ctypes.c_longlong, []),
+        "hpgmg_hip_pair_set_edge_inline": (None, [ctypes.c_int]),
     }
     for name, (res, args) in sig.items():
         fn = getattr(lib, name)
diff --git a/hpgmg_amd/csrc/host/plugin_internal.h b/hpgmg_amd/csrc/host/plugin_internal.h
--- a/hpgmg_amd/csrc/host/plugin_internal.h
+++ b/hpgmg_amd/csrc/host/plugin_internal.h
@@ -92,7 +92,7 @@
 
 typedef enum { SW_GHOST_FREE = 0, SW_ONE_LAUNCH_GHOSTS, SW_OVERLAP, SW_PAIR_REMOTE, SW_IMAGES, SW_FUSED_SWEEPS, SW_PAIR_MIN_CELLS, SW_FUSED_RESIDUAL, SW_FUSED_TAIL,
                SW_FUSED_FTAIL, SW_FUSED_BOTTOM, SW_SMALL_FUSED, SW_SMALL_VTAIL, SW_SMALL_27PT_GSRB, SW_SMALL_OPS, SW_LAZY, SW_LAZY_REPORT, SW_TEMP_SCRATCH,
-               SW_FV4_NO_EXACT_RB, SW_GRAPH, SW_SMOOTHER_PRECISION, SW_DEFER_NORM, SW_BRICK_VISITS, SW_BRICK_SIZE, SW_BRICK_MIN_DIM, SW_BRICK_FSTEP, SW_BRICK_CHAIN, SW_BRICK_WIDE, SW_BRICK_WIDE_MAX_DIM, SW_BRICK_WIDE_TAIL_DIM, SW_FTAIL_MAX_DIM, SW_COUNT } hp_switch_id;
+               SW_FV4_NO_EXACT_RB, SW_GRAPH, SW_SMOOTHER_PRECISION, SW_DEFER_NORM, SW_BRICK_VISITS, SW_BRICK_SIZE, SW_BRICK_MIN_DIM, SW_BRICK_FSTEP, SW_BRICK_CHAIN, SW_BRICK_WIDE, SW_BRICK_WIDE_MAX_DIM, SW_BRICK_WIDE_TAIL_DIM, SW_FTAIL_MAX_DIM, SW_PAIR_EDGE, SW_COUNT } hp_switch_id;
 HP_INTERNAL long long hp_switch(hp_switch_id id);
 HP_INTERNAL void hp_switch_set(hp_switch_id id, long long value);
 
diff --git a/hpgmg_amd/csrc/host/plugin_smooth.c b/hpgmg_amd/csrc/host/plugin_smooth.c
--- a/hpgmg_amd/csrc/host/plugin_smooth.c
+++ b/hpgmg_amd/csrc/host/plugin_smooth.c
@@ -329,6 +329,7 @@
   }
   hp_ensure_pair_scratch(L, B);
   hpgmg_hip_set_ghost_free(1);
+  hpgmg_hip_pair_set_edge_inline((int)hp_switch(SW_PAIR_EDGE));
   return 1;
 }
 
diff --git a/hpgmg_amd/csrc/host/plugin_switches.c b/hpgmg_amd/csrc/host/plugin_switches.c
--- a/hpgmg_amd/csrc/host/plugin_switches.c
+++ b/hpgmg_amd/csrc/host/plugin_switches.c
@@ -1,6 +1,6 @@
 #include "plugin_internal.h"
 
-enum { K_ON = 0, K_OFF = 1, K_INT = 2, K_TRI = 3 };
+enum { K_ON = 0, K_OFF = 1, K_INT = 2, K_TRI = 3, K_EDGE = 4 };
 static struct { const char *env; int kind; long long dflt; const char *what; long long value; int known; } table[SW_COUNT] = {
   [SW_GHOST_FREE]        = { "HPGMG_GHOST_FREE", K_ON, 1, "stencil launches read neighbouring boxes and the Dirichlet rule themselves; 0: the reference's exchange + boundary + stencil launches" },
   [SW_ONE_LAUNCH_GHOSTS] = { "HPGMG_ONE_LAUNCH_GHOSTS", K_ON, 1, "27-pt / fv2 / fv4: box-to-box ghost copies and boundary conditions as one launch" },
@@ -32,6 +32,7 @@
   [SW_BRICK_WIDE_MAX_DIM] = { "HPGMG_TUNE_BRICK_WIDE_MAX", K_INT, 64, "largest level (cells per side) the 27-pt / fv4 plugins visit as bricks (measured: fv4 `7 64` 29.71 / 29.91 / 30.15 ms with 64 / 32 / 16, 27-pt 12.27 / 12.51 / 12.52)" },
   [SW_BRICK_WIDE_TAIL_DIM] = { "HPGMG_TUNE_BRICK_WIDE_TAIL", K_INT, 1, "27-pt / fv4: the largest one-box level left to the single-workgroup tail (1: the 8^3, 4^3 (and 27-pt: 2^3) levels are visited as ONE brick each and only the bottom solve is left; 2 / 4 / 8: the tail starts there)" },
   [SW_FTAIL_MAX_DIM]    = { "HPGMG_TUNE_FTAIL_MAX", K_INT, 8, "7-pt: the largest level (cells per side) the single-launch F-cycle tail starts from (8: the 16^3 step of the climb is a brick launch each way, eight CUs instead of one: config 1 0.320 vs 0.328 ms with 16, config 2 the same within noise; profiles/r06i_ab_ftail.txt)" },
+  [SW_PAIR_EDGE]        = { "HPGMG_TUNE_PAIR_EDGE", K_EDGE, 1, "7-pt sweep pairs, x1 on the cell columns outside interior 128-cell tile edges: inline (1, default) = formed by the halo waves of the 10- and 12-wave kernels themselves; prepass (0) = by a launch of its own ahead of every pair, as the 16-wave, fp32-coefficient and multi-rank launches always do" },
   [SW_SMOOTHER_PRECISION]= { "HPGMG_SMOOTHER_PRECISION", K_INT, 64, "32: fp32 coefficient streams in the Chebyshev sweep pairs (BASELINE config 5: within 2e-4 of the fp64 norms, and bit-exact against the CPU oracle's fp32 mode, which rounds the same coefficients); 64: bit-exact" },
 };
 
@@ -43,6 +44,7 @@
       case K_ON:  v = !(e && e[0] == '0'); break;
       case K_OFF: v = (e && e[0] == '1'); break;
       case K_INT: if (e && *e) v = atoll(e); break;
+      case K_EDGE: v = !(e && strcmp(e, "prepass") == 0); break;
       default:    v = (e && e[0] == '0') ? 0 : ((e && e[0] == '1') ? 1 : table[id].dflt); break;
     }
     table[id].value = v; table[id].known = 1;
diff --git a/hpgmg_amd/csrc/kernels/cheby_pair.hpp b/hpgmg_amd/csrc/kernels/cheby_pair.hpp
--- a/hpgmg_amd/csrc/kernels/cheby_pair.hpp
+++ b/hpgmg_amd/csrc/kernels/cheby_pair.hpp
@@ -77,13 +77,24 @@
   return o;
 }
 
+template <int V, int SM>
+__device__ __forceinline__ double edge_cell_x1(double xc, double xl, double xr, double xjm, double xjp, double xkm, double xkp,
+                                               double bi0, double bi1, double bj0, double bj1, double bk0, double bk1, double al, double dinv,
+                                               double rhs, double xnm1, const PairArgs &A, bool swept) {
+  const double Ax = apply_op_7pt<V>(xc, xl, xr, xjm, xjp, xkm, xkp, bi0, bi1, bj0, bj1, bk0, bk1, al, A.a, A.b, A.h2inv);
+  if (SM == PAIR_CHEBY) return xc + A.c1a * (xc - xnm1) + A.c2a * dinv * (rhs - Ax);
+  return swept ? xc + dinv * (rhs - Ax) : xc;
+}
+
 constexpr int kPairMaxBoxes = 1024;
-template <int V, int NW, bool C32, int SM, bool NARROW, bool INTERP, bool REMOTE = false>
+template <int V, int NW, bool C32, int SM, bool NARROW, bool INTERP, bool REMOTE = false, bool EDGE_INLINE = false>
 __global__ __launch_bounds__(64 * NW) void cheby_pair_kernel(const hpgmg_hip_level L_in, const PairArgs A_in) {
   static_assert(!(REMOTE && C32) && !(REMOTE && NARROW && INTERP), "the multi-rank variant is built for fp64 coefficients; with narrow boxes the interpolation is not folded in");
+  static_assert(!(EDGE_INLINE && (REMOTE || C32 || NW > 12)), "remote faces, fp32 coefficient streams and the 16-wave shape keep the pre-pass");
   constexpr bool kVC = (V != HPGMG_HIP_7PT_CC);
   constexpr bool kHelm = (V == HPGMG_HIP_7PT_VC_HELMHOLTZ);
   constexpr int NR = NW - 2;
+  constexpr bool kEdgeEarly = EDGE_INLINE && !(NARROW && (INTERP || kHelm));
   extern __shared__ p2 pair_lds[];
   p2 (*slabX0)[NW][64] = reinterpret_cast<p2 (*)[NW][64]>(pair_lds);
   p2 (*slabX1)[NW][64] = reinterpret_cast<p2 (*)[NW][64]>(pair_lds + 2 * NW * 64);
@@ -92,6 +103,9 @@
   __shared__ double *sTabScr[kPairMaxBoxes];
   __shared__ const float *sTabC32[C32 ? kPairMaxBoxes : 1];
   __shared__ double *sTabCrs[INTERP ? kPairMaxBoxes : 1];
+  __shared__ double edgeX1[2][NW][2];
+  __shared__ double edgeIn[2][NW][12];
+  __shared__ double edgeX0[2][3][NW];
   hpgmg_hip_level L = L_in;
   PairArgs A = A_in;
   {
@@ -194,7 +208,67 @@
   p2 bj_c = {0, 0}, bj_n = {0, 0};
   PlaneCoef<V> qc = {}, qp = {};
 
+  const bool edge_left = EDGE_INLINE && w == 0 && !left_dom, edge_right = EDGE_INLINE && w == NRs + 1 && !right_dom;
+  const bool edge_wave = edge_left || edge_right;
+  const int es = edge_left ? 0 : 1;
+  const int e_bi = edge_left ? biL : biR, e_li = edge_left ? liL : liR, e_lfar = edge_left ? liL - 1 : liR + 1, e_gi = edge_left ? gi0 - 1 : gi0 + 128;
+  const int e_col = edge_left ? 2 * (ti - 1) : 2 * ti + 1;
+  const int e_bj0 = uni((R > 0 ? R - 1 : 0) / bd);
+  struct EdgeLane { int er, ev, gj, lj, boxrow, rowoff; bool row, out; };
+  auto hold = [](int v) { asm volatile("" : "+v"(v)); return v; };
+  auto e_lane = [&]() {
+    EdgeLane E; const int ln = hold(lane);
+    E.er = ln >> 2; E.ev = ln & 3; E.gj = R - 1 + E.er;
+    E.row = edge_wave && E.er <= NRs + 1 && E.gj >= 0 && E.gj < A.Dj;
+    E.out = E.row && E.er >= 1 && E.er <= NRs;
+    const int gjc = E.row ? E.gj : 0, bj = e_bj0 + (gjc >= (e_bj0 + 1) * bd ? 1 : 0);
+    E.lj = gjc - bj * bd; E.boxrow = e_bi + A.nbi * bj; E.rowoff = E.lj * jS;
+    return E;
+  };
+  auto e_box = [&](const EdgeLane &E, int gk) { return E.boxrow + A.nbi * A.nbj * (gk / bd); };
+  auto e_coarse = [&](const EdgeLane &E, int ebx, int l_i, int gk) { return gld1(vec_origin(A.Lc, ebx, A.coarse_id) + ((l_i >> 1) + (E.lj >> 1) * A.Lc.jStride + ((gk % bd) >> 1) * A.Lc.kStride)); };
+  auto e_wanted = [&](int pe) { return pe >= K0 && pe < K0 + KCs; };
+  d2v e_ra = {0, 0}; double e_rb = 0, e_rc = 0;
+  auto e_request = [&](int pe) {
+    e_ra = d2v{0, 0}; e_rb = 0; e_rc = 0;
+    const EdgeLane E = e_lane(); const int ev = E.ev;
+    if (!E.row) return;
+    const bool cell = E.out && e_wanted(pe);
+    const int gk = (ev == 3) ? pe + 1 : pe, l_i = (ev == 0) ? e_lfar : e_li;
+    const bool single = (ev == 3) ? (x0plane(pe + 1) && pe + 1 <= P1) : (cell && (ev != 2 || (SM == PAIR_CHEBY && A.c1a != 0.0)));
+    if (single) {
+      const int ebx = e_box(E, gk), idx = l_i + E.rowoff + plane_off(gk);
+      const double *ptr = (ev == 1) ? vec_origin(L, ebx, A.rhs_id) : ((ev == 2) ? pair_vec(L, A, A.xm1, ebx) : pair_vec(L, A, A.x0, ebx));
+      e_rb = gld1(ptr + idx);
+      if (INTERP && (ev == 0 || ev == 3)) e_rc = e_coarse(E, ebx, l_i, gk);
+    }
+    if (!cell) return;
+    if (kVC && A.edge_coef) {
+      e_ra = *(gd2cptr)as_global(A.edge_coef + (((size_t)(e_col * A.Dk + pe) * A.Dj + E.gj) * 8 + 2 * ev));
+    } else {
+      const int ebx = e_box(E, pe), idx = e_li + E.rowoff + plane_off(pe);
+      if (kVC && ev < 3) {
+        const CoefStream<false> beta(L, A, ebx, ev == 0 ? VECTOR_BETA_I : (ev == 1 ? VECTOR_BETA_J : VECTOR_BETA_K), 0);
+        e_ra.x = beta.one(idx); e_ra.y = beta.one(idx + (ev == 0 ? 1 : (ev == 1 ? jS : kS)));
+      }
+      if (ev == 3) {
+        if (kHelm) e_ra.x = CoefStream<false>(L, A, ebx, VECTOR_ALPHA, C32_ALPHA).one(idx);
+        e_ra.y = CoefStream<false>(L, A, ebx, VECTOR_DINV, C32_DINV).one(idx);
+      }
+    }
+  };
+
   const int pstart = in_dom(P0) ? P0 : P0 + 1;
+  if (EDGE_INLINE && edge_wave) {
+    const EdgeLane E = e_lane(); const int ev = E.ev;
+    if (E.row && (ev == 3 || (ev == 2 && x0plane(pstart - 1)))) {
+      const int gk = (ev == 3) ? pstart : pstart - 1, ebx = e_box(E, gk);
+      double v = gld1(pair_vec(L, A, A.x0, ebx) + (e_li + E.rowoff + plane_off(gk)));
+      if (INTERP) v = A.prescale * v + e_coarse(E, ebx, e_li, gk);
+      edgeX0[es][gk % 3][E.er] = v;
+    }
+    e_request(pstart);
+  }
   if (row_x1) {
     const int box = box_of(bi_, bj_, pstart), off = row_off + plane_off(pstart);
     x0c = REMOTE ? x0_row(bj_, lj, pstart) : x0_pair(box, li, lj, pstart);
@@ -220,6 +294,7 @@
     const bool have_next = in_dom(p + 1) && (p + 1 <= P1);
     const bool above_in = x0plane(p + 1);
     const bool ghost_plane = REMOTE && (p < 0 || p >= A.Dk);
+    p2 xm1 = {0, 0};
     if (row_x1) {
       if (above_in) {
         const int bn = box_of(bi_, bj_, p + 1), offn = row_off + plane_off(p + 1);
@@ -245,8 +320,37 @@
         else if (w == NRs + 1 || gj + 1 >= jhi || ((lj + 1) == bd)) qc.bjhi = CoefStream<C32>(L, A, box, VECTOR_BETA_J, C32_BETA_J, sh).pair(off + jS);
         else qc.bjhi = slabBJ[p & 1][w + 1][lane];
       }
-      p2 xm1 = x0c;
+      xm1 = x0c;
       if (SM == PAIR_CHEBY && A.c1a != 0.0) xm1 = pld(pair_vec(L, A, A.xm1, box) + shift_of(sh, A.xm1) + off);
+    }
+    auto e_form_request = [&](const EdgeLane &E) {
+      const int er = E.er;
+      __builtin_amdgcn_fence(__ATOMIC_RELEASE, "wavefront"); __builtin_amdgcn_wave_barrier(); __builtin_amdgcn_fence(__ATOMIC_ACQUIRE, "wavefront");
+      const int e_gj = E.gj;
+      if (E.out && E.ev == 0 && e_wanted(p)) {
+        const double *in = edgeIn[es][er], *xcol = edgeX0[es][p % 3];
+        const double xc = xcol[er], far = in[8];
+        const double near = edge_left ? slabX0[p & 1][er][0].x : slabX0[p & 1][er][63].y;
+        const double x1e = edge_cell_x1<V, SM>(xc, edge_left ? far : near, edge_left ? near : far,
+                                               e_gj - 1 < 0 ? -xc : xcol[er - 1], e_gj + 1 >= A.Dj ? -xc : xcol[er + 1],
+                                               x0plane(p - 1) ? edgeX0[es][(p - 1) % 3][er] : -xc, above_in ? edgeX0[es][(p + 1) % 3][er] : -xc,
+                                               in[0], in[1], in[2], in[3], in[4], in[5], in[6], in[7], in[9], (SM == PAIR_CHEBY && A.c1a != 0.0) ? in[10] : xc,
+                                               A, ((e_gi ^ e_gj ^ p ^ A.sweep_a) & 1) == 0);
+        edgeX1[p & 1][er][es] = x1e;
+      }
+      if (p + 1 <= P1) e_request(p + 1);
+    };
+    if (EDGE_INLINE && edge_wave) {
+      const EdgeLane E = e_lane(); const int er = E.er, ev = E.ev;
+      if (E.row) {
+        const double rb = (INTERP && (ev == 0 || ev == 3)) ? A.prescale * e_rb + e_rc : e_rb;
+        if (ev != 3) edgeIn[es][er][8 + ev] = rb;
+        else if (above_in && p + 1 <= P1) edgeX0[es][(p + 1) % 3][er] = rb;
+        edgeIn[es][er][2 * ev] = e_ra.x; edgeIn[es][er][2 * ev + 1] = e_ra.y;
+      }
+      if (kEdgeEarly) e_form_request(E);
+    }
+    if (row_x1) {
 #ifdef HPGMG_EXP_TIMELINE
       if (probe) { asm volatile("s_waitcnt vmcnt(0)" ::: "memory"); }
       TL_MARK();
@@ -277,14 +381,15 @@
       const p2 km = in_dom(q - 1) ? x1m2 : pneg(x1m1);
       const p2 kp = x1c;
       double left = __shfl_up(x1m1.y, 1, 64), right = __shfl_down(x1m1.x, 1, 64);
-      if (lane == 0)  left  = (left_dom && !left_ghost)   ? -x1m1.x : gld1(pair_vec(L, A, A.out1, box_of(biL, bj_, q)) + (liL + lj * jS + plane_off(q)));
-      if (lane == 63) right = (right_dom && !right_ghost) ? -x1m1.y : gld1(pair_vec(L, A, A.out1, box_of(biR, bj_, q)) + (liR + lj * jS + plane_off(q)));
+      if (lane == 0)  left  = (left_dom && !left_ghost)   ? -x1m1.x : (EDGE_INLINE ? edgeX1[q & 1][w][0] : gld1(pair_vec(L, A, A.out1, box_of(biL, bj_, q)) + (liL + lj * jS + plane_off(q))));
+      if (lane == 63) right = (right_dom && !right_ghost) ? -x1m1.y : (EDGE_INLINE ? edgeX1[q & 1][w][1] : gld1(pair_vec(L, A, A.out1, box_of(biR, bj_, q)) + (liR + lj * jS + plane_off(q))));
       const p2 x2 = pair_update<V, SM>(x1m1, left, right, jm, jp, km, kp, x0m, qp, A.a, A.b, A.h2inv, A.c1b, A.c2b, ((gj ^ q ^ (A.sweep_a + 1)) & 1) == 0);
       pst(pair_vec(L, A, A.out2, boxq) + shift_of(sh, A.out2) + offq, x2);
     }
     if (SM == PAIR_CHEBY && A.keep_x1 && row_out && p >= K0 && p < K0 + KCs) pst(pair_vec(L, A, A.out1, box) + shift_of(sh, A.out1) + off, x1c);
 
     TL_MARK();
+    if (EDGE_INLINE && !kEdgeEarly && edge_wave) e_form_request(e_lane());
     if (row_x1) {
       slabX1[p & 1][w][lane] = x1c;
       if (have_next) { slabX0[(p + 1) & 1][w][lane] = x0p; slabBJ[(p + 1) & 1][w][lane] = bj_n; }
@@ -308,8 +413,8 @@
       const p2 km = in_dom(q - 1) ? x1m2 : pneg(x1m1);
       const p2 kp = pneg(x1m1);
       double left = __shfl_up(x1m1.y, 1, 64), right = __shfl_down(x1m1.x, 1, 64);
-      if (lane == 0)  left  = (left_dom && !left_ghost)   ? -x1m1.x : gld1(pair_vec(L, A, A.out1, box_of(biL, bj_, q)) + (liL + lj * jS + plane_off(q)));
-      if (lane == 63) right = (right_dom && !right_ghost) ? -x1m1.y : gld1(pair_vec(L, A, A.out1, box_of(biR, bj_, q)) + (liR + lj * jS + plane_off(q)));
+      if (lane == 0)  left  = (left_dom && !left_ghost)   ? -x1m1.x : (EDGE_INLINE ? edgeX1[q & 1][w][0] : gld1(pair_vec(L, A, A.out1, box_of(biL, bj_, q)) + (liL + lj * jS + plane_off(q))));
+      if (lane == 63) right = (right_dom && !right_ghost) ? -x1m1.y : (EDGE_INLINE ? edgeX1[q & 1][w][1] : gld1(pair_vec(L, A, A.out1, box_of(biR, bj_, q)) + (liR + lj * jS + plane_off(q))));
       const p2 x2 = pair_update<V, SM>(x1m1, left, right, jm, jp, km, kp, x0m, qp, A.a, A.b, A.h2inv, A.c1b, A.c2b, ((gj ^ q ^ (A.sweep_a + 1)) & 1) == 0);
       pst(pair_vec(L, A, A.out2, boxq) + shift_of(sh, A.out2) + offq, x2);
     }
@@ -374,15 +479,11 @@
     if (pk) { pk[0] = bi0; pk[1] = bi1; pk[2] = bj0; pk[3] = bj1; pk[4] = bk0; pk[5] = bk1; pk[6] = al; pk[7] = dinv; }
     return;
   }
-  const double Ax = apply_op_7pt<V>(xc, x0_at(gi - 1, gj, gk, xc), x0_at(gi + 1, gj, gk, xc), x0_at(gi, gj - 1, gk, xc), x0_at(gi, gj + 1, gk, xc),
-                                    x0_at(gi, gj, gk - 1, xc), x0_at(gi, gj, gk + 1, xc), bi0, bi1, bj0, bj1, bk0, bk1, al, A.a, A.b, A.h2inv);
   const double rhs = vec_origin(L, box, A.rhs_id)[idx];
-  if (SM == PAIR_CHEBY) {
-    const double xnm1 = (A.c1a != 0.0) ? pair_vec(L, A, A.xm1, box)[idx] : xc;
-    pair_vec(L, A, A.out1, box)[idx] = xc + A.c1a * (xc - xnm1) + A.c2a * dinv * (rhs - Ax);
-  } else {
-    pair_vec(L, A, A.out1, box)[idx] = (((gi ^ gj ^ gk ^ A.sweep_a) & 1) == 0) ? xc + dinv * (rhs - Ax) : xc;
-  }
+  const double xnm1 = (SM == PAIR_CHEBY && A.c1a != 0.0) ? pair_vec(L, A, A.xm1, box)[idx] : xc;
+  pair_vec(L, A, A.out1, box)[idx] = edge_cell_x1<V, SM>(xc, x0_at(gi - 1, gj, gk, xc), x0_at(gi + 1, gj, gk, xc), x0_at(gi, gj - 1, gk, xc), x0_at(gi, gj + 1, gk, xc),
+                                                         x0_at(gi, gj, gk - 1, xc), x0_at(gi, gj, gk + 1, xc), bi0, bi1, bj0, bj1, bk0, bk1, al, dinv, rhs, xnm1,
+                                                         A, ((gi ^ gj ^ gk ^ A.sweep_a) & 1) == 0);
 }
 
 __global__ __launch_bounds__(256) void coef32_convert_kernel(const hpgmg_hip_level L, float *const *c32_base, int num_vectors) {
diff --git a/hpgmg_amd/csrc/kernels/pair.hip b/hpgmg_amd/csrc/kernels/pair.hip
--- a/hpgmg_amd/csrc/kernels/pair.hip
+++ b/hpgmg_amd/csrc/kernels/pair.hip
@@ -67,6 +67,8 @@
 static int g_pair_rem[6], g_pair_brick[3];
 static const double *g_pair_deep = nullptr, *g_pair_deep_beta = nullptr;
 static long long g_pair_launches = 0, g_pair_remote_launches = 0;
+static long long g_pair_prepass_launches = 0;
+static int g_pair_edge_inline = 1;
 static int g_pair_discard_x1 = 0;
 static const hpgmg_hip_level *g_pair_interp_level = nullptr;
 static int g_pair_interp_id = 0;
@@ -193,15 +195,19 @@
       }
     }
   }
+  const bool edge_inline = g_pair_edge_inline && !remote && !c32_base && A.tiles_i > 1 && nw <= 12;
+  const bool prepass = A.tiles_i > 1 && !edge_inline;
   const int prof = profile_begin(whole_cells);
 #define PAIR_NW_SWITCH(...) switch (nw) { case 10: { constexpr int NWC = 10; __VA_ARGS__ } break; case 12: { constexpr int NWC = 12; __VA_ARGS__ } break; default: { constexpr int NWC = 16; __VA_ARGS__ } break; }
-#define PAIR_LAUNCH2(VAR, C32, SM, NARROW, INTERP) PAIR_NW_SWITCH( \
-      static bool once = false; if (!once) { HPGMG_CHECK(hipFuncSetAttribute((const void *)cheby_pair_kernel<VAR, NWC, C32, SM, NARROW, INTERP>, hipFuncAttributeMaxDynamicSharedMemorySize, (int)((size_t)NWC * 6 * 64 * sizeof(p2)))); once = true; } \
-      hipLaunchKernelGGL((cheby_pair_kernel<VAR, NWC, C32, SM, NARROW, INTERP>), dim3(grid), dim3(64, NWC), lds, g_stream, *L, A); )
+#define PAIR_LAUNCH3(VAR, C32, SM, NARROW, INTERP, EDGE) PAIR_NW_SWITCH( \
+      constexpr bool EI = (EDGE) && !(C32) && NWC <= 12;       \
+      static bool once = false; if (!once) { HPGMG_CHECK(hipFuncSetAttribute((const void *)cheby_pair_kernel<VAR, NWC, C32, SM, NARROW, INTERP, false, EI>, hipFuncAttributeMaxDynamicSharedMemorySize, (int)((size_t)NWC * 6 * 64 * sizeof(p2)))); once = true; } \
+      hipLaunchKernelGGL((cheby_pair_kernel<VAR, NWC, C32, SM, NARROW, INTERP, false, EI>), dim3(grid), dim3(64, NWC), lds, g_stream, *L, A); )
+#define PAIR_LAUNCH2(VAR, C32, SM, NARROW, INTERP) { if (edge_inline) PAIR_LAUNCH3(VAR, C32, SM, NARROW, INTERP, true) else PAIR_LAUNCH3(VAR, C32, SM, NARROW, INTERP, false) }
 #define PAIR_LAUNCH_REMOTE_IP(VAR, SM, NRW, IP) { \
       const int ecols = 2 * (A.tiles_i - 1) + (A.rem[0] ? 1 : 0) + (A.rem[1] ? 1 : 0); \
       A.edge_blocks = ((A.Dj + 63) / 64) * A.Dk * ecols; const int egrid_r = grid_for(A.edge_blocks, &A.edge_per_xcd); \
-      if (ecols > 0) hipLaunchKernelGGL((cheby_pair_edge_kernel<VAR, false, SM, IP, true>), dim3(egrid_r), dim3(64), 0, g_stream, *L, A); \
+      if (ecols > 0) { hipLaunchKernelGGL((cheby_pair_edge_kernel<VAR, false, SM, IP, true>), dim3(egrid_r), dim3(64), 0, g_stream, *L, A); g_pair_prepass_launches++; } \
       PAIR_NW_SWITCH( \
       static bool once = false; if (!once) { HPGMG_CHECK(hipFuncSetAttribute((const void *)cheby_pair_kernel<VAR, NWC, false, SM, NRW, IP, true>, hipFuncAttributeMaxDynamicSharedMemorySize, (int)((size_t)NWC * 6 * 64 * sizeof(p2)))); once = true; } \
       hipLaunchKernelGGL((cheby_pair_kernel<VAR, NWC, false, SM, NRW, IP, true>), dim3(grid), dim3(64, NWC), lds, g_stream, *L, A); ) }
@@ -210,10 +216,10 @@
       A.edge_blocks = ((A.Dj + 63) / 64) * A.Dk * 2 * (A.tiles_i - 1); const dim3 egrid(A.edge_blocks > 0 ? grid_for(A.edge_blocks, &A.edge_per_xcd) : 1); \
       if (remote) PAIR_LAUNCH_REMOTE(VAR, SM) \
       else if (interp) { \
-        if (A.tiles_i > 1) hipLaunchKernelGGL((cheby_pair_edge_kernel<VAR, C32, SM, true>), egrid, dim3(64), 0, g_stream, *L, A); \
+        if (prepass) { hipLaunchKernelGGL((cheby_pair_edge_kernel<VAR, C32, SM, true>), egrid, dim3(64), 0, g_stream, *L, A); g_pair_prepass_launches++; } \
         if (L->dim % 128 == 0) PAIR_LAUNCH2(VAR, C32, SM, false, true) else PAIR_LAUNCH2(VAR, C32, SM, true, true) \
       } else { \
-        if (A.tiles_i > 1) hipLaunchKernelGGL((cheby_pair_edge_kernel<VAR, C32, SM, false>), egrid, dim3(64), 0, g_stream, *L, A); \
+        if (prepass) { hipLaunchKernelGGL((cheby_pair_edge_kernel<VAR, C32, SM, false>), egrid, dim3(64), 0, g_stream, *L, A); g_pair_prepass_launches++; } \
         if (L->dim % 128 == 0) PAIR_LAUNCH2(VAR, C32, SM, false, false) else PAIR_LAUNCH2(VAR, C32, SM, true, false) \
       } }
 #define PAIR_CASE(VAR) case VAR: \
@@ -228,6 +234,7 @@
 #undef PAIR_CASE
 #undef PAIR_LAUNCH
 #undef PAIR_LAUNCH2
+#undef PAIR_LAUNCH3
 #undef PAIR_NW_SWITCH
 #undef PAIR_LAUNCH_REMOTE
 #undef PAIR_LAUNCH_REMOTE_IP
@@ -254,6 +261,8 @@
 void hpgmg_hip_exp_timeline(void *buf) { g_exp_timeline = (double *)buf; }
 #endif
 void hpgmg_hip_pair_launch_counts(long long out[2]) { out[0] = g_pair_launches; out[1] = g_pair_remote_launches; }
+long long hpgmg_hip_pair_prepass_launches(void) { return g_pair_prepass_launches; }
+void hpgmg_hip_pair_set_edge_inline(int on) { g_pair_edge_inline = on ? 1 : 0; }
 
 static const hpgmg_hip_level *g_halo_fold_level = nullptr;
 static int g_halo_fold_id = 0;
diff --git a/include/hpgmg_hip.h b/include/hpgmg_hip.h
--- a/include/hpgmg_hip.h
+++ b/include/hpgmg_hip.h
@@ -126,6 +126,8 @@
 void hpgmg_hip_pair_packed_invalidate(const hpgmg_hip_level *L);
 void hpgmg_hip_pair_packed_forget(const hpgmg_hip_level *L);
 void hpgmg_hip_pair_launch_counts(long long out[2]);
+void hpgmg_hip_pair_set_edge_inline(int on);
+long long hpgmg_hip_pair_prepass_launches(void);
 typedef struct { int box, vec, i, j, k, ni, nj, nk, deep, pad_; long long off; } hpgmg_hip_halo_entry;
 void hpgmg_hip_pair_halo_fold_interpolation(const hpgmg_hip_level *Lc, int coarse_id, double prescale);
 int  hpgmg_hip_pair_halo_pack(const hpgmg_hip_level *L, double *const *scr_base, int x0_scr, int x0_id, int xm1_scr, int xm1_id, int rhs_id,
```

Result: slower. 6.189 billion (-2.8%).
